# roahmlab/armour

Measured on AMD Instinct MI355X. Metric: planning iters/s (eval_g+jac) Kinova 7-DOF, 100 timesteps × 20 obstacles, higher is better.
Workload: dtype f64

## Files before the change

armour_amd/csrc/api.hip:

```cpp
#include <algorithm>
#include <cmath>
#include <cstdarg>
#include <chrono>
#include <cstring>
#include <mutex>
#include <new>

#include "../../include/armour_robot_fetch.h"
#include "../../include/armour_robot_kinova.h"
#include "bezier.h"
#include "cacc.h"
#include "common.h"
#include "solver_common.h"

static thread_local char g_err[512] = "";

void armour_set_error(const char* fmt, ...) {
    va_list ap;
    va_start(ap, fmt);
    vsnprintf(g_err, sizeof(g_err), fmt, ap);
    va_end(ap);
}

extern "C" const char* armour_last_error(void) { return g_err; }

extern "C" void armour_robot_kinova_gen3_no_gripper(ArmourRobot* robot) { armour_fill_kinova_gen3_no_gripper(robot); }
extern "C" void armour_robot_kinova_gen3_gripper(ArmourRobot* robot) { armour_fill_kinova_gen3_gripper(robot); }
extern "C" void armour_robot_fetch(ArmourRobot* robot) { armour_fill_fetch(robot); }
extern "C" int armour_robot_fetch8(ArmourRobot* robot) {
#if ARMOUR_MAX_FACTORS >= 8
    if (!robot) { armour_set_error("null argument"); return ARMOUR_EINVAL; }
    armour_fill_fetch8(robot);
    return ARMOUR_OK;
#else
    (void)robot;
    armour_set_error("armour_robot_fetch8: an 8-factor robot needs the 128-bit-key library (libarmour_hip_k128.so: armour_abi_max_factors() == 8)");
    return ARMOUR_EINVAL;
#endif
}
extern "C" void armour_params_default(ArmourParams* params, int32_t T) { armour_fill_default_params(params, T); }

extern "C" int armour_device_available(void) {
    int n = 0;
    if (hipGetDeviceCount(&n) != hipSuccess) return 0;
    return n > 0 ? 1 : 0;
}

namespace {
struct PinnedRange { const char* p; size_t bytes; };
std::mutex g_pinned_mu;
std::vector<PinnedRange> g_pinned;
bool in_pinned(const void* q, size_t bytes) {
    if (!q) return true;
    const char* c = static_cast<const char*>(q);
    std::lock_guard<std::mutex> lk(g_pinned_mu);
    for (const PinnedRange& r : g_pinned)
        if (c >= r.p && c + bytes <= r.p + r.bytes) return true;
    return false;
}
}

extern "C" int armour_alloc_pinned(uint64_t bytes, void** out) {
    if (!out) { armour_set_error("null argument"); return ARMOUR_EINVAL; }
    HIPCHK(hipHostMalloc(out, bytes ? bytes : 1, hipHostMallocDefault));
    std::lock_guard<std::mutex> lk(g_pinned_mu);
    g_pinned.push_back({static_cast<const char*>(*out), (size_t)(bytes ? bytes : 1)});
    return ARMOUR_OK;
}
extern "C" void armour_free_pinned(void* p) {
    if (!p) return;
    {
        std::lock_guard<std::mutex> lk(g_pinned_mu);
        for (size_t i = 0; i < g_pinned.size(); i++)
            if (g_pinned[i].p == p) { g_pinned.erase(g_pinned.begin() + i); break; }
    }
    (void)hipHostFree(p);
}

static int ensure_capacity(ArmourPlanner* h, int B, int O) {
    if (B <= h->allocB && O <= h->allocO) return ARMOUR_OK;
    const int nb = B > h->allocB ? B : h->allocB, no = O > h->allocO ? O : h->allocO;
    h->allocB = 0; h->allocO = 0;
    const size_t nl = (size_t)nb * h->J * h->T, nt = (size_t)nb * h->n * h->T;
    ARMOUR_TRY(h->d_link_count.reserve(nl));
    ARMOUR_TRY(h->d_link_center.reserve(nl * 3));
    ARMOUR_TRY(h->d_link_indep.reserve(nl * 3));
    ARMOUR_TRY(h->d_link_keys.reserve(nl * h->lim.link_monomials));
    ARMOUR_TRY(h->d_link_coeff.reserve(nl * h->lim.link_monomials * 3));
    ARMOUR_TRY(h->d_tq_count.reserve(nt));
    ARMOUR_TRY(h->d_tq_center.reserve(nt));
    ARMOUR_TRY(h->d_tq_indep.reserve(nt));
    ARMOUR_TRY(h->d_tq_keys.reserve(nt * h->lim.torque_monomials));
    ARMOUR_TRY(h->d_tq_coeff.reserve(nt * h->lim.torque_monomials));
    ARMOUR_TRY(h->d_planes.reserve((size_t)nb * armour_planes_per_problem(h->J * h->T * no)));
    ARMOUR_TRY(h->d_planes_ll.reserve((size_t)nb * armour_planes_ll_per_problem(h->J * h->T)));
    ARMOUR_TRY(h->d_obs_center.reserve((size_t)nb * 3 * (no > 0 ? no : 1)));
    ARMOUR_TRY(h->d_plane_skip.reserve((size_t)nb));
    ARMOUR_TRY(h->d_bez.reserve((size_t)nb * 3 * h->n));
    const size_t mmax = (size_t)h->n * h->T + (size_t)h->J * h->T * no + 4 * h->n;
    ARMOUR_TRY(h->d_k.reserve((size_t)nb * h->n));
    ARMOUR_TRY(h->d_g.reserve((size_t)nb * mmax + std::max((size_t)nb * mmax * h->n, (size_t)nb * h->T * h->J * 3)));
    h->d_jac = h->d_g + (size_t)nb * mmax;
    ARMOUR_TRY(h->d_bounds.reserve((size_t)2 * nb * mmax));
    h->allocB = nb;
    h->allocO = no;
    return ARMOUR_OK;
}

P2Tables armour_make_tables(const ArmourPlanner* h) {
    P2Tables tb;
    memset(&tb, 0, sizeof(tb));
    tb.B = h->B; tb.T = h->T; tb.J = h->J; tb.n = h->n; tb.O = h->O; tb.Q = h->Q; tb.m = h->m;
    tb.capL = h->lim.link_monomials; tb.capT = h->lim.torque_monomials;
    tb.row0 = h->row0; tb.mode = h->mode;
    tb.link_count = h->d_link_count; tb.link_center = h->d_link_center; tb.link_indep = h->d_link_indep;
    tb.link_keys = h->d_link_keys; tb.link_coeff = h->d_link_coeff;
    tb.tq_count = h->d_tq_count; tb.tq_center = h->d_tq_center; tb.tq_indep = h->d_tq_indep;
    tb.tq_keys = h->d_tq_keys; tb.tq_coeff = h->d_tq_coeff;
    tb.planes = h->d_planes; tb.planes_ll = h->d_planes_ll; tb.ll_shared = h->ll_shared;
    tb.ex_allowed = h->tune(ARMOUR_OPT_P2_EX);
    tb.obs_center = (h->d_from_center && (h->B >= 8 || !h->planes_have_d)) ? h->d_obs_center : nullptr;
    tb.plane_skip = h->d_plane_skip; tb.bez = h->d_bez;
    for (int i = 0; i < ARMOUR_MAX_FACTORS; i++) tb.k_range[i] = h->params.k_range[i];
    tb.duration = h->params.duration;
    return tb;
}

namespace {
struct TuningSpec { int option; double def, lo, hi; };
const TuningSpec kTuning[] = {
    {ARMOUR_OPT_P1_STEP_WAVES, 0, 0, 4}, {ARMOUR_OPT_P1_STEP_FREE, 1, 0, 1}, {ARMOUR_OPT_P1_STEP_SPLIT_FK, -1, -1, 1}, {ARMOUR_OPT_P1_STEP_AUX3, 1, 0, 1},
    {ARMOUR_OPT_P1_MAX_WAVES_PER_CU, 4, 1, 8}, {ARMOUR_OPT_P1_TWO_PASS, 1, 0, 1}, {ARMOUR_OPT_P1_STEP_PAIRS, 1, 0, 2}, {ARMOUR_OPT_P1_STEP_QUEUE, 1, 0, 3}, {ARMOUR_OPT_P1_STEP_TAIL_CROSS, 0, 0, 514}, {ARMOUR_OPT_P1_STEP_TWO_CU, 3, 0, 33}, {ARMOUR_OPT_P1_STEP_LEAN_BACK, 1, 0, 3}, {ARMOUR_OPT_P1_TV_TAIL_CROSS, 111, 0, 514} ,
    {ARMOUR_OPT_P1_TV_MIN_GROUPS, 31, 1, 1e6}, {ARMOUR_OPT_P1_TV_WAVES, 0, 0, 8}, {ARMOUR_OPT_P1_TV_FREE, 1, 0, 1}, {ARMOUR_OPT_P1_TV_SPLIT_FK, -1, -1, 1},
    {ARMOUR_OPT_P1_TV_DEDICATED, 1, 0, 1}, {ARMOUR_OPT_P1_TV_HELP_SHIFT, 0, 0, 3}, {ARMOUR_OPT_P1_TV_HELPERS, 1, 0, 31}, {ARMOUR_OPT_P1_TV_HELP_MIN, 192, 1, 1e6},
    {ARMOUR_OPT_P1_TV_HELP_N, 1, 0, 1}, {ARMOUR_OPT_P1_TV_AUX3, 1, 0, 1}, {ARMOUR_OPT_P1_TV_ROW_WIDTH, 0, 0, 64}, {ARMOUR_OPT_P1_FULL_PLANES, 0, 0, 1},
    {ARMOUR_OPT_P2_EX, 1, 0, 1}, {ARMOUR_OPT_STEPS_GRAPH_MIN, 2, 0, 1e6}, {ARMOUR_OPT_PINNED_MODE, 0, 0, 2}, {ARMOUR_OPT_CULL_ROWS, 0, 0, 1},
    {ARMOUR_OPT_SOLVE_SUB_TILES, 48, 1, 1e6}, {ARMOUR_OPT_SOLVE_DEVICE, 1, 0, 2}, {ARMOUR_OPT_SOLVE_CUT_TILES, 156, 1, 1e6}, {ARMOUR_OPT_SOLVE_BLOCKS, 0, 0, 1e6},
    {ARMOUR_OPT_SOLVE_SUB_BATCH, 0, 0, 1e6}, {ARMOUR_OPT_SOLVE_ROW_CAP, 0, 0, 1e7}, {ARMOUR_OPT_SOLVE_HARD_CAP_S, 0, 0, 1e6}, {ARMOUR_OPT_SOLVE_WAVES_PER_SIMD, 0, 0, 2}, {ARMOUR_OPT_SOLVE_CULL, -1, -1, 1},
};
const TuningSpec* tuning_spec(int option) {
    for (const TuningSpec& t : kTuning) if (t.option == option) return &t;
    return nullptr;
}
}
void armour_tuning_defaults(double* tuning) {
    for (int o = ARMOUR_OPT_FIRST_TUNING; o <= ARMOUR_OPT_LAST_TUNING; o++) tuning[o - ARMOUR_OPT_FIRST_TUNING] = 0.0;
    for (const TuningSpec& t : kTuning) tuning[t.option - ARMOUR_OPT_FIRST_TUNING] = t.def;
}
bool armour_trace_p1() { static const bool on = getenv("ARMOUR_P1_TRACE") != nullptr; return on; }
BuildStamps& armour_build_stamps() { static thread_local BuildStamps s; return s; }
void armour_build_stamp(const char* name) {
    if (!armour_trace_p1()) return;
    BuildStamps& s = armour_build_stamps();
    if (s.n < 12) { s.t[s.n] = std::chrono::duration<double, std::micro>(std::chrono::steady_clock::now().time_since_epoch()).count(); s.name[s.n] = name; s.n++; }
}
static void armour_build_stamps_print(const char* what) {
    if (!armour_trace_p1()) return;
    BuildStamps& s = armour_build_stamps();
    fprintf(stderr, "[%s, host side, us]", what);
    for (int i = 1; i < s.n; i++) fprintf(stderr, " %s %.1f", s.name[i], s.t[i] - s.t[i - 1]);
    if (s.n > 1) fprintf(stderr, " | total %.1f\n", s.t[s.n - 1] - s.t[0]);
}
bool armour_trace_solve() { static const bool on = getenv("ARMOUR_SOLVE_TIMING") != nullptr; return on; }

extern "C" int armour_create(const ArmourRobot* robot, const ArmourParams* params, const ArmourLimits* limits,
                             int32_t device, ArmourPlanner** out) {
    if (!robot || !params || !out) { armour_set_error("armour_create: null argument"); return ARMOUR_EINVAL; }
    if (!armour_robot_shape_ok(robot)) {
        armour_set_error("armour_create: unsupported robot (joints=%d, factors=%d; max %d joints, %d factors -- the monomial key "
                         "packs 9 bits per factor into 64, RT/PZsparse.h:8-21)", robot->num_joints, robot->num_factors,
                         ARMOUR_MAX_JOINTS, ARMOUR_MAX_FACTORS);
        return ARMOUR_EINVAL;
    }
    for (int i = 0; i < robot->num_joints; i++)
        if ((i < robot->num_factors) != (robot->axes[i] != 0)) {
            armour_set_error("armour_create: the actuated joints must come first and the fixed ones last (RT/Dynamics.cu:103-105)");
            return ARMOUR_EINVAL;
        }
    if (params->num_time_steps < 2 || (params->num_time_steps & 1)) {
        armour_set_error("armour_create: num_time_steps must be even and >= 2 (RT/Parameters.h:16)");
        return ARMOUR_EINVAL;
    }
    int ndev = 0;
    if (hipGetDeviceCount(&ndev) != hipSuccess || ndev <= 0) {
        armour_set_error("armour_create: no HIP device visible -- libarmour_hip has no CPU path");
        return ARMOUR_EDEVICE;
    }
    if (device < 0 || device >= ndev) { armour_set_error("armour_create: device %d out of range (%d visible)", device, ndev); return ARMOUR_EINVAL; }
    HIPCHK(hipSetDevice(device));
    ArmourPlanner* h = new (std::nothrow) ArmourPlanner();
    if (!h) { armour_set_error("out of host memory"); return ARMOUR_EINVAL; }
    h->robot = *robot;
    h->params = *params;
    armour_tuning_defaults(h->tuning);
    ArmourLimits lim;
    memset(&lim, 0, sizeof(lim));
    if (limits) lim = *limits;
    if (lim.max_batch <= 0) lim.max_batch = 1;
    if (lim.max_obstacles <= 0) lim.max_obstacles = 40;
    if (lim.link_monomials <= 0) lim.link_monomials = 32;
    if (lim.torque_monomials <= 0) lim.torque_monomials = 128;
    if (lim.work_monomials <= 0) lim.work_monomials = 1024;
    if (lim.raw_terms <= 0) lim.raw_terms = 4096;
    h->lim = lim;
    h->ub = armour_ultimate_bound(robot);
    h->device = device;
    h->T = params->num_time_steps; h->J = robot->num_joints; h->n = robot->num_factors;
    hipError_t e = hipStreamCreateWithFlags(&h->stream, hipStreamNonBlocking);
    if (e != hipSuccess) { armour_set_error("hipStreamCreate failed: %s", hipGetErrorString(e)); delete h; return ARMOUR_EDEVICE; }
    *out = h;
    return ARMOUR_OK;
}

double* armour_handle_pinned(ArmourPlanner* h, int slot, size_t bytes) {
    if (h->solve_pin[slot] && h->solve_pin_bytes[slot] >= bytes) return static_cast<double*>(h->solve_pin[slot]);
    if (h->solve_pin[slot]) { armour_free_pinned(h->solve_pin[slot]); h->solve_pin[slot] = nullptr; h->solve_pin_bytes[slot] = 0; }
    void* p = nullptr;
    if (armour_alloc_pinned(bytes, &p) != ARMOUR_OK) return nullptr;
    h->solve_pin[slot] = p; h->solve_pin_bytes[slot] = bytes;
    return static_cast<double*>(p);
}

static void drop_step_graphs(ArmourPlanner* h) {
    for (auto& g : h->step_graphs) (void)hipGraphExecDestroy(g.exec);
    h->step_graphs.clear();
}

extern "C" void armour_destroy(ArmourPlanner* h) {
    if (!h) return;
    (void)hipSetDevice(h->device);
    if (h->stream) (void)hipStreamSynchronize(h->stream);
    drop_step_graphs(h);
    for (void* pin : h->solve_pin) armour_free_pinned(pin);
    armour_p1_free(h);
    if (h->stream) (void)hipStreamDestroy(h->stream);
    delete h;
}

static int begin_problem_set(ArmourPlanner* h, int B, int O, const double* q0, const double* qd0, const double* qdd0,
                             const double* q_des, int mode = ARMOUR_MODE_ARMOUR) {
    if (!h || !q0 || !qd0 || !qdd0 || !q_des) { armour_set_error("null argument"); return ARMOUR_EINVAL; }
    if (B < 1 || O < 0) { armour_set_error("bad batch/obstacle count (B=%d, O=%d)", B, O); return ARMOUR_EINVAL; }
    {
        const double* arrs[4] = {q0, qd0, qdd0, q_des};
        const size_t bn = (size_t)B * h->n;
        for (int a = 0; a < 4; a++)
            if (const size_t i = first_nonfinite(arrs[a], bn); i < bn) { armour_set_error("non-finite entry in the initial state / goal arrays (array %d, entry %zu)", a, i); return ARMOUR_EINVAL; }
    }
    HIPCHK(hipSetDevice(h->device));
    h->ready = false;
    h->rel.fresh = false; h->rel2.fresh = false;
    h->bounds_on_device = false; h->bounds_on_host = false;
    h->tables_from_host = false;
    h->stats_fresh = false;
    drop_step_graphs(h);
    int rc = ensure_capacity(h, B, O);
    if (rc != ARMOUR_OK) return rc;
    h->B = B; h->O = O; h->Q = h->J * h->T * O;
    h->mode = mode;
    h->row0 = h->no_torque() ? 0 : h->n * h->T;
    h->m = h->row0 + h->Q + 4 * h->n;
    h->d_jac = h->d_g + (size_t)B * h->m;
    const size_t bn = (size_t)B * h->n;
    h->h_q0.assign(q0, q0 + bn); h->h_qd0.assign(qd0, qd0 + bn);
    h->h_qdes.assign(q_des, q_des + bn);
    if (mode == ARMOUR_MODE_ARMTD) { h->h_qdd0.assign(bn, 0.0); h->h_krange.assign(qdd0, qdd0 + bn); }
    else { h->h_qdd0.assign(qdd0, qdd0 + bn); h->h_krange.clear(); }
    std::vector<double> bz((size_t)B * 3 * h->n);
    const double D = mode == ARMOUR_MODE_ARMTD ? 1.0 : h->params.duration;
    for (int b = 0; b < B; b++)
        for (int i = 0; i < h->n; i++) {
            bz[((size_t)b * 3 + 0) * h->n + i] = q0[b * h->n + i];
            bz[((size_t)b * 3 + 1) * h->n + i] = qd0[b * h->n + i] * D;
            bz[((size_t)b * 3 + 2) * h->n + i] = qdd0[b * h->n + i] * D * D;
        }
    HIPCHK(hipMemcpy(h->d_bez, bz.data(), bz.size() * sizeof(double), hipMemcpyHostToDevice));
    return ARMOUR_OK;
}

int armour_refresh_table_stats(ArmourPlanner* h) {
    if (h->stats_fresh) { h->stats_fresh = false; return ARMOUR_OK; }
    const size_t nl = (size_t)h->B * h->J * h->T, nt = (size_t)h->B * h->n * h->T;
    std::vector<int> lc(nl), tc(nt);
    HIPCHK(hipMemcpy(lc.data(), h->d_link_count, nl * sizeof(int), hipMemcpyDeviceToHost));
    HIPCHK(hipMemcpy(tc.data(), h->d_tq_count, nt * sizeof(int), hipMemcpyDeviceToHost));
    long long sl = 0, st = 0;
    int ml = 0, mt = 0;
    for (int v : lc) { sl += v; if (v > ml) ml = v; }
    for (int v : tc) { st += v; if (v > mt) mt = v; }
    h->sum_link = sl; h->sum_torque = st; h->max_link = ml; h->max_torque = mt;
    h->h_plane_skip.assign((size_t)h->B, 0ull);
    if (h->O > 0) HIPCHK(hipMemcpy(h->h_plane_skip.data(), h->d_plane_skip, (size_t)h->B * sizeof(unsigned long long), hipMemcpyDeviceToHost));
    if (h->O > 0 && armour_trace_p1()) {
        unsigned long long all_and = ~0ull, all_or = 0ull;
        for (unsigned long long v : h->h_plane_skip) { all_and &= v; all_or |= v; }
        fprintf(stderr, "[P1 planes] plane_skip of %d problem(s): AND 0x%09llx OR 0x%09llx\n", h->B, all_and & ((1ull << ARMOUR_NPLANES) - 1ull), all_or & ((1ull << ARMOUR_NPLANES) - 1ull));
    }
    return ARMOUR_OK;
}

static int check_obstacles(int B, int O, const double* obstacles) {
    if (O > 0 && !obstacles) { armour_set_error("obstacles is null but O=%d", O); return ARMOUR_EINVAL; }
    const size_t cnt = (size_t)B * O * 12;
    if (const size_t i = first_nonfinite(obstacles, cnt); i < cnt) { armour_set_error("non-finite obstacle entry %zu", i); return ARMOUR_EINVAL; }
    return ARMOUR_OK;
}

extern "C" int armour_set_problems(ArmourPlanner* h, int32_t B, int32_t O, const double* q0, const double* qd0,
                                   const double* qdd0, const double* q_des, const double* obstacles) {
    armour_build_stamps().n = 0;
    armour_build_stamp("start");
    int rc = begin_problem_set(h, B, O, q0, qd0, qdd0, q_des);
    if (rc != ARMOUR_OK) return rc;
    ARMOUR_TRY(check_obstacles(B, O, obstacles));
    armour_build_stamp("checks+bezier-upload");
    rc = armour_p1_build(h, obstacles);
    if (rc != ARMOUR_OK) return rc;
    armour_build_stamp("copy-out");
    rc = armour_refresh_table_stats(h);
    if (rc != ARMOUR_OK) return rc;
    h->ready = true;
    armour_build_stamp("table-stats");
    armour_build_stamps_print("armour_set_problems");
    return ARMOUR_OK;
}

extern "C" int armour_set_problems_armtd(ArmourPlanner* h, int32_t B, int32_t O, const double* q0, const double* qd0, const double* q_des,
                                         const double* jrs, const double* k_range, const double* obstacles) {
    if (!jrs || !k_range) { armour_set_error("null argument"); return ARMOUR_EINVAL; }
    int rc = begin_problem_set(h, B, O, q0, qd0, k_range, q_des, ARMOUR_MODE_ARMTD);
    if (rc != ARMOUR_OK) return rc;
    ARMOUR_TRY(check_obstacles(B, O, obstacles));
    const size_t cnt = (size_t)B * h->n * 6 * h->T;
    if (const size_t i = first_nonfinite(jrs, cnt); i < cnt) { armour_set_error("non-finite entry %zu in the offline JRS tables", i); return ARMOUR_EINVAL; }
    ARMOUR_TRY(h->d_jrs.reserve(cnt));
    HIPCHK(hipMemcpy(h->d_jrs, jrs, cnt * sizeof(double), hipMemcpyHostToDevice));
    rc = armour_p1_build(h, obstacles);
    if (rc != ARMOUR_OK) return rc;
    rc = armour_refresh_table_stats(h);
    if (rc != ARMOUR_OK) return rc;
    h->ready = true;
    return ARMOUR_OK;
}

extern "C" int armour_debug_load_tables(ArmourPlanner* h, int32_t B, int32_t O, const double* q0, const double* qd0,
                                        const double* qdd0, const double* q_des, const int32_t* link_count,
                                        const double* link_center, const uint64_t* link_keys, const double* link_coeffs,
                                        int32_t cap_l, const int32_t* torque_count, const double* torque_center,
                                        const uint64_t* torque_keys, const double* torque_coeffs, int32_t cap_t,
                                        const double* A, const double* d, const double* delta, const double* torque_radius) {
    int rc = begin_problem_set(h, B, O, q0, qd0, qdd0, q_des);
    if (rc != ARMOUR_OK) return rc;
    h->build_ms = 0; h->build_info[0] = h->build_info[1] = h->build_info[2] = h->build_info[3] = 0;
    h->h_prune_margin.clear();
    const int J = h->J, T = h->T, n = h->n, capL = h->lim.link_monomials, capT = h->lim.torque_monomials;
    const size_t nl = (size_t)B * J * T, nt = (size_t)B * n * T;
    std::vector<double> lc(nl * 3), li(nl * 3), lco(nl * capL * 3, 0.0), tc(nt), ti(nt), tco(nt * capT, 0.0);
    std::vector<uint32_t> lk(nl * capL, 0), tk(nt * capT, 0);
    for (size_t i = 0; i < nl; i++) {
        if (link_count[i] > capL) { armour_set_error("link PZ %zu has %d monomials > capacity %d", i, link_count[i], capL); return ARMOUR_ECAPACITY; }
        for (int e = 0; e < 3; e++) { lc[i * 3 + e] = link_center[(i * 2) * 3 + e]; li[i * 3 + e] = link_center[(i * 2 + 1) * 3 + e]; }
        for (int mo = 0; mo < link_count[i]; mo++) {
            lk[i * capL + mo] = (uint32_t)link_keys[i * cap_l + mo];
            for (int e = 0; e < 3; e++) lco[(i * capL + mo) * 3 + e] = link_coeffs[(i * cap_l + mo) * 3 + e];
        }
    }
    for (size_t i = 0; i < nt; i++) {
        if (torque_count[i] > capT) { armour_set_error("torque PZ %zu has %d monomials > capacity %d", i, torque_count[i], capT); return ARMOUR_ECAPACITY; }
        tc[i] = torque_center[i * 2]; ti[i] = torque_center[i * 2 + 1];
        for (int mo = 0; mo < torque_count[i]; mo++) { tk[i * capT + mo] = (uint32_t)torque_keys[i * cap_t + mo]; tco[i * capT + mo] = torque_coeffs[i * cap_t + mo]; }
    }
    const size_t ppp = armour_planes_per_problem(h->Q);
    std::vector<double> pl((size_t)B * ppp, 0.0);
    for (int b = 0; b < B; b++)
        for (int t = 0; t < T; t++)
            for (int l = 0; l < J; l++)
                for (int o = 0; o < O; o++)
                    for (int p = 0; p < 36; p++) {
                        const size_t src = ((((size_t)b * T + t) * J + l) * O + o) * 36 + p;
                        const int q = (l * T + t) * O + o;
                        double* base = &pl[(size_t)b * ppp];
                        base[armour_plane_index(h->Q, q, p, 0)] = A[src * 3 + 0]; base[armour_plane_index(h->Q, q, p, 1)] = A[src * 3 + 1];
                        base[armour_plane_index(h->Q, q, p, 2)] = A[src * 3 + 2];
                        base[armour_plane_index(h->Q, q, p, 3)] = d[src]; base[armour_plane_index(h->Q, q, p, 4)] = delta[src];
                    }
#define UP(dst, vec) HIPCHK(hipMemcpy(dst, vec.data(), vec.size() * sizeof(vec[0]), hipMemcpyHostToDevice))
    HIPCHK(hipMemcpy(h->d_link_count, link_count, nl * sizeof(int), hipMemcpyHostToDevice));
    HIPCHK(hipMemcpy(h->d_tq_count, torque_count, nt * sizeof(int), hipMemcpyHostToDevice));
    UP(h->d_link_center, lc); UP(h->d_link_indep, li); UP(h->d_link_keys, lk); UP(h->d_link_coeff, lco);
    UP(h->d_tq_center, tc); UP(h->d_tq_indep, ti); UP(h->d_tq_keys, tk); UP(h->d_tq_coeff, tco);
    if (!pl.empty()) UP(h->d_planes, pl);
    {
        const int JT = J * T;
        std::vector<double> pll((size_t)B * armour_planes_ll_per_problem(JT), 0.0);
        bool shared = O > 0;
        for (int b = 0; b < B && O > 0; b++)
            for (int t = 0; t < T; t++)
                for (int l = 0; l < J; l++)
                    for (int p = ARMOUR_FIRST_LL_PLANE; p < 36; p++)
                        for (int o = 0; o < O; o++) {
                            const size_t src = ((((size_t)b * T + t) * J + l) * O + o) * 36 + p, src0 = ((((size_t)b * T + t) * J + l) * O) * 36 + p;
                            for (int cc = 0; cc < 3; cc++) {
                                if (o == 0) pll[(size_t)b * armour_planes_ll_per_problem(JT) + armour_plane_ll_index(JT, l * T + t, p - ARMOUR_FIRST_LL_PLANE, cc)] = A[src * 3 + cc];
                                else if (memcmp(&A[src * 3 + cc], &A[src0 * 3 + cc], sizeof(double)) != 0) shared = false;
                            }
                        }
        UP(h->d_planes_ll, pll);
        h->ll_shared = shared ? 1 : 0;
        h->d_from_center = 0;
        h->planes_lean = 0; h->planes_have_d = 1;
    }
    HIPCHK(hipMemset(h->d_plane_skip, 0, (size_t)B * sizeof(unsigned long long)));
#undef UP
    h->h_torque_radius.assign(torque_radius, torque_radius + (size_t)B * n * T);
    h->h_link_gens.assign((size_t)B * T * J * 18, 0.0);
    rc = armour_refresh_table_stats(h);
    if (rc != ARMOUR_OK) return rc;
    h->tables_from_host = true;
    h->ready = true;
    return ARMOUR_OK;
}

static const double* torque_radius_of(const ArmourPlanner* h, int b) { return h->no_torque() ? nullptr : &h->h_torque_radius[(size_t)b * h->n * h->T]; }

extern "C" int armour_get_sizes(const ArmourPlanner* h, int32_t* B, int32_t* n, int32_t* m) {
    NEED_READY(h);
    if (B) *B = h->B;
    if (n) *n = h->n;
    if (m) *m = h->m;
    return ARMOUR_OK;
}

extern "C" int armour_get_bounds(ArmourPlanner* h, double* x_l, double* x_u, double* g_l, double* g_u) {
    NEED_READY(h);
    const int n = h->n;
    if (x_l) for (int i = 0; i < n; i++) x_l[i] = -1.0;
    if (x_u) for (int i = 0; i < n; i++) x_u[i] = 1.0;
    if (!g_l || !g_u) return ARMOUR_OK;
    const slv::RowRule R = armour_row_rule(h);
    const slv::RowLimits L = armour_row_limits(h);
    for (int b = 0; b < h->B; b++) {
        const double* tr = torque_radius_of(h, b);
        for (int r = 0; r < R.m; r++) slv::row_bounds(R, L, r, tr, &g_l[(size_t)b * R.m + r], &g_u[(size_t)b * R.m + r]);
    }
    return ARMOUR_OK;
}

int armour_checked_collision_rows(const ArmourPlanner* h) {
    return h->mode == ARMOUR_MODE_ARMTD ? (h->n - 1 < h->J ? h->n - 1 : h->J) * h->T * h->O : h->Q;
}

slv::RowRule armour_row_rule(const ArmourPlanner* h) {
    slv::RowRule R;
    R.n = h->n; R.T = h->T; R.m = h->m; R.row0 = h->row0; R.Q = h->Q; R.n_checked = armour_checked_collision_rows(h);
    R.torque_slack = h->params.torque_violation_threshold; R.collision_slack = h->params.collision_violation_threshold;
    return R;
}

slv::RowLimits armour_row_limits(const ArmourPlanner* h) {
    slv::RowLimits L;
    for (int j = 0; j < ARMOUR_MAX_FACTORS; j++) {
        L.torque_limits[j] = h->robot.torque_limits[j]; L.lb[j] = h->robot.state_limits_lb[j]; L.ub[j] = h->robot.state_limits_ub[j]; L.speed[j] = h->robot.speed_limits[j];
    }
    L.qe = h->ub.qe; L.qde = h->ub.qde;
    return L;
}

void armour_plan_coeffs(const ArmourPlanner* h, size_t ix, double c[3]) {
    const double D = h->params.duration;
    const bool armtd = h->mode == ARMOUR_MODE_ARMTD;
    c[0] = h->h_q0[ix];
    c[1] = armtd ? h->h_qd0[ix] : h->h_qd0[ix] * D;
    c[2] = armtd ? h->h_krange[ix] : h->h_qdd0[ix] * D * D;
}

extern "C" int armour_eval_f(ArmourPlanner* h, const double* k, double* f) {
    NEED_READY(h);
    const int n = h->n;
    for (int b = 0; b < h->B; b++) {
        double sq[slv::NV];
        for (int i = 0; i < n; i++) {
            const size_t ix = (size_t)b * n + i;
            double c[3];
            armour_plan_coeffs(h, ix, c);
            const double qp = slv::plan_point(h->mode, c[0], c[1], c[2], h->params.k_range[i], k[ix], h->params.t_plan);
            const double e = h->robot.continuous[i] ? slv::wrap_to_pi(h->h_qdes[ix] - qp) : (h->h_qdes[ix] - qp);
            sq[i] = e * e;
        }
        f[b] = slv::cost_from_sq(n, h->continuous_mask(), sq, h->params.cost_scale);
    }
    return ARMOUR_OK;
}

extern "C" int armour_eval_grad_f(ArmourPlanner* h, const double* k, double* grad_f) {
    NEED_READY(h);
    const int n = h->n;
    const double tp = h->params.t_plan;
    for (int b = 0; b < h->B; b++)
        for (int i = 0; i < n; i++) {
            const size_t ix = (size_t)b * n + i;
            double c[3];
            armour_plan_coeffs(h, ix, c);
            const double qp = slv::plan_point(h->mode, c[0], c[1], c[2], h->params.k_range[i], k[ix], tp);
            const double dk = slv::plan_dk(h->mode, c[2], h->params.k_range[i], tp);
            const double e = h->robot.continuous[i] ? slv::wrap_to_pi(qp - h->h_qdes[ix]) : (qp - h->h_qdes[ix]);
            grad_f[ix] = 2 * e * dk * h->params.cost_scale;
        }
    return ARMOUR_OK;
}

extern "C" int armour_desired_trajectory(int32_t n, const double* q0, const double* qd0, const double* qdd0, const double* k_range,
                                         double duration, const double* k, double t, double* q, double* qd, double* qdd) {
    if (n < 1 || !q0 || !qd0 || !qdd0 || !k_range || !k || !(duration > 0)) { armour_set_error("bad argument"); return ARMOUR_EINVAL; }
    const double D = duration, s = t / D;
    for (int i = 0; i < n; i++) {
        const double a = qd0[i] * D, b = qdd0[i] * D * D, ka = k_range[i] * k[i];
        if (q) q[i] = bez::q_des(q0[i], a, b, ka, s);
        if (qd) qd[i] = bez::qd_des(q0[i], a, b, ka, s) / D;
        if (qdd) qdd[i] = bez::qdd_des(q0[i], a, b, ka, s) / (D * D);
    }
    return ARMOUR_OK;
}

extern "C" int armour_eval_g_jac_device(ArmourPlanner* h, const double* d_k, double* d_g, double* d_jac, void* stream) {
    NEED_READY(h);
    if (!d_k) { armour_set_error("d_k is null"); return ARMOUR_EINVAL; }
    const P2Tables tb = armour_make_tables(h);
    return armour_p2_launch(tb, h->max_link, h->max_torque, h->h_plane_skip.data(), d_k, d_g, d_jac, stream ? (hipStream_t)stream : h->stream);
}

static int enqueue_steps(ArmourPlanner* h, const double* d_k, int steps, double* d_g, double* d_jac, hipStream_t st) {
    const P2Tables tb = armour_make_tables(h);
    const size_t stride = (size_t)h->B * h->n;
    for (int s = 0; s < steps; s++) {
        int rc = armour_p2_launch(tb, h->max_link, h->max_torque, h->h_plane_skip.data(), d_k + (size_t)s * stride, d_g, d_jac, st);
        if (rc != ARMOUR_OK) return rc;
    }
    return ARMOUR_OK;
}

static int steps_graph(ArmourPlanner* h, const double* d_k, int steps, double* d_g, double* d_jac, hipGraphExec_t* out) {
    h->graph_clock++;
    for (auto& g : h->step_graphs)
        if (g.d_k == d_k && g.steps == steps && g.d_g == d_g && g.d_jac == d_jac) { g.last_use = h->graph_clock; *out = g.exec; return ARMOUR_OK; }
    HIPCHK(hipSetDevice(h->device));
    HIPCHK(hipStreamSynchronize(h->stream));
    hipGraph_t graph = nullptr;
    HIPCHK(hipStreamBeginCapture(h->stream, hipStreamCaptureModeThreadLocal));
    const int rc = enqueue_steps(h, d_k, steps, d_g, d_jac, h->stream);
    const hipError_t e = hipStreamEndCapture(h->stream, &graph);
    if (rc != ARMOUR_OK) { if (graph) (void)hipGraphDestroy(graph); return rc; }
    if (e != hipSuccess) { armour_set_error("hipStreamEndCapture failed: %s", hipGetErrorString(e)); return ARMOUR_EDEVICE; }
    hipGraphExec_t exec = nullptr;
    const hipError_t ei = hipGraphInstantiate(&exec, graph, nullptr, nullptr, 0);
    (void)hipGraphDestroy(graph);
    if (ei != hipSuccess) { armour_set_error("hipGraphInstantiate failed: %s", hipGetErrorString(ei)); return ARMOUR_EDEVICE; }
    if (h->step_graphs.size() >= 4) {
        size_t lru = 0;
        for (size_t i = 1; i < h->step_graphs.size(); i++) if (h->step_graphs[i].last_use < h->step_graphs[lru].last_use) lru = i;
        (void)hipGraphExecDestroy(h->step_graphs[lru].exec);
        h->step_graphs.erase(h->step_graphs.begin() + lru);
    }
    h->step_graphs.push_back({d_k, steps, d_g, d_jac, exec, h->graph_clock});
    *out = exec;
    return ARMOUR_OK;
}

static bool steps_use_graph(const ArmourPlanner* h, int steps) {
    const int min_steps = h->tune(ARMOUR_OPT_STEPS_GRAPH_MIN);
    return min_steps > 0 && steps >= min_steps;
}

extern "C" int armour_prepare_steps(ArmourPlanner* h, const double* d_k, int32_t steps, double* d_g, double* d_jac) {
    NEED_READY(h);
    if (!d_k || steps < 0) { armour_set_error("bad argument"); return ARMOUR_EINVAL; }
    if (!steps_use_graph(h, steps)) return ARMOUR_OK;
    hipGraphExec_t exec;
    return steps_graph(h, d_k, steps, d_g, d_jac, &exec);
}

extern "C" int armour_eval_g_jac_device_steps(ArmourPlanner* h, const double* d_k, int32_t steps, double* d_g, double* d_jac,
                                              void* stream) {
    NEED_READY(h);
    if (!d_k || steps < 0) { armour_set_error("bad argument"); return ARMOUR_EINVAL; }
    if (steps == 0 || (!d_g && !d_jac)) return ARMOUR_OK;
    const hipStream_t st = stream ? (hipStream_t)stream : h->stream;
    if (steps_use_graph(h, steps))
        for (auto& g : h->step_graphs)
            if (g.d_k == d_k && g.steps == steps && g.d_g == d_g && g.d_jac == d_jac) {
                g.last_use = ++h->graph_clock;
                HIPCHK(hipGraphLaunch(g.exec, st));
                return ARMOUR_OK;
            }
    return enqueue_steps(h, d_k, steps, d_g, d_jac, st);
}

extern "C" int armour_eval_g_jac_device_multi(ArmourPlanner* h, const double* d_k, int32_t points, double* d_g, double* d_jac,
                                              void* stream) {
    NEED_READY(h);
    if (!d_k || points < 0) { armour_set_error("bad argument"); return ARMOUR_EINVAL; }
    if (points == 0) return ARMOUR_OK;
    const P2Tables tb = armour_make_tables(h);
    const long long bn = (long long)h->B * h->n, bm = (long long)h->B * h->m;
    return armour_p2_launch(tb, h->max_link, h->max_torque, h->h_plane_skip.data(), d_k, d_g, d_jac, stream ? (hipStream_t)stream : h->stream,
                            points, bn, bm, bm * h->n);
}

int armour_spin_on_stream(hipStream_t st) {
    for (;;) {
        const hipError_t q = hipStreamQuery(st);
        if (q == hipSuccess) return ARMOUR_OK;
        if (q != hipErrorNotReady) { armour_set_error("hipStreamQuery failed: %s", hipGetErrorString(q)); return ARMOUR_EDEVICE; }
    }
}

extern "C" int armour_eval_g_jac(ArmourPlanner* h, const double* k, double* g, double* jac) {
    NEED_READY(h);
    if (!k) { armour_set_error("k is null"); return ARMOUR_EINVAL; }
    HIPCHK(hipSetDevice(h->device));
    const size_t bn = (size_t)h->B * h->n, bm = (size_t)h->B * h->m;
    const P2Tables tb = armour_make_tables(h);
    const int pinned_mode = h->tune(ARMOUR_OPT_PINNED_MODE);
    const bool all_pinned = in_pinned(k, bn * sizeof(double)) && in_pinned(g, bm * sizeof(double)) && in_pinned(jac, bm * h->n * sizeof(double));
    if (all_pinned && pinned_mode == 1) {
        int rc = armour_p2_launch(tb, h->max_link, h->max_torque, h->h_plane_skip.data(), k, g, jac, h->stream);
        if (rc != ARMOUR_OK) return rc;
        return armour_spin_on_stream(h->stream);
    }
    const double* k_dev = h->d_k;
    if (all_pinned && pinned_mode == 2) k_dev = k;
    else HIPCHK(hipMemcpyAsync(h->d_k, k, bn * sizeof(double), hipMemcpyHostToDevice, h->stream));
    int rc = armour_p2_launch(tb, h->max_link, h->max_torque, h->h_plane_skip.data(), k_dev, g ? h->d_g : nullptr, jac ? h->d_jac : nullptr, h->stream);
    if (rc != ARMOUR_OK) return rc;
    if (g && jac && jac == g + bm) {
        HIPCHK(hipMemcpyAsync(g, h->d_g, bm * (1 + (size_t)h->n) * sizeof(double), hipMemcpyDeviceToHost, h->stream));
        return armour_spin_on_stream(h->stream);
    }
    if (g) HIPCHK(hipMemcpyAsync(g, h->d_g, bm * sizeof(double), hipMemcpyDeviceToHost, h->stream));
    if (jac) HIPCHK(hipMemcpyAsync(jac, h->d_jac, bm * h->n * sizeof(double), hipMemcpyDeviceToHost, h->stream));
    return armour_spin_on_stream(h->stream);
}

extern "C" int armour_check_feasible(ArmourPlanner* h, const double* g, int32_t* feasible) {
    NEED_READY(h);
    const slv::RowRule R = armour_row_rule(h);
    const slv::RowLimits L = armour_row_limits(h);
    for (int b = 0; b < h->B; b++) {
        const double* gb = g + (size_t)b * R.m;
        const double* tr = torque_radius_of(h, b);
        bool ok = true;
        for (int r = 0; r < R.m && ok; r++) {
            double l, u;
            slv::row_bounds(R, L, r, tr, &l, &u);
            ok = !slv::outside_slack(R, r, gb[r], l, u);
        }
        feasible[b] = ok ? 1 : 0;
    }
    return ARMOUR_OK;
}

namespace {
struct BoundsArgs {
    slv::RowRule rule;
    slv::RowLimits lim;
    const double* tr;
    double* lo; double* hi;
};
__global__ __launch_bounds__(256) void armour_bounds_kernel(BoundsArgs a) {
    const int b = blockIdx.y, r = blockIdx.x * 256 + threadIdx.x, m = a.rule.m;
    if (r >= m) return;
    double l, u;
    slv::row_bounds(a.rule, a.lim, r, a.tr + (size_t)b * a.rule.n * a.rule.T, &l, &u);
    a.lo[(size_t)b * m + r] = l;
    a.hi[(size_t)b * m + r] = u;
}
}

int armour_bounds_launch(ArmourPlanner* h, const double* d_tr) {
    const size_t bm = (size_t)h->B * h->m;
    BoundsArgs a;
    a.rule = armour_row_rule(h); a.lim = armour_row_limits(h);
    a.lo = h->d_bounds; a.hi = h->d_bounds + bm;
    a.tr = d_tr;
    hipLaunchKernelGGL(armour_bounds_kernel, dim3((h->m + 255) / 256, h->B), dim3(256), 0, h->stream, a);
    HIPCHK(hipGetLastError());
    h->bounds_on_device = true;
    return ARMOUR_OK;
}

int armour_upload_bounds(ArmourPlanner* h) {
    if (h->bounds_on_device) return ARMOUR_OK;
    const double* d_tr = nullptr;
    if (!h->no_torque()) {
        const size_t ntr = (size_t)h->B * h->n * h->T;
        ARMOUR_TRY(h->d_tr_stage.reserve(ntr));
        HIPCHK(hipMemcpyAsync(h->d_tr_stage, h->h_torque_radius.data(), ntr * sizeof(double), hipMemcpyHostToDevice, h->stream));
        d_tr = h->d_tr_stage;
    }
    const int rc = armour_bounds_launch(h, d_tr);
    if (rc != ARMOUR_OK) return rc;
    HIPCHK(hipStreamSynchronize(h->stream));
    return ARMOUR_OK;
}

extern "C" int armour_set_option(ArmourPlanner* h, int32_t option, double value) {
    if (!h) { armour_set_error("null handle"); return ARMOUR_EINVAL; }
    if (option == ARMOUR_OPT_P1_BUILD && (value == 0.0 || value == 1.0 || value == 2.0)) { h->opt_p1_build = (int)value; return ARMOUR_OK; }
    if (option == ARMOUR_OPT_P1_WORK_MEMORY_MB && value >= 0.0 && value <= 1e9) { h->opt_p1_work_mb = value; return ARMOUR_OK; }
    if (option == ARMOUR_OPT_P1_KEEP_WORK_MEMORY && (value == 0.0 || value == 1.0)) { h->opt_p1_keep_work = (int)value; return ARMOUR_OK; }
    if (const TuningSpec* t = tuning_spec(option)) {
        bool ok = value >= t->lo && value <= t->hi && (option == ARMOUR_OPT_SOLVE_HARD_CAP_S || value == (double)(long long)value);
        if (ok && (option == ARMOUR_OPT_P1_STEP_TAIL_CROSS || option == ARMOUR_OPT_P1_TV_TAIL_CROSS)) {
            const int v = (int)value, lo2 = v % 100, hi2 = v / 100;
            ok = (lo2 <= 4 || (lo2 >= 10 && lo2 <= 14)) && hi2 <= 5;
        }
        if (ok && option == ARMOUR_OPT_P1_TV_ROW_WIDTH) ok = value == 0.0 || value == 50.0 || value == 64.0;
        if (ok && option == ARMOUR_OPT_P1_STEP_TWO_CU) { const int lv = (int)value % 10; ok = lv <= 3 && (value < 10.0 || lv >= 1); if (ok) h->p1_two_cu_off = false; }
        if (ok) {
            h->tuning[option - ARMOUR_OPT_FIRST_TUNING] = value;
            h->p1_step_cap_hint = 0; h->p1_tv_shape_hint = 0;
            return ARMOUR_OK;
        }
    }
    armour_set_error("armour_set_option: unknown option %d or bad value %g", option, value);
    return ARMOUR_EINVAL;
}

extern "C" int armour_abi_max_factors(void) { return ARMOUR_MAX_FACTORS; }

extern "C" int armour_device_memory(int32_t device, uint64_t* free_bytes, uint64_t* total_bytes) {
    int ndev = 0;
    if (hipGetDeviceCount(&ndev) != hipSuccess || device < 0 || device >= ndev) { (void)hipGetLastError(); armour_set_error("armour_device_memory: no such device %d", device); return ARMOUR_EDEVICE; }
    HIPCHK(hipSetDevice(device));
    size_t f = 0, t = 0;
    HIPCHK(hipMemGetInfo(&f, &t));
    if (free_bytes) *free_bytes = f;
    if (total_bytes) *total_bytes = t;
    return ARMOUR_OK;
}

extern "C" int armour_get_option(ArmourPlanner* h, int32_t option, double* value) {
    if (!h || !value) { armour_set_error("null argument"); return ARMOUR_EINVAL; }
    if (option == ARMOUR_OPT_P1_BUILD) { *value = h->opt_p1_build; return ARMOUR_OK; }
    if (option == ARMOUR_OPT_P1_WORK_MEMORY_MB) { *value = h->opt_p1_work_mb; return ARMOUR_OK; }
    if (option == ARMOUR_OPT_P1_KEEP_WORK_MEMORY) { *value = h->opt_p1_keep_work; return ARMOUR_OK; }
    if (tuning_spec(option)) { *value = h->tuning[option - ARMOUR_OPT_FIRST_TUNING]; return ARMOUR_OK; }
    armour_set_error("armour_get_option: unknown option %d", option);
    return ARMOUR_EINVAL;
}

namespace {
struct ViolArgs {
    slv::RowRule rule;
    const double* g; const double* lo; const double* hi;
    ArmourViolation* out;
};
__global__ __launch_bounds__(256) void armour_violation_kernel(ViolArgs a) {
    __shared__ slv::ViolShared<1> sh;
    const int b = blockIdx.x, tid = threadIdx.x, m = a.rule.m;
    const double* g = a.g + (size_t)b * m;
    const double* lo = a.lo + (size_t)b * m;
    const double* hi = a.hi + (size_t)b * m;
    slv::ViolPartial p[1];
    for (int r = tid; r < m; r += 256) p[0].take(a.rule, r, g[r], lo[r], hi[r]);
    slv::ViolPartial::tree_reduce(sh, p, tid);
    if (tid == 0) a.out[b] = slv::ViolPartial::finish(sh, 0);
}
}

static int eval_violations_device_impl(ArmourPlanner* h, const double* d_k, ArmourViolation* d_out, void* stream, bool allow_cull) {
    NEED_READY(h);
    if (!d_k || !d_out) { armour_set_error("null argument"); return ARMOUR_EINVAL; }
    HIPCHK(hipSetDevice(h->device));
    int rc = armour_upload_bounds(h);
    if (rc != ARMOUR_OK) return rc;
    const hipStream_t st = stream ? (hipStream_t)stream : h->stream;
    if (allow_cull && h->tune(ARMOUR_OPT_CULL_ROWS)) return armour_eval_violations_culled(h, d_k, d_out, st);
    const P2Tables tb = armour_make_tables(h);
    rc = armour_p2_launch(tb, h->max_link, h->max_torque, h->h_plane_skip.data(), d_k, h->d_g, nullptr, st);
    if (rc != ARMOUR_OK) return rc;
    ViolArgs a;
    a.rule = armour_row_rule(h);
    a.g = h->d_g; a.lo = h->d_bounds; a.hi = h->d_bounds + (size_t)h->B * h->m; a.out = d_out;
    hipLaunchKernelGGL(armour_violation_kernel, dim3(h->B), dim3(256), 0, st, a);
    HIPCHK(hipGetLastError());
    return ARMOUR_OK;
}

extern "C" int armour_eval_violations_device(ArmourPlanner* h, const double* d_k, ArmourViolation* d_out, void* stream) {
    return eval_violations_device_impl(h, d_k, d_out, stream, true);
}

extern "C" int armour_eval_violations(ArmourPlanner* h, const double* k, ArmourViolation* out) {
    NEED_READY(h);
    if (!k || !out) { armour_set_error("null argument"); return ARMOUR_EINVAL; }
    HIPCHK(hipSetDevice(h->device));
    const size_t bn = (size_t)h->B * h->n;
    ARMOUR_TRY(h->d_viol.reserve((size_t)h->B));
    double* hk = armour_handle_pinned(h, 6, bn * sizeof(double));
    ArmourViolation* hv = reinterpret_cast<ArmourViolation*>(armour_handle_pinned(h, 7, (size_t)h->B * sizeof(ArmourViolation)));
    if (!hk || !hv) return ARMOUR_EDEVICE;
    memcpy(hk, k, bn * sizeof(double));
    HIPCHK(hipMemcpyAsync(h->d_k, hk, bn * sizeof(double), hipMemcpyHostToDevice, h->stream));
    bool in_box = true;
    for (size_t i = 0; i < bn && in_box; i++) in_box = fabs(k[i]) <= 1.0;
    int rc = eval_violations_device_impl(h, h->d_k, h->d_viol, h->stream, in_box);
    if (rc != ARMOUR_OK) return rc;
    HIPCHK(hipMemcpyAsync(hv, h->d_viol, (size_t)h->B * sizeof(ArmourViolation), hipMemcpyDeviceToHost, h->stream));
    rc = armour_spin_on_stream(h->stream);
    if (rc != ARMOUR_OK) return rc;
    memcpy(out, hv, (size_t)h->B * sizeof(ArmourViolation));
    return ARMOUR_OK;
}

extern "C" int armour_get_torque_radius(ArmourPlanner* h, double* out) {
    NEED_READY(h);
    memcpy(out, h->h_torque_radius.data(), h->h_torque_radius.size() * sizeof(double));
    return ARMOUR_OK;
}

extern "C" int armour_get_link_generators(ArmourPlanner* h, double* out) {
    NEED_READY(h);
    memcpy(out, h->h_link_gens.data(), h->h_link_gens.size() * sizeof(double));
    return ARMOUR_OK;
}

extern "C" int armour_get_link_centers(ArmourPlanner* h, const double* k, double* centers) {
    NEED_READY(h);
    HIPCHK(hipSetDevice(h->device));
    const size_t bn = (size_t)h->B * h->n, cnt = (size_t)h->B * h->T * h->J * 3;
    HIPCHK(hipMemcpyAsync(h->d_k, k, bn * sizeof(double), hipMemcpyHostToDevice, h->stream));
    const P2Tables tb = armour_make_tables(h);
    int rc = armour_p2_slice_links_launch(tb, h->d_k, h->d_jac, h->stream);
    if (rc != ARMOUR_OK) return rc;
    HIPCHK(hipMemcpyAsync(centers, h->d_jac, cnt * sizeof(double), hipMemcpyDeviceToHost, h->stream));
    HIPCHK(hipStreamSynchronize(h->stream));
    return ARMOUR_OK;
}

extern "C" int armour_get_pz(ArmourPlanner* h, int32_t b, int32_t which, int32_t i, int32_t t, double* center,
                             uint64_t* keys, double* coeffs, int32_t capacity) {
    NEED_READY(h);
    if (b < 0 || b >= h->B || t < 0 || t >= h->T || which < 0 || which > 1 || i < 0 || i >= (which == 0 ? h->J : h->n)) {
        armour_set_error("armour_get_pz: index out of range");
        return ARMOUR_EINVAL;
    }
    if (which == 1 && h->no_torque()) {
        if (center) center[0] = center[1] = 0.0;
        return 0;
    }
    HIPCHK(hipSetDevice(h->device));
    HIPCHK(hipStreamSynchronize(h->stream));
    const int sz = which == 0 ? 3 : 1;
    const int cap = which == 0 ? h->lim.link_monomials : h->lim.torque_monomials;
    const size_t idx = which == 0 ? ((size_t)b * h->J + i) * h->T + t : ((size_t)b * h->n + i) * h->T + t;
    int cnt = 0;
    HIPCHK(hipMemcpy(&cnt, (which == 0 ? h->d_link_count : h->d_tq_count) + idx, sizeof(int), hipMemcpyDeviceToHost));
    if (center) {
        HIPCHK(hipMemcpy(center, (which == 0 ? h->d_link_center : h->d_tq_center) + idx * sz, sz * sizeof(double), hipMemcpyDeviceToHost));
        HIPCHK(hipMemcpy(center + sz, (which == 0 ? h->d_link_indep : h->d_tq_indep) + idx * sz, sz * sizeof(double), hipMemcpyDeviceToHost));
    }
    if (keys && coeffs) {
        if (capacity < cnt) { armour_set_error("armour_get_pz: capacity %d < count %d", capacity, cnt); return ARMOUR_EINVAL; }
        std::vector<uint32_t> k32(cnt > 0 ? cnt : 1);
        if (cnt > 0) {
            HIPCHK(hipMemcpy(k32.data(), (which == 0 ? h->d_link_keys : h->d_tq_keys) + idx * cap, cnt * sizeof(uint32_t), hipMemcpyDeviceToHost));
            HIPCHK(hipMemcpy(coeffs, (which == 0 ? h->d_link_coeff : h->d_tq_coeff) + idx * cap * sz, (size_t)cnt * sz * sizeof(double), hipMemcpyDeviceToHost));
        }
        for (int mo = 0; mo < cnt; mo++) keys[mo] = k32[mo];
    }
    return cnt;
}

extern "C" int armour_get_table_sizes(ArmourPlanner* h, int64_t* out4) {
    NEED_READY(h);
    out4[0] = h->sum_link; out4[1] = h->sum_torque; out4[2] = h->max_link; out4[3] = h->max_torque;
    return ARMOUR_OK;
}

extern "C" int armour_get_hyperplanes(ArmourPlanner* h, double* A, double* d, double* delta) {
    NEED_READY(h);
    HIPCHK(hipSetDevice(h->device));
    HIPCHK(hipStreamSynchronize(h->stream));
    const int B = h->B, T = h->T, J = h->J, O = h->O;
    const size_t ppp = armour_planes_per_problem(h->Q);
    std::vector<double> pl(h->Q > 0 ? (size_t)B * ppp : 0);
    if (pl.empty()) return ARMOUR_OK;
    if (h->planes_lean) {
        DevBuf<double> d_full;
        int rc = d_full.reserve(pl.size());
        if (rc == ARMOUR_OK) rc = armour_p1_full_planes(h, d_full);
        if (rc != ARMOUR_OK) return rc;
        if (hipMemcpy(pl.data(), d_full, pl.size() * sizeof(double), hipMemcpyDeviceToHost) != hipSuccess) { armour_set_error("copy of the half-space table failed"); return ARMOUR_EDEVICE; }
    } else
    HIPCHK(hipMemcpy(pl.data(), h->d_planes, pl.size() * sizeof(double), hipMemcpyDeviceToHost));
    for (int b = 0; b < B; b++)
        for (int t = 0; t < T; t++)
            for (int l = 0; l < J; l++)
                for (int o = 0; o < O; o++)
                    for (int p = 0; p < 36; p++) {
                        const size_t dst = ((((size_t)b * T + t) * J + l) * O + o) * 36 + p;
                        const int q = (l * T + t) * O + o;
                        const double* base = &pl[(size_t)b * ppp];
                        if (A) { A[dst * 3 + 0] = base[armour_plane_index(h->Q, q, p, 0)]; A[dst * 3 + 1] = base[armour_plane_index(h->Q, q, p, 1)]; A[dst * 3 + 2] = base[armour_plane_index(h->Q, q, p, 2)]; }
                        if (d) d[dst] = base[armour_plane_index(h->Q, q, p, 3)];
                        if (delta) delta[dst] = base[armour_plane_index(h->Q, q, p, 4)];
                    }
    return ARMOUR_OK;
}

extern "C" int armour_debug_pz_op(ArmourPlanner* h, int32_t op, int32_t nops, const int32_t* sz, const int32_t* cnt, const uint64_t* const* keys,
                                  const double* const* coef, const double* cen, const double* ind, const double* ind2, const double* consts,
                                  int32_t r, int32_t out_cap, uint64_t* out_keys, double* out_coef, double* out_misc) {
    if (!h || nops < 1 || nops > 3 || op < 0 || op > 11) { armour_set_error("armour_debug_pz_op: bad argument"); return ARMOUR_EINVAL; }
    for (int o = 0; o < nops; o++)
        if ((sz[o] != 1 && sz[o] != 3 && sz[o] != 9) || cnt[o] < 0 || cnt[o] > h->lim.work_monomials || (sz[o] == 9 && o == 1 && cnt[o] > 8)) {
            armour_set_error("armour_debug_pz_op: bad operand"); return ARMOUR_EINVAL;
        }
    return armour_p1_debug_pz_op(h, op, nops, sz, cnt, keys, coef, cen, ind, ind2, consts, r, out_cap, out_keys, out_coef, out_misc);
}

extern "C" int armour_get_plane_skip(ArmourPlanner* h, uint64_t* plane_skip) {
    NEED_READY(h);
    if (!plane_skip) { armour_set_error("null argument"); return ARMOUR_EINVAL; }
    for (int b = 0; b < h->B; b++) plane_skip[b] = (uint64_t)h->h_plane_skip[b] & ((1ull << ARMOUR_NPLANES) - 1ull);
    return ARMOUR_OK;
}

extern "C" int armour_get_prune_margin(ArmourPlanner* h, double* margin) {
    NEED_READY(h);
    if (!margin) { armour_set_error("null argument"); return ARMOUR_EINVAL; }
    if ((int)h->h_prune_margin.size() != h->B) { armour_set_error("no reach-set build on this handle (tables loaded by armour_debug_load_tables carry no prune margin)"); return ARMOUR_ESTATE; }
    for (int b = 0; b < h->B; b++) margin[b] = h->h_prune_margin[(size_t)b];
    return ARMOUR_OK;
}

extern "C" int armour_get_build_ms(ArmourPlanner* h, double* ms) {
    NEED_READY(h);
    *ms = h->build_ms;
    return ARMOUR_OK;
}

extern "C" int armour_get_build_info(ArmourPlanner* h, int32_t* out4) {
    NEED_READY(h);
    if (!out4) { armour_set_error("null argument"); return ARMOUR_EINVAL; }
    for (int i = 0; i < 4; i++) out4[i] = h->build_info[i];
    return ARMOUR_OK;
}
```

armour_amd/csrc/common.h:

```cpp
#pragma once

#include <hip/hip_runtime.h>

#include <cstdint>
#include <cstdio>
#include <string>
#include <vector>

#include "../../include/armour_hip.h"
#include "device_mem.h"
#include "row_rules.h"

#define ARMOUR_NPLANES 36
#define ARMOUR_PLANE_COMPONENTS 5

#define ARMOUR_FIRST_LL_PLANE 21
#define ARMOUR_N_LL_PLANES 15
__host__ __device__ inline int armour_row_stride(int Q) { return (Q + 15) & ~15; }
__host__ __device__ inline size_t armour_planes_ab_offset(int Q) { (void)Q; return 0; }
__host__ __device__ inline size_t armour_planes_cd_offset(int Q) { return (size_t)2 * ARMOUR_NPLANES * armour_row_stride(Q); }
__host__ __device__ inline size_t armour_planes_dll_offset(int Q) { return (size_t)4 * ARMOUR_NPLANES * armour_row_stride(Q); }
__host__ __device__ inline size_t armour_planes_d_offset(int Q) { return (size_t)(4 * ARMOUR_NPLANES + 16) * armour_row_stride(Q); }
__host__ __device__ inline size_t armour_planes_per_problem(int Q) { return (size_t)(5 * ARMOUR_NPLANES + 16) * armour_row_stride(Q); }
__host__ __device__ inline size_t armour_plane_index(int Q, int q, int p, int c) {
    const size_t Qs = (size_t)armour_row_stride(Q);
    if (c < 2) return ((size_t)p * Qs + q) * 2 + c;
    if (c == 2) return armour_planes_cd_offset(Q) + ((size_t)p * Qs + q) * 2;
    if (c == 3) return armour_planes_d_offset(Q) + (size_t)p * Qs + q;
    if (p < ARMOUR_FIRST_LL_PLANE) return armour_planes_cd_offset(Q) + ((size_t)p * Qs + q) * 2 + 1;
    return armour_planes_dll_offset(Q) + ((size_t)((p - ARMOUR_FIRST_LL_PLANE) >> 1) * Qs + q) * 2 + ((p - ARMOUR_FIRST_LL_PLANE) & 1);
}
#define ARMOUR_RECOMPUTE_D_ROWS 32768
#define ARMOUR_LL_RECORD 48
__host__ __device__ inline size_t armour_planes_ll_per_problem(int JT) { return (size_t)ARMOUR_LL_RECORD * (size_t)JT; }
__host__ __device__ inline size_t armour_plane_ll_index(int JT, int lt, int pll, int c) { (void)JT; return (size_t)lt * ARMOUR_LL_RECORD + (size_t)pll * 3 + c; }

int armour_spin_on_stream(hipStream_t st);

struct P2Tables {
    int B, T, J, n, O, Q, m;
    int capL, capT;
    int row0;
    const int* link_count;
    const double* link_center;
    const double* link_indep;
    const uint32_t* link_keys;
    const double* link_coeff;
    const int* tq_count;
    const double* tq_center;
    const double* tq_indep;
    const uint32_t* tq_keys;
    const double* tq_coeff;
    const double* planes;
    const double* obs_center;
    const double* planes_ll;
    int ll_shared;
    int ex_allowed;
    int mode;
    const unsigned long long* plane_skip;
    const double* bez;
    double k_range[ARMOUR_MAX_FACTORS];
    double duration;
};

#define ARMOUR_MODE_ARMOUR 0
#define ARMOUR_MODE_ARMTD 1

struct SolveDeviceWork {
    DevBuf<unsigned char> ctl;
    DevBuf<unsigned char> blk_word;
    int words_clean = 0;
    DevBuf<unsigned char> blk_rows, qp_rows, flags;
};

struct RelLists {
    DevBuf<unsigned char> mask;
    DevBuf<int> rows;
    DevBuf<int> count;
    DevBuf<double> packed;
    DevBuf<long long> pack_off;
    DevBuf<int> extra;
    std::vector<int> h_count, h_tq_count;
    int max_count = 0;
    bool fresh = false;
    double ms = 0;
};

struct ArmourPlanner {
    ArmourRobot robot;
    ArmourParams params;
    ArmourLimits lim;
    ArmourUltimateBound ub;
    int device = 0;
    hipStream_t stream = nullptr;
    int T = 0, J = 0, n = 0;
    int B = 0, O = 0, Q = 0, m = 0;
    bool ready = false;
    int mode = ARMOUR_MODE_ARMOUR;
    bool no_torque() const { return mode == ARMOUR_MODE_ARMTD || params.input_constraints_off != 0; }
    int continuous_mask() const { int mk = 0; for (int i = 0; i < n; i++) if (robot.continuous[i]) mk |= 1 << i; return mk; }
    int row0 = 0;
    std::vector<double> h_krange;
    DevBuf<double> d_jrs;
    void* solve_pin[10] = {nullptr, nullptr, nullptr, nullptr, nullptr, nullptr, nullptr, nullptr, nullptr, nullptr};
    size_t solve_pin_bytes[10] = {0, 0, 0, 0, 0, 0, 0, 0, 0, 0};
    bool stats_fresh = false;
    int opt_p1_build = 0;
    double opt_p1_work_mb = 0;
    int opt_p1_keep_work = 1;
    double tuning[ARMOUR_OPT_LAST_TUNING - ARMOUR_OPT_FIRST_TUNING + 1];
    int tune(int option) const { return (int)tuning[option - ARMOUR_OPT_FIRST_TUNING]; }
    double tune_f(int option) const { return tuning[option - ARMOUR_OPT_FIRST_TUNING]; }
    DevBuf<ArmourViolation> d_viol;
    RelLists rel, rel2;
    int rel2_tq_cap = 0;
    DevBuf<unsigned char> d_sweep;
    SolveDeviceWork solve_dev;
    DevBuf<double> d_bounds;
    bool bounds_on_device = false, bounds_on_host = false;
    bool tables_from_host = false;
    std::vector<double> h_gl, h_gu;
    std::vector<double> h_q0, h_qd0, h_qdd0, h_qdes;
    std::vector<double> h_torque_radius;
    DevBuf<double> d_tr_stage;
    std::vector<double> h_link_gens;
    std::vector<unsigned long long> h_plane_skip;
    std::vector<double> h_prune_margin;
    int allocB = 0, allocO = 0;
    DevBuf<int> d_link_count;
    DevBuf<double> d_link_center;
    DevBuf<double> d_link_indep;
    DevBuf<uint32_t> d_link_keys;
    DevBuf<double> d_link_coeff;
    DevBuf<int> d_tq_count;
    DevBuf<double> d_tq_center;
    DevBuf<double> d_tq_indep;
    DevBuf<uint32_t> d_tq_keys;
    DevBuf<double> d_tq_coeff;
    DevBuf<double> d_planes;
    DevBuf<double> d_obs_center;
    int d_from_center = 0;
    int planes_lean = 0;
    int planes_have_d = 1;
    double planes_ms = 0;
    DevBuf<double> d_planes_ll;
    int ll_shared = 0;
    DevBuf<unsigned long long> d_plane_skip;
    DevBuf<double> d_bez;
    DevBuf<double> d_k;
    DevBuf<double> d_g;
    double* d_jac = nullptr;
    double build_ms = 0;
    int p1_step_cap_hint = 0, p1_tv_shape_hint = 0;
    bool p1_two_cu_off = false;
    int p1_hint_B = 0, p1_hint_T = 0, p1_hint_O = 0, p1_hint_builds = 0;
    int build_info[4] = {0, 0, 0, 0};
    int max_link = 0, max_torque = 0;
    long long sum_link = 0, sum_torque = 0;
    void* p1 = nullptr;
    struct StepsGraph { const double* d_k; int steps; double* d_g; double* d_jac; hipGraphExec_t exec; unsigned long long last_use; };
    std::vector<StepsGraph> step_graphs;
    unsigned long long graph_clock = 0;
};

void armour_tuning_defaults(double* tuning);
bool armour_trace_p1();
bool armour_trace_solve();

int armour_p2_launch(const P2Tables& tb, int max_link, int max_torque, const unsigned long long* h_skip, const double* d_k, double* d_g, double* d_jac, hipStream_t stream,
                     int steps = 1, long long k_stride = 0, long long g_stride = 0, long long j_stride = 0, bool skip_collision_blocks = false);
int armour_relevance_build(ArmourPlanner* h, bool for_solver);
int armour_eval_violations_culled(ArmourPlanner* h, const double* d_k, ArmourViolation* d_out, hipStream_t st);
int armour_refresh_table_stats(ArmourPlanner* h);
int armour_checked_collision_rows(const ArmourPlanner* h);
slv::RowRule armour_row_rule(const ArmourPlanner* h);
slv::RowLimits armour_row_limits(const ArmourPlanner* h);
#define NEED_READY(h)                                                                        \
    if (!(h)) { armour_set_error("null handle"); return ARMOUR_EINVAL; }                     \
    if (!(h)->ready) { armour_set_error("no problem set: call armour_set_problems first"); return ARMOUR_ESTATE; }
void armour_plan_coeffs(const ArmourPlanner* h, size_t ix, double c[3]);
double* armour_handle_pinned(ArmourPlanner* h, int slot, size_t bytes);
int armour_p2_slice_links_launch(const P2Tables& tb, const double* d_k, double* d_centers, hipStream_t stream);
P2Tables armour_make_tables(const ArmourPlanner* h);
int armour_upload_bounds(ArmourPlanner* h);
struct BuildStamps { double t[12]; const char* name[12]; int n; };
BuildStamps& armour_build_stamps();
void armour_build_stamp(const char* name);
int armour_bounds_launch(ArmourPlanner* h, const double* d_torque_radius);

int armour_p1_build(ArmourPlanner* h, const double* obstacles);
void armour_p1_free(ArmourPlanner* h);
int armour_p1_full_planes(ArmourPlanner* h, double* d_full);

inline int armour_p1_auto_kernel(int B, int T, int min_groups, bool fk_only) {
    return (long long)B * T >= 50ll * (fk_only ? min_groups * 5 / 3 : min_groups) ? ARMOUR_P1_KERNEL_TIME_VECTORISED : ARMOUR_P1_KERNEL_PER_STEP;
}

int armour_p1_debug_pz_op(ArmourPlanner* h, int op, int nops, const int* sz, const int* cnt, const uint64_t* const* keys,
                          const double* const* coef, const double* cen, const double* ind, const double* ind2, const double* consts,
                          int r, int out_cap, uint64_t* out_keys, double* out_coef, double* out_misc);
```

armour_amd/csrc/solver.hip:

```cpp
#include <chrono>
#include <cmath>
#include <cstdio>
#include <cstdlib>
#include <cstring>
#include <thread>
#include <vector>

#include "bezier.h"
#include "common.h"
#include "solver_common.h"
#include "solver_device.h"

using slv::NV;
using slv::SolveRow;

namespace {

constexpr double kInf = 1e300;
using Clock = std::chrono::steady_clock;

bool spd_solve(const double* M, int q, const double* rhs, double* y) {
    double L[NV][NV], inv[NV];
    for (int i = 0; i < q; i++)
        for (int j = 0; j <= i; j++) {
            double s = M[i * NV + j];
            for (int k = 0; k < j; k++) s -= L[i][k] * L[j][k];
            if (i == j) {
                if (s <= 1e-14 * std::fabs(M[i * NV + i]) || s <= 0) return false;
                L[i][i] = std::sqrt(s);
                inv[i] = 1.0 / L[i][i];
            } else {
                L[i][j] = s * inv[j];
            }
        }
    double t[NV];
    for (int i = 0; i < q; i++) {
        double s = rhs[i];
        for (int k = 0; k < i; k++) s -= L[i][k] * t[k];
        t[i] = s * inv[i];
    }
    for (int i = q - 1; i >= 0; i--) {
        double s = t[i];
        for (int k = i + 1; k < q; k++) s -= L[k][i] * y[k];
        y[i] = s * inv[i];
    }
    return true;
}

struct QpRow {
    double a[NV];
    double b;
};

struct QpResult {
    double x[NV];
    double max_mult;
    int iterations;
    bool feasible;
    int dropped, dropped_mid, excluded, active;
};

QpResult solve_qp(int n, const double* Gd, const double* g0, const std::vector<QpRow>& rows, int max_iter = slv::kQpMaxSteps, int box_rows = 0) {
    QpResult res;
    res.iterations = 0; res.feasible = true; res.max_mult = 0;
    res.dropped = res.dropped_mid = res.excluded = res.active = 0;
    double x[NV], invG[NV];
    for (int j = 0; j < n; j++) { invG[j] = 1.0 / Gd[j]; x[j] = -g0[j] * invG[j]; }
    if (box_rows == 2 * n && (int)rows.size() >= box_rows) {
        const int m0 = (int)rows.size() - box_rows;
        double lo[NV], hi[NV], d[NV];
        for (int j = 0; j < n; j++) { lo[j] = rows[m0 + 2 * j].b; hi[j] = -rows[m0 + 2 * j + 1].b; }
        const double mm = slv::box_clipped_step(n, Gd, invG, g0, lo, hi, d);
        bool ok = true;
        for (int i = 0; i < (int)rows.size() && ok; i++) {
            double s = -rows[i].b;
            for (int j = 0; j < n; j++) s += rows[i].a[j] * d[j];
            if (s < -1e-7) ok = false;
        }
        if (ok) {
            for (int j = 0; j < n; j++) res.x[j] = d[j];
            res.max_mult = mm;
            return res;
        }
    }
    int A[NV];
    double u[NV + 1];
    int q = 0;
    const int m = (int)rows.size();
    std::vector<char> is_active(m, 0), excluded(m, 0);
    for (;;) {
        int p = -1;
        double worst = -1e-10;
        for (int i = 0; i < m; i++) {
            if (is_active[i] || excluded[i]) continue;
            double s = -rows[i].b;
            for (int j = 0; j < n; j++) s += rows[i].a[j] * x[j];
            if (s < worst) { worst = s; p = i; }
        }
        if (p < 0) break;
        if (++res.iterations > max_iter) { res.feasible = false; break; }
        const double* np = rows[p].a;
        double up = 0.0;
        bool added = false;
        for (int guard = 0; guard < 4 * NV + 8 && !added; guard++) {
            double r[NV] = {0}, z[NV];
            if (q > 0) {
                double M[NV * NV], rhs[NV];
                for (int i = 0; i < q; i++) {
                    for (int k = 0; k <= i; k++) {
                        double s = 0;
                        for (int j = 0; j < n; j++) s += rows[A[i]].a[j] * rows[A[k]].a[j] * invG[j];
                        M[i * NV + k] = s; M[k * NV + i] = s;
                    }
                    double s = 0;
                    for (int j = 0; j < n; j++) s += rows[A[i]].a[j] * np[j] * invG[j];
                    rhs[i] = s;
                }
                if (!spd_solve(M, q, rhs, r)) { excluded[p] = 1; res.excluded++; break; }
            }
            double zz = 0, znp = 0;
            for (int j = 0; j < n; j++) {
                double s = np[j];
                for (int i = 0; i < q; i++) s -= rows[A[i]].a[j] * r[i];
                z[j] = s * invG[j];
                zz += z[j] * z[j];
                znp += z[j] * np[j];
            }
            double t1 = kInf;
            int l = -1;
            for (int i = 0; i < q; i++)
                if (r[i] > 1e-14 && u[i] / r[i] < t1) { t1 = u[i] / r[i]; l = i; }
            double sp = -rows[p].b;
            for (int j = 0; j < n; j++) sp += np[j] * x[j];
            double t2 = kInf;
            if (zz > 1e-24 && znp > 1e-16) t2 = -sp / znp;
            if (t2 < 0) t2 = 0;
            const double t = t1 < t2 ? t1 : t2;
            if (t >= kInf) { res.feasible = false; break; }
            if (t2 >= kInf) {
                for (int i = 0; i < q; i++) u[i] -= t * r[i];
                up += t;
                is_active[A[l]] = 0;
                res.dropped++; if (l < q - 1) res.dropped_mid++;
                for (int i = l; i < q - 1; i++) { A[i] = A[i + 1]; u[i] = u[i + 1]; }
                q--;
                continue;
            }
            for (int j = 0; j < n; j++) x[j] += t * z[j];
            for (int i = 0; i < q; i++) u[i] -= t * r[i];
            up += t;
            if (t == t2) {
                if (q >= n) { res.feasible = false; break; }
                A[q] = p; u[q] = up; q++;
                is_active[p] = 1;
                added = true;
            } else {
                is_active[A[l]] = 0;
                res.dropped++; if (l < q - 1) res.dropped_mid++;
                for (int i = l; i < q - 1; i++) { A[i] = A[i + 1]; u[i] = u[i + 1]; }
                q--;
            }
        }
        if (!res.feasible) break;
        if (!added && !excluded[p]) { excluded[p] = 1; res.excluded++; }
    }
    res.active = q;
    for (int j = 0; j < n; j++) res.x[j] = x[j];
    for (int i = 0; i < q; i++) if (u[i] > res.max_mult) res.max_mult = u[i];
    for (int i = 0; i < m && res.feasible; i++) {
        double s = -rows[i].b;
        for (int j = 0; j < n; j++) s += rows[i].a[j] * x[j];
        if (s < -1e-7) res.feasible = false;
    }
    return res;
}

constexpr int kElasticAttempts = 4;
inline double elastic_sigma(int attempt) { return attempt == 0 ? 0.0 : attempt == 1 ? 0.5 : attempt == 2 ? 0.9 : 0.99; }
inline double elastic_rhs(double v, double sigma) { return v - (v > 0 ? sigma * v : 0.0); }
template <class RowsAt>
QpResult solve_qp_elastic(int n, const double* Hd, const double* gradf, std::vector<QpRow>& rows, RowsAt&& rows_at, double* sigma_out, int* attempt_out, QpResult* tried = nullptr) {
    QpResult qp;
    int attempt = 0;
    for (;; attempt++) {
        rows_at(elastic_sigma(attempt));
        qp = solve_qp(n, Hd, gradf, rows, slv::kQpMaxSteps, 2 * n);
        if (tried) tried[attempt] = qp;
        if (qp.feasible || attempt == kElasticAttempts - 1) break;
    }
    *sigma_out = elastic_sigma(attempt);
    *attempt_out = attempt;
    return qp;
}
inline void append_box_rows(int n, const double* xl, const double* xu, const double* x, std::vector<QpRow>& rows) {
    for (int j = 0; j < n; j++) {
        QpRow r; memset(&r, 0, sizeof(r)); r.a[j] = 1.0; r.b = xl[j] - x[j]; rows.push_back(r);
        QpRow r2; memset(&r2, 0, sizeof(r2)); r2.a[j] = -1.0; r2.b = -(xu[j] - x[j]); rows.push_back(r2);
    }
}

constexpr int kScanRowsPerBlock = 2048;

template <int MODE>
__global__ __launch_bounds__(256) void armour_solve_scan_kernel(slv::RowRule rule, const double* __restrict__ g_all, const double* __restrict__ jac_all,
                                                                const double* __restrict__ lo_all, const double* __restrict__ hi_all, int cap,
                                                                long long* __restrict__ viol_out, int* __restrict__ count_out, SolveRow* __restrict__ rows_out) {
    const int b = blockIdx.y, seg = blockIdx.x, nseg = gridDim.x, tid = threadIdx.x, lane = tid & 63, wv = tid >> 6;
    const int m = rule.m, n = rule.n;
    const double* g = g_all + (size_t)b * m;
    constexpr bool ROWS = MODE == 1;
    const double* jac = ROWS ? jac_all + (size_t)b * m * n : nullptr;
    const double* lo = lo_all + (size_t)b * m;
    const double* hi = hi_all + (size_t)b * m;
    SolveRow* rows = ROWS ? rows_out + ((size_t)b * nseg + seg) * cap : nullptr;
    const int row_end = min(m, (seg + 1) * kScanRowsPerBlock);
    __shared__ int wave_tot[4];
    __shared__ long long red[256];
    int base = 0, bad = 0;
    long long vsum = 0;
    for (int i0 = seg * kScanRowsPerBlock; i0 < row_end; i0 += 256) {
        const int i = i0 + tid;
        const bool in = i < row_end;
        const double gi = in ? g[i] : 0.0, li = in ? lo[i] : -1e300, ui = in ? hi[i] : 1e300;
        vsum += slv::row_violation(gi, li, ui);
        if (MODE == 2 && in && slv::outside_slack(rule, i, gi, li, ui)) bad++;
        if (ROWS) {
            double J[NV], l1 = 0.0;
#pragma unroll
            for (int j = 0; j < NV; j++) { J[j] = (in && j < n) ? jac[(size_t)i * n + j] : 0.0; l1 += fabs(J[j]); }
            const bool fh = in && slv::row_upper_candidate(gi, ui, l1);
            const bool fl = in && slv::row_lower_candidate(gi, li, l1);
            const unsigned long long bh = __ballot(fh), bl = __ballot(fl);
            const unsigned long long below = (1ull << lane) - 1ull;
            if (lane == 0) wave_tot[wv] = __popcll(bh) + __popcll(bl);
            __syncthreads();
            int pos = base + __popcll(bh & below) + __popcll(bl & below);
            for (int w2 = 0; w2 < wv; w2++) pos += wave_tot[w2];
            if (fh) {
                if (pos < cap) {
                    SolveRow r; r.idx = i; r.side = 0; r.v = gi - ui;
#pragma unroll
                    for (int j = 0; j < NV; j++) r.a[j] = -J[j];
                    rows[pos] = r;
                }
                pos++;
            }
            if (fl && pos < cap) {
                SolveRow r; r.idx = i; r.side = 1; r.v = li - gi;
#pragma unroll
                for (int j = 0; j < NV; j++) r.a[j] = J[j];
                rows[pos] = r;
            }
            base += wave_tot[0] + wave_tot[1] + wave_tot[2] + wave_tot[3];
            __syncthreads();
        }
    }
    red[tid] = vsum;
    __syncthreads();
    for (int s2 = 128; s2 > 0; s2 >>= 1) {
        if (tid < s2) red[tid] += red[tid + s2];
        __syncthreads();
    }
    if (MODE == 2) {
        __shared__ int bad_tot;
        if (tid == 0) bad_tot = 0;
        __syncthreads();
        if (bad) atomicAdd(&bad_tot, bad);
        __syncthreads();
        base = bad_tot;
    }
    if (tid == 0) { viol_out[(size_t)b * nseg + seg] = red[0]; if (MODE != 0) count_out[(size_t)b * nseg + seg] = base; }
}

}

extern "C" void armour_solve_options_default(ArmourSolveOptions* o) {
    memset(o, 0, sizeof(*o));
    o->max_iterations = 60;
    o->max_line_search = 12;
    o->tolerance = 1e-4;
    o->max_wall_time_s = 0.0;
}

extern "C" int armour_debug_qp(int32_t n, const double* Gd, const double* g0, int32_t m, const double* Amat, const double* lo,
                               const double* hi, double* x, int32_t* feasible) {
    if (n < 1 || n > NV || m < 0) { armour_set_error("armour_debug_qp: bad size"); return ARMOUR_EINVAL; }
    std::vector<QpRow> rows;
    for (int i = 0; i < m; i++) {
        if (hi[i] < 1e18) { QpRow r; for (int j = 0; j < n; j++) r.a[j] = -Amat[i * n + j]; r.b = -hi[i]; rows.push_back(r); }
        if (lo[i] > -1e18) { QpRow r; for (int j = 0; j < n; j++) r.a[j] = Amat[i * n + j]; r.b = lo[i]; rows.push_back(r); }
    }
    const QpResult q = solve_qp(n, Gd, g0, rows);
    for (int j = 0; j < n; j++) x[j] = q.x[j];
    *feasible = q.feasible ? 1 : 0;
    return ARMOUR_OK;
}

extern "C" int armour_debug_qp_box(int32_t n, const double* Gd, const double* g0, int32_t m, const double* Amat, const double* lo, const double* hi,
                                   const double* x_lo, const double* x_hi, int32_t first_try, double* x, int32_t* feasible, int32_t* steps, double* max_mult) {
    if (n < 1 || n > NV || m < 0 || !x_lo || !x_hi) { armour_set_error("armour_debug_qp_box: bad argument"); return ARMOUR_EINVAL; }
    std::vector<QpRow> rows;
    for (int i = 0; i < m; i++) {
        if (hi[i] < 1e18) { QpRow r; for (int j = 0; j < n; j++) r.a[j] = -Amat[i * n + j]; r.b = -hi[i]; rows.push_back(r); }
        if (lo[i] > -1e18) { QpRow r; for (int j = 0; j < n; j++) r.a[j] = Amat[i * n + j]; r.b = lo[i]; rows.push_back(r); }
    }
    for (int j = 0; j < n; j++) {
        QpRow r; memset(&r, 0, sizeof(r)); r.a[j] = 1.0; r.b = x_lo[j]; rows.push_back(r);
        QpRow r2; memset(&r2, 0, sizeof(r2)); r2.a[j] = -1.0; r2.b = -x_hi[j]; rows.push_back(r2);
    }
    const QpResult q = solve_qp(n, Gd, g0, rows, slv::kQpMaxSteps, first_try ? 2 * n : 0);
    for (int j = 0; j < n; j++) x[j] = q.x[j];
    *feasible = q.feasible ? 1 : 0;
    if (steps) *steps = q.iterations;
    if (max_mult) *max_mult = q.max_mult;
    return ARMOUR_OK;
}

static int check_posed_qp(const char* who, int32_t n, const double* Hd, const double* gradf, const double* x, int32_t ncand, const double* a, const double* v) {
    if (n < 1 || n > NV || ncand < 0 || ncand > 16384 || !Hd || !gradf || !x || (ncand > 0 && (!a || !v))) { armour_set_error("%s: bad argument (n = %d, ncand = %d)", who, n, ncand); return ARMOUR_EINVAL; }
    bool ok = finite_all(Hd, n) && finite_all(gradf, n) && finite_all(x, n) && finite_all(a, (size_t)ncand * n) && finite_all(v, ncand);
    for (int j = 0; j < n && ok; j++) ok = Hd[j] > 0;
    if (!ok) { armour_set_error("%s: non-finite input or Hd <= 0", who); return ARMOUR_EINVAL; }
    return ARMOUR_OK;
}

extern "C" int armour_debug_qp_elastic(int32_t n, const double* Hd, const double* gradf, const double* x, int32_t ncand, const double* a, const double* v,
                                       double* d, int32_t* feasible, int32_t* attempt, double* max_mult, int32_t* steps, int32_t* dropped,
                                       int32_t* dropped_mid, int32_t* excluded, int32_t* active) {
    ARMOUR_TRY(check_posed_qp("armour_debug_qp_elastic", n, Hd, gradf, x, ncand, a, v));
    if (!d || !feasible || !attempt) { armour_set_error("armour_debug_qp_elastic: null output"); return ARMOUR_EINVAL; }
    double xl[NV], xu[NV];
    for (int j = 0; j < NV; j++) { xl[j] = -1.0; xu[j] = 1.0; }
    std::vector<QpRow> rows;
    const auto rows_at = [&](double sigma) {
        rows.clear();
        for (int i = 0; i < ncand; i++) {
            QpRow r; for (int j = 0; j < n; j++) r.a[j] = a[(size_t)i * n + j];
            r.b = elastic_rhs(v[i], sigma); rows.push_back(r);
        }
        append_box_rows(n, xl, xu, x, rows);
    };
    QpResult tried[kElasticAttempts];
    double sigma = 0.0;
    int k = 0;
    const QpResult qp = solve_qp_elastic(n, Hd, gradf, rows, rows_at, &sigma, &k, tried);
    for (int j = 0; j < n; j++) d[j] = qp.x[j];
    *feasible = qp.feasible ? 1 : 0;
    *attempt = k;
    if (max_mult) *max_mult = qp.max_mult;
    for (int e = 0; e < kElasticAttempts; e++) {
        const bool ran = e <= k;
        if (steps) steps[e] = ran ? tried[e].iterations : -1;
        if (dropped) dropped[e] = ran ? tried[e].dropped : -1;
        if (dropped_mid) dropped_mid[e] = ran ? tried[e].dropped_mid : -1;
        if (excluded) excluded[e] = ran ? tried[e].excluded : -1;
        if (active) active[e] = ran ? tried[e].active : -1;
    }
    return ARMOUR_OK;
}

extern "C" int armour_debug_qp_device(int32_t n, const double* Hd, const double* gradf, const double* x, int32_t ncand, const double* a, const double* v,
                                      int32_t wps, int32_t lds_rows, double* d, int32_t* feasible, int32_t* attempt, double* max_mult, int32_t* qp_iter) {
    ARMOUR_TRY(check_posed_qp("armour_debug_qp_device", n, Hd, gradf, x, ncand, a, v));
    if (!d || !feasible || !attempt || (wps != 1 && wps != 2) || lds_rows < 0 || lds_rows > armour_qp_probe_lds_rows(wps)) {
        armour_set_error("armour_debug_qp_device: wps = %d (1, 2), lds_rows = %d (0..%d), or a null output", wps, lds_rows, armour_qp_probe_lds_rows(wps == 2 ? 2 : 1));
        return ARMOUR_EINVAL;
    }
    if (!armour_device_available()) { armour_set_error("armour_debug_qp_device: no HIP device visible (armour_debug_qp_elastic runs without one)"); return ARMOUR_EDEVICE; }
    QpProbe io;
    memset(&io, 0, sizeof(io));
    for (int j = 0; j < NV; j++) { io.x[j] = j < n ? x[j] : 0.0; io.gradf[j] = j < n ? gradf[j] : 0.0; io.Hd[j] = j < n ? Hd[j] : 1e-12; }
    io.ncand = ncand;
    std::vector<SolveRow> rows((size_t)ncand);
    for (int i = 0; i < ncand; i++) {
        SolveRow& r = rows[i];
        r.idx = i; r.side = 0; r.v = v[i];
        for (int j = 0; j < NV; j++) r.a[j] = j < n ? a[(size_t)i * n + j] : 0.0;
    }
    ARMOUR_TRY(armour_qp_probe(n, rows.data(), wps, lds_rows, &io));
    for (int j = 0; j < n; j++) d[j] = io.d[j];
    *feasible = io.feasible;
    *attempt = io.attempt;
    if (max_mult) *max_mult = io.max_mult;
    if (qp_iter) for (int e = 0; e < 4; e++) qp_iter[e] = e <= io.attempt ? io.qp_iter[e] : -1;
    return ARMOUR_OK;
}

enum class DeviceOutcome { Solved, HandBack };

struct DevicePlan {
    SolvePlan plan;
    bool culled = false;
    p2::SparseList sl = {nullptr, nullptr, nullptr, nullptr};
    const int* tq_tiles = nullptr; const int* tq_count = nullptr;
    int tq_cap = 0, n_tiles_culled = 0;
    int Bs = 0, n_launch = 0, nb = 0, tiles_per_block = 0, cap_blk = 0, cap_rows = 0;
};

static int plan_device_solve(ArmourPlanner* h, const P2Tables& tb, DevicePlan& p) {
    const int B = h->B, m = h->m;
    SolvePlan& plan = p.plan;
    int rc;
    const int cull_opt = h->tune(ARMOUR_OPT_SOLVE_CULL);
    constexpr long long kSolveCullMinRows = 150000;
    p.culled = h->Q > 0 && (cull_opt > 0 || (cull_opt < 0 && (long long)B * h->Q >= kSolveCullMinRows));
    if (p.culled) {
        if ((rc = armour_solver_lists(h, &p.sl, &p.tq_tiles, &p.tq_count, &p.tq_cap)) != ARMOUR_OK) return rc;
        for (int b = 0; b < B; b++) p.n_tiles_culled = std::max(p.n_tiles_culled, (h->rel2.h_tq_count[b] + P2_BLOCK - 1) / P2_BLOCK + (h->rel2.h_count[b] + P2_BLOCK - 1) / P2_BLOCK + 1);
    }
    if ((rc = armour_solve_device_capacity(tb, h->max_link, h->max_torque, h->h_plane_skip.data(), h->device, B, h->tune(ARMOUR_OPT_SOLVE_WAVES_PER_SIMD), &plan, p.n_tiles_culled)) != ARMOUR_OK) return rc;
    if (plan.capacity < 1) return ARMOUR_OK;
    const int sub_tiles = std::max(1, h->tune(ARMOUR_OPT_SOLVE_SUB_TILES));
    const int cut_tiles = std::max(1, h->tune(ARMOUR_OPT_SOLVE_CUT_TILES));
    int Bs = B;
    if (plan.capacity < B || (plan.n_tiles + std::max(1, plan.capacity / B) - 1) / std::max(1, plan.capacity / B) > cut_tiles) {
        const int nb_want = std::min(plan.n_tiles, (plan.n_tiles + sub_tiles - 1) / sub_tiles);
        Bs = std::max(1, std::min(B, plan.capacity / std::max(1, nb_want)));
        if ((rc = armour_solve_device_capacity(tb, h->max_link, h->max_torque, h->h_plane_skip.data(), h->device, Bs, h->tune(ARMOUR_OPT_SOLVE_WAVES_PER_SIMD), &plan, p.n_tiles_culled)) != ARMOUR_OK) return rc;
        Bs = std::max(1, std::min(Bs, plan.capacity));
    }
    int nb = std::min(std::min(plan.n_tiles, plan.capacity / Bs), 1024);
    if (h->tune(ARMOUR_OPT_SOLVE_BLOCKS) > 0) nb = std::max(1, std::min(nb, h->tune(ARMOUR_OPT_SOLVE_BLOCKS)));
    if (h->tune(ARMOUR_OPT_SOLVE_SUB_BATCH) > 0) Bs = std::max(1, std::min(Bs, h->tune(ARMOUR_OPT_SOLVE_SUB_BATCH)));
    p.Bs = Bs; p.nb = nb;
    p.n_launch = (B + Bs - 1) / Bs;
    p.tiles_per_block = (plan.n_tiles + nb - 1) / nb;
    p.cap_blk = std::min(2 * p.tiles_per_block * (p.culled ? P2_BLOCK : 64), 4096);
    p.cap_rows = std::min(2 * m, 16384);
    if (h->tune(ARMOUR_OPT_SOLVE_ROW_CAP) > 0) p.cap_blk = std::max(1, std::min(p.cap_blk, h->tune(ARMOUR_OPT_SOLVE_ROW_CAP)));
    return ARMOUR_OK;
}

struct DeviceStage {
    SolveArgs a;
    ArmourSolveResult* hres = nullptr;
    unsigned char* hblock = nullptr;
    long long* hstamps = nullptr;
    size_t off_args = 0, args_stride = 0, block_bytes = 0;
    double hard_s = 0;
};

static int stage_device_solve(ArmourPlanner* h, const ArmourSolveOptions& opt, const double* k_start, const P2Tables& tb, const DevicePlan& p, Clock::time_point t_begin, DeviceStage& s) {
    const int B = h->B, n = h->n, m = h->m;
    const SolvePlan& plan = p.plan;
    int rc;
    if ((rc = armour_upload_bounds(h)) != ARMOUR_OK) return rc;
    SolveDeviceWork& w = h->solve_dev;
    const size_t off_qdes = ((size_t)B * sizeof(SolveCtl) + 255) & ~(size_t)255;
    s.off_args = (off_qdes + (size_t)B * n * sizeof(double) + 255) & ~(size_t)255;
    s.args_stride = (sizeof(SolveArgs) + 255) & ~(size_t)255;
    s.block_bytes = s.off_args + (size_t)p.n_launch * s.args_stride;
    ARMOUR_TRY(w.ctl.reserve(s.block_bytes));
    bool fresh = false;
    ARMOUR_TRY(w.blk_word.reserve((size_t)p.Bs * p.nb * sizeof(BlockWord), &fresh));
    if (fresh || !w.words_clean) HIPCHK(hipMemsetAsync(w.blk_word, 0, w.blk_word.cap, h->stream));
    w.words_clean = 0;
    ARMOUR_TRY(w.blk_rows.reserve((size_t)p.Bs * p.nb * p.cap_blk * sizeof(SolveRow)));
    ARMOUR_TRY(w.qp_rows.reserve((size_t)p.Bs * p.cap_rows * sizeof(SolveRow)));
    ARMOUR_TRY(w.flags.reserve((size_t)p.Bs * 8 * (p.cap_rows + 2 * NV)));
    s.hres = reinterpret_cast<ArmourSolveResult*>(armour_handle_pinned(h, 1, (size_t)B * sizeof(ArmourSolveResult)));
    s.hblock = reinterpret_cast<unsigned char*>(armour_handle_pinned(h, 2, s.block_bytes));
    if (!s.hres || !s.hblock) return ARMOUR_EDEVICE;
    SolveCtl* hctl = reinterpret_cast<SolveCtl*>(s.hblock);
    memset(s.hres, 0, (size_t)B * sizeof(ArmourSolveResult));
    memset(hctl, 0, (size_t)B * sizeof(SolveCtl));
    for (int b = 0; b < B; b++) {
        hctl[b].go = 1; s.hres[b].status = -2;
        if (k_start) for (int j = 0; j < n; j++) hctl[b].x[j] = k_start[(size_t)b * n + j];
    }
    memcpy(s.hblock + off_qdes, h->h_qdes.data(), (size_t)B * n * sizeof(double));
    SolveArgs& a = s.a;
    memset(&a, 0, sizeof(a));
    a.tb = tb; a.lp = plan.lp; a.nb = p.nb; a.n_tiles = plan.n_tiles; a.cap_blk = p.cap_blk; a.cap_rows = p.cap_rows;
    a.lds_rows = (int)(plan.smem / ((NV + 1) * sizeof(double)));
    a.culled = p.culled ? 1 : 0; a.sl = p.sl; a.tq_tiles = p.tq_tiles; a.tq_count = p.tq_count; a.tq_cap = p.tq_cap;
    a.lo = h->d_bounds; a.hi = h->d_bounds + (size_t)B * m; a.g = h->d_g; a.jac = h->d_jac;
    a.ctl = w.ctl.as<SolveCtl>(); a.blk_word = w.blk_word.as<BlockWord>();
    a.blk_rows = w.blk_rows.as<SolveRow>(); a.qp_rows = w.qp_rows.as<SolveRow>(); a.flags = w.flags;
    a.q_des = reinterpret_cast<const double*>(w.ctl + off_qdes); a.out = s.hres;
    a.continuous_mask = h->continuous_mask();
    a.max_iter = opt.max_iterations; a.max_ls = opt.max_line_search; a.tol = opt.tolerance;
    const slv::RowRule rule = armour_row_rule(h);
    a.n_checked_collision = rule.n_checked; a.torque_slack = rule.torque_slack; a.collision_slack = rule.collision_slack;
    a.t_plan = h->params.t_plan; a.cost_scale = h->params.cost_scale;
    a.budget_ticks = -1;
    if (opt.max_wall_time_s > 0) {
        const double left_ms = (opt.max_wall_time_s - std::chrono::duration<double>(Clock::now() - t_begin).count()) * 1e3 / p.n_launch;
        a.budget_ticks = left_ms > 0 ? (long long)(left_ms * plan.ticks_per_ms) : 0;
    }
    const double hard_cap_s = h->tune_f(ARMOUR_OPT_SOLVE_HARD_CAP_S);
    const double no_budget_s = std::max(5.0, 1.0 + 50.0 * (double)std::max(1, opt.max_iterations) * (1.0 + std::max(0, opt.max_line_search)) * p.tiles_per_block * 4e-6);
    s.hard_s = hard_cap_s > 0 ? hard_cap_s : (a.budget_ticks >= 0 ? a.budget_ticks / plan.ticks_per_ms * 1e-3 + 1.0 : no_budget_s);
    a.hard_ticks = std::max<long long>(1, (long long)(s.hard_s * 1e3 * plan.ticks_per_ms));
    const bool timing = armour_trace_solve();
    s.hstamps = timing ? reinterpret_cast<long long*>(armour_handle_pinned(h, 0, (size_t)B * 64 * sizeof(long long) + (size_t)B * n * sizeof(double))) : nullptr;
    if (s.hstamps) memset(s.hstamps, 0, (size_t)B * 64 * sizeof(long long));
    a.stamps = s.hstamps;
    return ARMOUR_OK;
}

static void report_device_timing(const ArmourPlanner* h, const DevicePlan& p, const DeviceStage& s, double ms, Clock::time_point t_begin, Clock::time_point t_launch) {
    const SolvePlan& plan = p.plan;
    const ArmourSolveResult* hres = s.hres;
    const long long* hstamps = s.hstamps;
    const int B = h->B, n_launch = p.n_launch, Bs = p.Bs, nb = p.nb, n_tiles_culled = p.n_tiles_culled;
    if (p.culled) fprintf(stderr, "[armour_solve, device form] culled: at most %d listed tiles per problem (problem 0: %d of %d collision rows, %d of %d torque rows), lists %.3f + %.3f ms\n",
                          n_tiles_culled, h->rel2.h_count[0], h->Q, h->rel2.h_tq_count[0], h->row0, h->rel.ms, h->rel2.ms);
    fprintf(stderr, "[armour_solve, device form] B=%d in %d launch(es) of <= %d problems: %d blocks per problem (%d tiles), %.3f ms wall (%.3f ms before the launch), kernel %.3f ms (problem 0); phases of problem 0 in us (barrier passed / leader done):", B, n_launch, Bs, nb, plan.n_tiles, ms,
            std::chrono::duration<double, std::milli>(t_launch - t_begin).count(), hres[0].time_ms / plan.ticks_per_ms);
    int bs = 0;
    for (int b = 1; b < B; b++) if (hres[b].time_ms > hres[bs].time_ms) bs = b;
    for (int which = 0; which < 2; which++) {
        const int b = which == 0 ? 0 : bs;
        const long long* st = hstamps + (size_t)b * 64;
        if (which == 1) fprintf(stderr, "\n   slowest problem %d: kernel %.3f ms, %d iterations, %d evaluations, status %d, %lld QP solves with %lld steps in all; phases in us:", b, hres[b].time_ms / plan.ticks_per_ms,
                                hres[b].iterations, hres[b].evaluations, hres[b].status, st[43], st[42]);
        for (int i = 0; i < 32 && (i < 2 || st[i]); i++) fprintf(stderr, " %.1f", st[i] / plan.ticks_per_ms * 1e3);
        fprintf(stderr, " | first leader step: bookkeeping %.1f, candidates gathered %.1f, QP done %.1f us (%lld QP steps, %lld candidate rows)", st[32] / plan.ticks_per_ms * 1e3,
                st[33] / plan.ticks_per_ms * 1e3, st[34] / plan.ticks_per_ms * 1e3, st[40], st[41]);
        fprintf(stderr, " | QP steps by attempt (sigma 0, 0.5, 0.9, 0.99), all solves: %lld %lld %lld %lld", st[44], st[45], st[46], st[47]);
        fprintf(stderr, " | attempt 0, all steps, us: row search %.1f, entering row %.1f, M + rhs %.1f, factor + solves %.1f, z + step lengths %.1f, update %.1f",
                st[50] / plan.ticks_per_ms * 1e3, st[51] / plan.ticks_per_ms * 1e3, st[52] / plan.ticks_per_ms * 1e3, st[53] / plan.ticks_per_ms * 1e3, st[54] / plan.ticks_per_ms * 1e3, st[55] / plan.ticks_per_ms * 1e3);
    }
    long long longest_ok = 0, long_bad = 0, steps_all = 0;
    for (int b = 0; b < B; b++) { const long long* st = hstamps + (size_t)b * 64; longest_ok = std::max(longest_ok, st[48]); long_bad += st[49]; steps_all += st[44] + st[45] + st[46] + st[47]; }
    fprintf(stderr, "\n   all problems: %lld QP steps; longest attempt that ended feasible %lld steps; attempts of more than 60 steps that ended infeasible: %lld\n", steps_all, longest_ok, long_bad);
}

static int solve_on_device(ArmourPlanner* h, const ArmourSolveOptions& opt, const double* k_start, ArmourSolveResult* results, Clock::time_point t_begin, DeviceOutcome* out) {
    *out = DeviceOutcome::HandBack;
    const P2Tables tb = armour_make_tables(h);
    DevicePlan p;
    DeviceStage s;
    int rc;
    if ((rc = plan_device_solve(h, tb, p)) != ARMOUR_OK || p.plan.capacity < 1) return rc;
    if ((rc = stage_device_solve(h, opt, k_start, tb, p, t_begin, s)) != ARMOUR_OK) return rc;
    SolveDeviceWork& w = h->solve_dev;
    const int B = h->B, n_launch = p.n_launch;
    const auto t_launch = Clock::now();
    for (int li = 0; li < n_launch; li++) { s.a.b0 = li * p.Bs; memcpy(s.hblock + s.off_args + (size_t)li * s.args_stride, &s.a, sizeof(SolveArgs)); }
    HIPCHK(hipMemcpyAsync(w.ctl, s.hblock, s.block_bytes, hipMemcpyHostToDevice, h->stream));
    for (int li = 0; li < n_launch; li++)
        if ((rc = armour_solve_device_launch(reinterpret_cast<const SolveArgs*>(w.ctl + s.off_args + (size_t)li * s.args_stride), p.nb, p.plan,
                                             std::min(p.Bs, B - li * p.Bs), h->stream)) != ARMOUR_OK) return rc;
    for (unsigned long long polls = 0;; polls++) {
        const hipError_t q = hipStreamQuery(h->stream);
        if (q == hipSuccess) break;
        if (q != hipErrorNotReady) { armour_set_error("armour_solve (device form): %s", hipGetErrorString(q)); return ARMOUR_EDEVICE; }
        if ((polls & 0xfffull) == 0xfffull && std::chrono::duration<double>(Clock::now() - t_launch).count() > n_launch * (2.0 * s.hard_s + 5.0)) {
            armour_set_error("armour_solve (device form): the persistent kernel did not finish within %.1f s", n_launch * (2.0 * s.hard_s + 5.0));
            return ARMOUR_EDEVICE;
        }
    }
    w.words_clean = 1;
    for (int b = 0; b < B; b++)
        if (s.hres[b].status < 0) { w.words_clean = 0; return ARMOUR_OK; }
    const double ms = std::chrono::duration<double, std::milli>(Clock::now() - t_begin).count();
    if (s.hstamps) report_device_timing(h, p, s, ms, t_begin, t_launch);
    for (int b = 0; b < B; b++) { results[b] = s.hres[b]; results[b].time_ms = ms; }
    *out = DeviceOutcome::Solved;
    return ARMOUR_OK;
}

enum class Scan { Violation = 0, Rows = 1, Verdict = 2 };

struct ProblemState {
    double x[NV] = {}, f, gradf[NV], viol, mu = 1.0;
    int iters = 0, evals = 0, status = 0;
    bool done = false;
    bool searching = false;
    double d[NV], alpha, phi0, dphi;
};

struct HostSolve {
    ArmourPlanner* h;
    ArmourSolveOptions opt;
    int B, n, m, nseg, cap_rows;
    double* hk; long long* hviol_seg; int* hcount; SolveRow* hrows;
    double *hg = nullptr, *hj = nullptr;
    bool full_on_host = false;
    std::vector<double> xl, xu, Hd;
    std::vector<double> viol, f, gradf;
    std::vector<ProblemState> st;
    double t_eval = 0, t_qp = 0;
};

static int setup_host_solve(ArmourPlanner* h, const ArmourSolveOptions& opt, const double* k_start, HostSolve& s) {
    const int B = h->B, n = h->n, m = h->m;
    int rc;
    s.h = h; s.opt = opt; s.B = B; s.n = n; s.m = m;
    s.hk = armour_handle_pinned(h, 0, (size_t)B * n * sizeof(double));
    if (!s.hk) return ARMOUR_EDEVICE;
    s.xl.resize(n); s.xu.resize(n);
    if ((rc = armour_upload_bounds(h)) != ARMOUR_OK) return rc;
    if (!h->bounds_on_host) {
        h->h_gl.resize((size_t)B * m); h->h_gu.resize((size_t)B * m);
        if ((rc = armour_get_bounds(h, s.xl.data(), s.xu.data(), h->h_gl.data(), h->h_gu.data())) != ARMOUR_OK) return rc;
        h->bounds_on_host = true;
    } else if ((rc = armour_get_bounds(h, s.xl.data(), s.xu.data(), nullptr, nullptr)) != ARMOUR_OK) return rc;
    s.nseg = (m + kScanRowsPerBlock - 1) / kScanRowsPerBlock;
    s.cap_rows = (int)std::max<size_t>(64, std::min<size_t>(2 * kScanRowsPerBlock, ((size_t)128 << 20) / ((size_t)B * s.nseg * sizeof(SolveRow))));
    if (h->tune(ARMOUR_OPT_SOLVE_ROW_CAP) > 0) s.cap_rows = std::max(1, h->tune(ARMOUR_OPT_SOLVE_ROW_CAP));
    s.hviol_seg = reinterpret_cast<long long*>(armour_handle_pinned(h, 3, (size_t)B * s.nseg * sizeof(long long)));
    s.hcount = reinterpret_cast<int*>(armour_handle_pinned(h, 4, (size_t)B * s.nseg * sizeof(int)));
    s.hrows = reinterpret_cast<SolveRow*>(armour_handle_pinned(h, 5, (size_t)B * s.nseg * s.cap_rows * sizeof(SolveRow)));
    if (!s.hviol_seg || !s.hcount || !s.hrows) return ARMOUR_EDEVICE;
    s.viol.resize(B); s.f.resize(B); s.gradf.resize((size_t)B * n);
    s.Hd.assign((size_t)B * NV, 1e-12);
    for (int b = 0; b < B; b++)
        for (int j = 0; j < n; j++) {
            const size_t ix = (size_t)b * n + j;
            const double dk = slv::plan_dk(h->mode, h->mode == ARMOUR_MODE_ARMTD ? h->h_krange[ix] : 0.0, h->params.k_range[j], h->params.t_plan);
            s.Hd[(size_t)b * NV + j] = slv::hess_diag(h->params.cost_scale, dk);
        }
    s.st.assign(B, ProblemState());
    std::fill(s.hk, s.hk + (size_t)B * n, 0.0);
    if (k_start)
        for (int b = 0; b < B; b++) for (int j = 0; j < n; j++) s.hk[(size_t)b * n + j] = s.st[b].x[j] = k_start[(size_t)b * n + j];
    return ARMOUR_OK;
}

static int evaluate(HostSolve& s, Scan mode) {
    const auto e0 = Clock::now();
    struct Acc { double& t; decltype(e0) s; ~Acc() { t += std::chrono::duration<double, std::milli>(Clock::now() - s).count(); } } acc{s.t_eval, e0};
    ArmourPlanner* h = s.h;
    const int B = s.B, n = s.n, m = s.m, nseg = s.nseg;
    const size_t bm = (size_t)B * m;
    const bool rows = mode == Scan::Rows;
    int r = armour_eval_g_jac_device(h, s.hk, h->d_g, rows ? h->d_jac : nullptr, h->stream);
    if (r != ARMOUR_OK) return r;
    const auto scan = mode == Scan::Violation ? armour_solve_scan_kernel<0> : rows ? armour_solve_scan_kernel<1> : armour_solve_scan_kernel<2>;
    hipLaunchKernelGGL(scan, dim3(nseg, B), dim3(256), 0, h->stream, armour_row_rule(h), h->d_g, rows ? h->d_jac : nullptr,
                       h->d_bounds, h->d_bounds + bm, s.cap_rows, s.hviol_seg, mode == Scan::Violation ? nullptr : s.hcount, rows ? s.hrows : nullptr);
    HIPCHK(hipGetLastError());
    if ((r = armour_spin_on_stream(h->stream)) != ARMOUR_OK) return r;
    for (int b = 0; b < B; b++) {
        long long v = 0;
        for (int sg = 0; sg < nseg; sg++) v += s.hviol_seg[(size_t)b * nseg + sg];
        s.viol[b] = slv::viol_from_fixed(v);
    }
    s.full_on_host = false;
    if (!rows) return ARMOUR_OK;
    bool overflow = false;
    for (size_t i = 0; i < (size_t)B * nseg; i++) overflow = overflow || s.hcount[i] > s.cap_rows;
    if (overflow) {
        s.hg = armour_handle_pinned(h, 1, bm * sizeof(double));
        s.hj = armour_handle_pinned(h, 2, bm * n * sizeof(double));
        if (!s.hg || !s.hj) return ARMOUR_EDEVICE;
        HIPCHK(hipMemcpyAsync(s.hg, h->d_g, bm * sizeof(double), hipMemcpyDeviceToHost, h->stream));
        HIPCHK(hipMemcpyAsync(s.hj, h->d_jac, bm * n * sizeof(double), hipMemcpyDeviceToHost, h->stream));
        if ((r = armour_spin_on_stream(h->stream)) != ARMOUR_OK) return r;
        s.full_on_host = true;
    }
    return ARMOUR_OK;
}

static void gather_rows(const HostSolve& s, int b, double sigma, std::vector<QpRow>& rows) {
    const int n = s.n, m = s.m, nseg = s.nseg;
    const auto elastic = [sigma](double v) { return elastic_rhs(v, sigma); };
    rows.clear();
    if (!s.full_on_host) {
        for (int sg = 0; sg < nseg; sg++) {
            const SolveRow* cr = s.hrows + ((size_t)b * nseg + sg) * s.cap_rows;
            for (int r0 = 0; r0 < s.hcount[(size_t)b * nseg + sg]; r0++) {
                QpRow r; for (int j = 0; j < n; j++) r.a[j] = cr[r0].a[j];
                r.b = elastic(cr[r0].v); rows.push_back(r);
            }
        }
    } else {
        const double* g = s.hg + (size_t)b * m;
        const double* J = s.hj + (size_t)b * m * n;
        const double* lo = s.h->h_gl.data() + (size_t)b * m;
        const double* hi = s.h->h_gu.data() + (size_t)b * m;
        for (int i = 0; i < m; i++) {
            const double* Ji = J + (size_t)i * n;
            double l1 = 0;
            for (int j = 0; j < n; j++) l1 += std::fabs(Ji[j]);
            if (slv::row_upper_candidate(g[i], hi[i], l1)) { QpRow r; for (int j = 0; j < n; j++) r.a[j] = -Ji[j]; r.b = elastic(g[i] - hi[i]); rows.push_back(r); }
            if (slv::row_lower_candidate(g[i], lo[i], l1)) { QpRow r; for (int j = 0; j < n; j++) r.a[j] = Ji[j]; r.b = elastic(lo[i] - g[i]); rows.push_back(r); }
        }
    }
    append_box_rows(n, s.xl.data(), s.xu.data(), s.st[b].x, rows);
}

static void qp_step(HostSolve& s, int it, int b0, int b1) {
    const int n = s.n;
    const ArmourSolveOptions& opt = s.opt;
    std::vector<QpRow> rows;
    for (int b = b0; b < b1; b++) {
        ProblemState& p = s.st[b];
        if (p.done) continue;
        double sigma = 0.0;
        int attempt = 0;
        const QpResult qp = solve_qp_elastic(n, &s.Hd[(size_t)b * NV], p.gradf, rows, [&](double sg) { gather_rows(s, b, sg, rows); }, &sigma, &attempt);
        if (armour_trace_solve() && s.B == 1) {
            fprintf(stderr, "[armour_solve, host form] iteration %d: QP %s at sigma %.2f after %d steps, %zu rows; x =", it, qp.feasible ? "feasible" : "INFEASIBLE", sigma, qp.iterations, rows.size());
            for (int j = 0; j < n; j++) fprintf(stderr, " %.6g", p.x[j]);
            fprintf(stderr, "; d =");
            for (int j = 0; j < n; j++) fprintf(stderr, " %.6g", qp.x[j]);
            fprintf(stderr, "; viol %.6g\n", p.viol);
        }
        if (!qp.feasible) { p.done = true; p.status = 3; continue; }
        double dn = 0, gd = 0;
        for (int j = 0; j < n; j++) { p.d[j] = qp.x[j]; dn = std::fmax(dn, std::fabs(qp.x[j])); gd += p.gradf[j] * qp.x[j]; }
        if (dn <= opt.tolerance * 1e-2 || (dn <= opt.tolerance && p.viol <= opt.tolerance)) { p.done = true; p.status = 1; continue; }
        p.mu = std::fmax(p.mu, 1.5 * qp.max_mult + 1e-3);
        p.phi0 = p.f + p.mu * p.viol;
        p.dphi = gd - p.mu * (1.0 - sigma) * p.viol;
        if (p.dphi > -1e-14) p.dphi = -1e-14;
        p.alpha = 1.0;
        p.searching = true;
    }
}

static int line_search(HostSolve& s, bool* linearised) {
    const int B = s.B, n = s.n, max_ls = s.opt.max_line_search;
    int rc;
    *linearised = false;
    for (int ls = 0; ls <= max_ls; ls++) {
        bool need = false;
        for (int b = 0; b < B; b++) {
            const ProblemState& p = s.st[b];
            for (int j = 0; j < n; j++) s.hk[b * n + j] = p.x[j] + (p.searching ? p.alpha * p.d[j] : 0.0);
            need = need || p.searching;
        }
        if (!need) break;
        const bool speculative = ls == 0;
        if ((rc = evaluate(s, speculative ? Scan::Rows : Scan::Violation)) != ARMOUR_OK) return rc;
        if (speculative) *linearised = true;
        if ((rc = armour_eval_f(s.h, s.hk, s.f.data())) != ARMOUR_OK) return rc;
        for (int b = 0; b < B; b++) {
            ProblemState& p = s.st[b];
            if (!p.searching) continue;
            p.evals++;
            const double v = s.viol[b];
            const double phi = s.f[b] + p.mu * v;
            if (phi <= p.phi0 + 1e-4 * p.alpha * p.dphi || ls == max_ls) {
                if (ls == max_ls && phi > p.phi0) { p.done = true; p.status = 4; p.searching = false; continue; }
                for (int j = 0; j < n; j++) p.x[j] = s.hk[b * n + j];
                p.f = s.f[b]; p.viol = v; p.searching = false; p.iters++;
            } else {
                p.alpha *= 0.5;
                *linearised = false;
            }
        }
    }
    return ARMOUR_OK;
}

static int finish_host_solve(HostSolve& s, ArmourSolveResult* results, Clock::time_point t_begin) {
    const int B = s.B, n = s.n, nseg = s.nseg;
    int rc;
    for (int b = 0; b < B; b++) for (int j = 0; j < n; j++) s.hk[b * n + j] = s.st[b].x[j];
    if ((rc = evaluate(s, Scan::Verdict)) != ARMOUR_OK) return rc;
    if ((rc = armour_eval_f(s.h, s.hk, s.f.data())) != ARMOUR_OK) return rc;
    const double ms = std::chrono::duration<double, std::milli>(Clock::now() - t_begin).count();
    if (armour_trace_solve()) fprintf(stderr, "[armour_solve] B=%d total %.3f ms: evaluations+scan %.3f ms, QP %.3f ms, rows of problem 0, segment 0: %d (cap %d, %d segments)\n", B, ms, s.t_eval, s.t_qp, s.hcount[0], s.cap_rows, nseg);
    for (int b = 0; b < B; b++) {
        int bad = 0;
        for (int sg = 0; sg < nseg; sg++) bad += s.hcount[(size_t)b * nseg + sg];
        ArmourSolveResult& r = results[b];
        memset(&r, 0, sizeof(r));
        for (int j = 0; j < n; j++) r.k_opt[j] = s.st[b].x[j];
        r.cost = s.f[b];
        r.max_violation = s.viol[b];
        r.feasible = bad == 0 ? 1 : 0;
        r.iterations = s.st[b].iters;
        r.evaluations = s.st[b].evals + 1;
        r.status = s.st[b].done ? s.st[b].status : 2;
        r.time_ms = ms;
    }
    return ARMOUR_OK;
}

static int solve_on_host(ArmourPlanner* h, const ArmourSolveOptions& opt, const double* k_start, ArmourSolveResult* results, Clock::time_point t_begin) {
    HostSolve s;
    int rc;
    if ((rc = setup_host_solve(h, opt, k_start, s)) != ARMOUR_OK) return rc;
    const int B = s.B, n = s.n;
    if ((rc = evaluate(s, Scan::Rows)) != ARMOUR_OK) return rc;
    if ((rc = armour_eval_f(h, s.hk, s.f.data())) != ARMOUR_OK) return rc;
    if ((rc = armour_eval_grad_f(h, s.hk, s.gradf.data())) != ARMOUR_OK) return rc;
    for (int b = 0; b < B; b++) {
        s.st[b].f = s.f[b];
        for (int j = 0; j < n; j++) s.st[b].gradf[j] = s.gradf[(size_t)b * n + j];
        s.st[b].viol = s.viol[b];
        s.st[b].evals = 1;
    }
    const unsigned nthreads = std::max(1u, std::min(std::thread::hardware_concurrency(), (unsigned)B / 32u));
    for (int it = 0; it < opt.max_iterations; it++) {
        bool any = false;
        for (int b = 0; b < B; b++) any = any || !s.st[b].done;
        if (!any) break;
        if (opt.max_wall_time_s > 0 && std::chrono::duration<double>(Clock::now() - t_begin).count() >= opt.max_wall_time_s) {
            for (int b = 0; b < B; b++) if (!s.st[b].done) { s.st[b].done = true; s.st[b].status = 5; }
            break;
        }
        for (int b = 0; b < B; b++) s.st[b].searching = false;
        const auto q0 = Clock::now();
        if (nthreads <= 1) qp_step(s, it, 0, B);
        else {
            std::vector<std::thread> th;
            const int per = (B + (int)nthreads - 1) / (int)nthreads;
            for (unsigned tI = 0; tI < nthreads; tI++) { const int b0 = (int)tI * per, b1 = std::min(B, b0 + per); if (b0 < b1) th.emplace_back(qp_step, std::ref(s), it, b0, b1); }
            for (auto& t : th) t.join();
        }
        s.t_qp += std::chrono::duration<double, std::milli>(Clock::now() - q0).count();
        bool linearised = false;
        if ((rc = line_search(s, &linearised)) != ARMOUR_OK) return rc;
        for (int b = 0; b < B; b++) for (int j = 0; j < n; j++) s.hk[b * n + j] = s.st[b].x[j];
        if (!linearised && (rc = evaluate(s, Scan::Rows)) != ARMOUR_OK) return rc;
        if ((rc = armour_eval_grad_f(h, s.hk, s.gradf.data())) != ARMOUR_OK) return rc;
        for (int b = 0; b < B; b++) {
            if (s.st[b].done) continue;
            s.st[b].evals++;
            for (int j = 0; j < n; j++) s.st[b].gradf[j] = s.gradf[(size_t)b * n + j];
            s.st[b].viol = s.viol[b];
        }
    }
    return finish_host_solve(s, results, t_begin);
}

extern "C" int armour_solve(ArmourPlanner* h, const ArmourSolveOptions* opt_in, ArmourSolveResult* results) { return armour_solve_from(h, opt_in, nullptr, results); }

extern "C" int armour_solve_from(ArmourPlanner* h, const ArmourSolveOptions* opt_in, const double* k_start, ArmourSolveResult* results) {
    if (!results) { armour_set_error("null argument"); return ARMOUR_EINVAL; }
    NEED_READY(h);
    if (k_start)
        for (size_t i = 0; i < (size_t)h->B * h->n; i++)
            if (!(std::fabs(k_start[i]) <= 1.0)) { armour_set_error("armour_solve_from: k_start[%zu] = %g is outside [-1, 1]", i, k_start[i]); return ARMOUR_EINVAL; }
    ArmourSolveOptions opt;
    if (opt_in) opt = *opt_in; else armour_solve_options_default(&opt);
    const auto t_begin = Clock::now();
    const int dev_env = h->tune(ARMOUR_OPT_SOLVE_DEVICE);
    const bool want_device = opt.force_host_qp > 0.0 ? false : opt.force_host_qp < 0.0 ? true : dev_env != 0;
    HIPCHK(hipSetDevice(h->device));
    if (want_device) {
        DeviceOutcome out;
        const int rc = solve_on_device(h, opt, k_start, results, t_begin, &out);
        if (rc != ARMOUR_OK || out == DeviceOutcome::Solved) return rc;
    }
    return solve_on_host(h, opt, k_start, results, t_begin);
}
```

armour_amd/csrc/solver_device.h:

```cpp
#pragma once
#include "common.h"
#include "p2_tiles.h"
#include "p2_sparse.h"
#include "solver_common.h"

struct alignas(128) SolveCtl {
    unsigned go;
    int pad0;
    double x[slv::NV];
};
struct alignas(64) BlockWord {
    unsigned flag;
    int count;
    int bad;
    int pad0;
    long long viol;
};

struct SolveArgs {
    P2Tables tb;
    p2::P2Launch lp;
    int nb, n_tiles;
    int culled;
    p2::SparseList sl;
    const int* tq_tiles; const int* tq_count; int tq_cap;
    int b0;
    int cap_blk, cap_rows;
    int lds_rows;
    const double* lo; const double* hi;
    double* g; double* jac;
    SolveCtl* ctl;
    BlockWord* blk_word;
    slv::SolveRow* blk_rows;
    slv::SolveRow* qp_rows;
    unsigned char* flags;
    const double* q_des;
    ArmourSolveResult* out;
    int continuous_mask;
    int max_iter, max_ls;
    int n_checked_collision;
    double t_plan, cost_scale, tol, torque_slack, collision_slack;
    long long budget_ticks;
    long long hard_ticks;
    long long* stamps;
};

struct SolvePlan {
    p2::P2Launch lp;
    size_t smem;
    bool six;
    int n_tiles;
    int capacity;
    double ticks_per_ms;
    const void* fn;
};

int armour_p2_plan(const P2Tables& tb, int max_link, int max_torque, const unsigned long long* h_skip, int steps, long long k_stride,
                   long long g_stride, long long j_stride, p2::P2Launch* lp_out, size_t* smem_out, bool* dfc_out, bool* six_out, bool* exact_out);
int armour_solve_device_capacity(const P2Tables& tb, int max_link, int max_torque, const unsigned long long* h_skip, int device, int b_launch, int waves_per_simd, SolvePlan* plan,
                                 int n_tiles_override = 0);
int armour_solver_lists(ArmourPlanner* h, p2::SparseList* sl, const int** tq_tiles, const int** tq_count, int* tq_cap);
int armour_solve_device_launch(const SolveArgs* d_args, int nb, const SolvePlan& plan, int B, hipStream_t stream);

struct QpProbe {
    double x[slv::NV], gradf[slv::NV], Hd[slv::NV];
    int ncand, pad0;
    double d[slv::NV], max_mult;
    int feasible, attempt, qp_iter[4];
};
int armour_qp_probe_lds_rows(int wps);
int armour_qp_probe(int n, const slv::SolveRow* rows, int wps, int lds_rows, QpProbe* io);
```

armour_amd/csrc/solver_device.hip:

```cpp
#include <algorithm>
#include <atomic>
#include <cmath>
#include <cstring>

#include "bezier.h"
#include "cacc.h"
#include "common.h"
#include "p2_tiles.h"
#include "solver_common.h"
#include "solver_device.h"

using namespace p2;
using namespace slv;

namespace {

enum { CMD_EVAL = 1, CMD_DONE = 4 };
enum { ST_AFTER_FIRST = 0, ST_AFTER_TRIAL = 1, ST_AFTER_RELIN = 2, ST_AFTER_VERDICT = 3 };
constexpr double kInf = 1e300;
#define WAVE_LDS_SYNC() do { __builtin_amdgcn_fence(__ATOMIC_SEQ_CST, "wavefront"); __builtin_amdgcn_wave_barrier(); } while (0)

__device__ inline unsigned ld_coh(const unsigned* p) { return __hip_atomic_load(p, __ATOMIC_RELAXED, __HIP_MEMORY_SCOPE_AGENT); }
__device__ inline int ld_coh(const int* p) { return __hip_atomic_load(p, __ATOMIC_RELAXED, __HIP_MEMORY_SCOPE_AGENT); }
__device__ inline long long ld_coh(const long long* p) { return __hip_atomic_load(p, __ATOMIC_RELAXED, __HIP_MEMORY_SCOPE_AGENT); }
__device__ inline double ld_coh(const double* p) { return __longlong_as_double(__hip_atomic_load(reinterpret_cast<const long long*>(p), __ATOMIC_RELAXED, __HIP_MEMORY_SCOPE_AGENT)); }
__device__ inline void st_coh(unsigned* p, unsigned v) { __hip_atomic_store(p, v, __ATOMIC_RELAXED, __HIP_MEMORY_SCOPE_AGENT); }
__device__ inline void st_coh(int* p, int v) { __hip_atomic_store(p, v, __ATOMIC_RELAXED, __HIP_MEMORY_SCOPE_AGENT); }
__device__ inline void st_coh(long long* p, long long v) { __hip_atomic_store(p, v, __ATOMIC_RELAXED, __HIP_MEMORY_SCOPE_AGENT); }
__device__ inline void st_coh(double* p, double v) { __hip_atomic_store(reinterpret_cast<long long*>(p), __double_as_longlong(v), __ATOMIC_RELAXED, __HIP_MEMORY_SCOPE_AGENT); }
__device__ inline void wait_my_memory_ops() { asm volatile("s_waitcnt vmcnt(0) lgkmcnt(0)" ::: "memory"); }
__device__ inline void st_coh_row(SolveRow* dst, const SolveRow& r) {
    long long* d = reinterpret_cast<long long*>(dst);
    st_coh(d, ((long long)(unsigned)r.side << 32) | (unsigned)r.idx);
    st_coh(reinterpret_cast<double*>(d + 1), r.v);
#pragma unroll
    for (int j = 0; j < NV; j++) st_coh(reinterpret_cast<double*>(d + 2 + j), r.a[j]);
}
__device__ inline SolveRow ld_coh_row(const SolveRow* src) {
    const long long* d = reinterpret_cast<const long long*>(src);
    SolveRow r;
    const long long w0 = ld_coh(d);
    r.idx = (int)(unsigned)(w0 & 0xffffffffll); r.side = (int)(w0 >> 32);
    r.v = ld_coh(reinterpret_cast<const double*>(d + 1));
#pragma unroll
    for (int j = 0; j < NV; j++) r.a[j] = ld_coh(reinterpret_cast<const double*>(d + 2 + j));
    return r;
}

__device__ inline void tile_info(const SolveArgs& a, int t, int& role, int& r0, int& r1) {
    const int nbt = a.lp.nbt, nbc = a.lp.nbc, row0 = a.tb.row0;
    if (t < nbt) { role = nbc + t; r0 = t * P2_TQ_ROWS; r1 = min(row0, r0 + P2_TQ_ROWS); }
    else if (t < nbt + nbc) { role = t - nbt; r0 = row0 + (t - nbt) * P2_ROWS; r1 = min(row0 + a.tb.Q, r0 + P2_ROWS); }
    else { role = nbc + nbt; r0 = row0 + a.tb.Q; r1 = a.tb.m; }
}

__device__ inline double plan_point(const SolveArgs& a, const double* bz, int i, double k) {
    const int n = a.tb.n;
    return a.tb.mode == ARMOUR_MODE_ARMTD ? cacc::q_plan(bz[i], bz[n + i], bz[2 * n + i], k)
                                          : bez::q_des(bz[i], bz[n + i], bz[2 * n + i], a.tb.k_range[i] * k, a.t_plan);
}
__device__ inline double cost_sum(const SolveArgs& a, const double* sq) {
    double obj = 0;
    for (int pass = 0; pass < 2; pass++)
        for (int i = 0; i < a.tb.n; i++)
            if ((((a.continuous_mask >> i) & 1) != 0) == (pass == 0)) obj += sq[i];
    return obj * a.cost_scale;
}
__device__ inline double plan_dk(const SolveArgs& a, const double* bz, int i) {
    const double tp = a.t_plan;
    return a.tb.mode == ARMOUR_MODE_ARMTD ? cacc::q_plan_dk(bz[2 * a.tb.n + i]) : (tp * tp * tp) * (6 * tp * tp - 15 * tp + 10) * a.tb.k_range[i];
}
__device__ inline void block_sum(long long& v, int& i, long long* sh4, int* si4) {
#pragma unroll
    for (int off = 32; off > 0; off >>= 1) { v += __shfl_xor(v, off, 64); i += __shfl_xor(i, off, 64); }
    __syncthreads();
    if ((threadIdx.x & 63) == 0) { sh4[threadIdx.x >> 6] = v; si4[threadIdx.x >> 6] = i; }
    __syncthreads();
    v = sh4[0] + sh4[1] + sh4[2] + sh4[3];
    i = si4[0] + si4[1] + si4[2] + si4[3];
}
__device__ inline int block_exclusive_scan(int v, int* si4, int& total) {
    const int lane = threadIdx.x & 63, wv = threadIdx.x >> 6;
    int inc = v;
#pragma unroll
    for (int off = 1; off < 64; off <<= 1) { const int o = __shfl_up(inc, off, 64); if (lane >= off) inc += o; }
    __syncthreads();
    if (lane == 63) si4[wv] = inc;
    __syncthreads();
    int base = 0;
#pragma unroll
    for (int w = 0; w < 4; w++) if (w < wv) base += si4[w];
    total = si4[0] + si4[1] + si4[2] + si4[3];
    return base + inc - v;
}

struct ScanShared {
    int wave_tot[4];
    long long red[256];
    int redi[256];
};
template <int MODE>
__device__ inline void scan_rows(const SolveArgs& a, int b, int r0, int r1, SolveRow* __restrict__ rows, int cap, ScanShared& sh,
                                 long long& viol_out, int& count_out, int& bad_out) {
    const int n = a.tb.n, m = a.tb.m, tid = threadIdx.x, lane = tid & 63, wv = tid >> 6;
    const double* g = a.g + (size_t)b * m;
    const double* jac = a.jac + (size_t)b * m * n;
    const double* lo = a.lo + (size_t)b * m;
    const double* hi = a.hi + (size_t)b * m;
    const int n_unchecked = a.tb.Q - a.n_checked_collision;
    int base = 0, bad = 0;
    long long vsum = 0;
    for (int i0 = r0; i0 < r1; i0 += 256) {
        const int i = i0 + tid;
        const bool in = i < r1;
        const double gi = in ? g[i] : 0.0, li = in ? lo[i] : -1e300, ui = in ? hi[i] : 1e300;
        vsum += row_violation(gi, li, ui);
        if ((MODE & 2) && in) {
            const int ic = i - a.tb.row0 - a.n_checked_collision;
            const double slack = i < a.tb.row0 ? a.torque_slack : ic < 0 ? a.collision_slack : 0.0;
            if ((ic < 0 || ic >= n_unchecked) && (gi < li - slack || gi > ui + slack)) bad++;
        }
        if (MODE & 1) {
            double J[NV], l1 = 0.0;
#pragma unroll
            for (int j = 0; j < NV; j++) { J[j] = (in && j < n) ? jac[(size_t)i * n + j] : 0.0; l1 += fabs(J[j]); }
            const bool fh = in && row_upper_candidate(gi, ui, l1);
            const bool fl = in && row_lower_candidate(gi, li, l1);
            const unsigned long long bh = __ballot(fh), bl = __ballot(fl);
            const unsigned long long below = (1ull << lane) - 1ull;
            if (lane == 0) sh.wave_tot[wv] = __popcll(bh) + __popcll(bl);
            __syncthreads();
            int pos = base + __popcll(bh & below) + __popcll(bl & below);
            for (int w2 = 0; w2 < wv; w2++) pos += sh.wave_tot[w2];
            if (fh) {
                if (pos < cap) {
                    SolveRow r; r.idx = i; r.side = 0; r.v = gi - ui;
#pragma unroll
                    for (int j = 0; j < NV; j++) r.a[j] = -J[j];
                    st_coh_row(rows + pos, r);
                }
                pos++;
            }
            if (fl && pos < cap) {
                SolveRow r; r.idx = i; r.side = 1; r.v = li - gi;
#pragma unroll
                for (int j = 0; j < NV; j++) r.a[j] = J[j];
                st_coh_row(rows + pos, r);
            }
            base += sh.wave_tot[0] + sh.wave_tot[1] + sh.wave_tot[2] + sh.wave_tot[3];
            __syncthreads();
        }
    }
    block_sum(vsum, bad, sh.red, sh.redi);
    viol_out = vsum;
    bad_out = bad;
    count_out = base;
    __syncthreads();
}

struct TileSet { int ntq, nsp, cnt2, cntq; };
__device__ inline TileSet problem_tiles(const SolveArgs& a, int b) {
    TileSet ts;
    ts.cntq = a.tq_count[b]; ts.ntq = (ts.cntq + P2_BLOCK - 1) / P2_BLOCK;
    ts.cnt2 = a.sl.count[b]; ts.nsp = (ts.cnt2 + P2_BLOCK - 1) / P2_BLOCK;
    return ts;
}
__device__ inline int tile_row(const SolveArgs& a, int b, const TileSet& ts, int t, int tid) {
    if (t < ts.ntq) {
        const int i = t * P2_BLOCK + tid;
        return i < ts.cntq ? a.tq_tiles[(size_t)b * a.tq_cap + i] : -1;
    }
    if (t < ts.ntq + ts.nsp) {
        const int i = (t - ts.ntq) * P2_BLOCK + tid;
        return i < ts.cnt2 ? a.tb.row0 + a.sl.rows[(size_t)b * a.tb.Q + i] : -1;
    }
    const int r = a.tb.row0 + a.tb.Q + tid;
    return r < a.tb.m ? r : -1;
}
__device__ inline void scan_tiles(const SolveArgs& a, int b, const TileSet& ts, int t0, int t1, SolveRow* __restrict__ rows, int cap, ScanShared& sh,
                                  long long& viol_out, int& count_out, int& bad_out) {
    const int n = a.tb.n, m = a.tb.m, tid = threadIdx.x, lane = tid & 63, wv = tid >> 6;
    const double* g = a.g + (size_t)b * m;
    const double* jac = a.jac + (size_t)b * m * n;
    const double* lo = a.lo + (size_t)b * m;
    const double* hi = a.hi + (size_t)b * m;
    const int n_unchecked = a.tb.Q - a.n_checked_collision;
    int base = 0, bad = 0;
    long long vsum = 0;
    for (int t = t0; t < t1; t++) {
        const int i = tile_row(a, b, ts, t, tid);
        const bool in = i >= 0;
        const double gi = in ? g[i] : 0.0, li = in ? lo[i] : -1e300, ui = in ? hi[i] : 1e300;
        vsum += row_violation(gi, li, ui);
        if (in) {
            const int ic = i - a.tb.row0 - a.n_checked_collision;
            const double slack = i < a.tb.row0 ? a.torque_slack : ic < 0 ? a.collision_slack : 0.0;
            if ((ic < 0 || ic >= n_unchecked) && (gi < li - slack || gi > ui + slack)) bad++;
        }
        double J[NV], l1 = 0.0;
#pragma unroll
        for (int j = 0; j < NV; j++) { J[j] = (in && j < n) ? jac[(size_t)i * n + j] : 0.0; l1 += fabs(J[j]); }
        const bool fh = in && row_upper_candidate(gi, ui, l1);
        const bool fl = in && row_lower_candidate(gi, li, l1);
        const unsigned long long bh = __ballot(fh), bl = __ballot(fl);
        const unsigned long long below = (1ull << lane) - 1ull;
        if (lane == 0) sh.wave_tot[wv] = __popcll(bh) + __popcll(bl);
        __syncthreads();
        int pos = base + __popcll(bh & below) + __popcll(bl & below);
        for (int w2 = 0; w2 < wv; w2++) pos += sh.wave_tot[w2];
        if (fh) {
            if (pos < cap) {
                SolveRow r; r.idx = i; r.side = 0; r.v = gi - ui;
#pragma unroll
                for (int j = 0; j < NV; j++) r.a[j] = -J[j];
                st_coh_row(rows + pos, r);
            }
            pos++;
        }
        if (fl && pos < cap) {
            SolveRow r; r.idx = i; r.side = 1; r.v = li - gi;
#pragma unroll
            for (int j = 0; j < NV; j++) r.a[j] = J[j];
            st_coh_row(rows + pos, r);
        }
        base += sh.wave_tot[0] + sh.wave_tot[1] + sh.wave_tot[2] + sh.wave_tot[3];
        __syncthreads();
    }
    block_sum(vsum, bad, sh.red, sh.redi);
    viol_out = vsum;
    bad_out = bad;
    count_out = base;
    __syncthreads();
}

constexpr int kFlagsInLds = 1024;
struct Leader {
    double x[NV], d[NV], xt[NV], gradf[NV], Hd[NV];
    double f, viol, mu, alpha, phi0, dphi;
    int it, ls, iters, evals, status, stage, ncand, bad;
    long long t_start;
    double bz[3 * NV], qdes[NV];
    double qx[NV], u[NV + 1], An[NV][NV], np[NV];
    double M[NV * NV], Lc[NV][NV], Lci[NV], invHd[NV], rhs[NV], r[NV], z[NV];
    double bp, up, max_mult, sigma;
    int A[NV], q, p, qp_iter, feasible, stop, added, chol_rows;
    unsigned char act[kFlagsInLds], exc[kFlagsInLds];
    double rs[256];
    int ri[256];
    int scan[1024];
};

__device__ inline int ld_lds_int(const int* p) { return *reinterpret_cast<const volatile int*>(p); }
struct QpWave {
    double qx[NV], An[NV][NV], np[NV], M[NV * NV], Lc[NV][NV], Lci[NV], rhs[NV];
    double bp, max_mult;
    int A[NV], q, qp_iter, feasible;
    unsigned char act[kFlagsInLds], exc[kFlagsInLds];
};
struct QpShared {
    QpWave w[4];
    int first_ok;
};
__device__ inline double attempt_sigma(int attempt) { return attempt == 0 ? 0.0 : attempt == 1 ? 0.5 : attempt == 2 ? 0.9 : 0.99; }
__device__ inline void qp_row_s(const SolveArgs& a, const Leader& L, const SolveRow* cand, int i, double sigma, double* arow, double& brow) {
    if (i < L.ncand) {
        const SolveRow& r = cand[i];
#pragma unroll
        for (int j = 0; j < NV; j++) arow[j] = r.a[j];
        const double v = r.v;
        brow = v - (v > 0 ? sigma * v : 0.0);
    } else {
        const int e = i - L.ncand, j = e >> 1;
        const double sg = (e & 1) == 0 ? 1.0 : -1.0;
#pragma unroll
        for (int jj = 0; jj < NV; jj++) arow[jj] = jj == j ? sg : 0.0;
        brow = (e & 1) == 0 ? -1.0 - L.x[j] : -(1.0 - L.x[j]);
    }
}
__device__ inline double readlane_f64(double v, int src_lane) {
    return __hiloint2double(__builtin_amdgcn_readlane(__double2hiint(v), src_lane), __builtin_amdgcn_readlane(__double2loint(v), src_lane));
}
template <int CTRL, int ROW_MASK>
__device__ inline void min_pair_dpp(double& best, int& bi) {
    const int hi = __double2hiint(best), lo = __double2loint(best);
    const int ohi = __builtin_amdgcn_update_dpp(hi, hi, CTRL, ROW_MASK, 0xf, false);
    const int olo = __builtin_amdgcn_update_dpp(lo, lo, CTRL, ROW_MASK, 0xf, false);
    const int oi = __builtin_amdgcn_update_dpp(bi, bi, CTRL, ROW_MASK, 0xf, false);
    const double o = __hiloint2double(ohi, olo);
    if (oi >= 0 && (bi < 0 || o < best || (o == best && oi < bi))) { best = o; bi = oi; }
}
__device__ inline int wave_argmin_first(double best, int bi) {
    min_pair_dpp<0x111, 0xf>(best, bi);
    min_pair_dpp<0x112, 0xf>(best, bi);
    min_pair_dpp<0x114, 0xf>(best, bi);
    min_pair_dpp<0x118, 0xf>(best, bi);
    min_pair_dpp<0x142, 0xa>(best, bi);
    min_pair_dpp<0x143, 0xc>(best, bi);
    return __builtin_amdgcn_readlane(bi, 63);
}

template <int WPS>
__device__ __forceinline__ void solve_qp_wave(const SolveArgs& a, const Leader& L, QpShared& S, const SolveRow* cand, const double* lds_rows, unsigned char* flags_g, int max_iter = kQpMaxSteps) {
    constexpr int kRegRows = WPS == 1 ? 4 : 2;
    const int n = a.tb.n, lane = threadIdx.x & 63, attempt = threadIdx.x >> 6;
    QpWave& W = S.w[attempt];
    const double sigma = attempt_sigma(attempt);
    const int mrows = L.ncand + 2 * n;
    unsigned char* is_active = mrows <= kFlagsInLds ? W.act : flags_g + (size_t)(2 * attempt) * (a.cap_rows + 2 * NV);
    unsigned char* excluded = mrows <= kFlagsInLds ? W.exc : flags_g + (size_t)(2 * attempt + 1) * (a.cap_rows + 2 * NV);
    for (int i = lane; i < mrows; i += 64) { is_active[i] = 0; excluded[i] = 0; }
    const bool reg_rows = mrows <= 64 * kRegRows;
    auto load_row = [&](int i, double* arow, double& brow) {
        if (lds_rows && i < L.ncand) {
#pragma unroll
            for (int j = 0; j < NV; j++) arow[j] = lds_rows[(size_t)j * a.lds_rows + i];
            const double v = lds_rows[(size_t)NV * a.lds_rows + i];
            brow = v - (v > 0 ? sigma * v : 0.0);
        } else qp_row_s(a, L, cand, i, sigma, arow, brow);
    };
    double my_a[kRegRows][NV], my_b[kRegRows];
#pragma unroll
    for (int r = 0; r < kRegRows; r++) {
        my_b[r] = 0.0;
#pragma unroll
        for (int j = 0; j < NV; j++) my_a[r][j] = 0.0;
        if (reg_rows && lane + 64 * r < mrows) load_row(lane + 64 * r, my_a[r], my_b[r]);
    }
    double qx[NV], u[NV + 1], ih[NV];
#pragma unroll
    for (int j = 0; j < NV; j++) { ih[j] = L.invHd[j]; qx[j] = j < n ? -L.gradf[j] * ih[j] : 0.0; u[j] = 0.0; }
    u[NV] = 0.0;
    int q = 0, cv = 0, qp_iter = 0;
    bool feasible = true, stop = false;
    unsigned act_bits = 0, exc_bits = 0;
    long long* qst = a.stamps && attempt == 0 ? a.stamps + (size_t)(blockIdx.x / a.nb + a.b0) * 64 + 50 : nullptr;
    long long q_t = qst ? wall_clock64() : 0;
#define QPW_LAP(slot) if (qst && lane == 0) { const long long n__ = wall_clock64(); qst[slot] += n__ - q_t; q_t = n__; }
    WAVE_LDS_SYNC();
    {
        double lo[NV], hi[NV], hd[NV], g0[NV], d[NV];
#pragma unroll
        for (int j = 0; j < NV; j++) { lo[j] = -1.0 - L.x[j]; hi[j] = 1.0 - L.x[j]; hd[j] = L.Hd[j]; g0[j] = L.gradf[j]; d[j] = 0.0; }
        const double mmc = box_clipped_step(n, hd, ih, g0, lo, hi, d);
        int viol = 0;
        for (int i = lane; i < mrows; i += 64) {
            double ar[NV], br;
            load_row(i, ar, br);
            double s = -br;
#pragma unroll
            for (int j = 0; j < NV; j++) if (j < n) s += ar[j] * d[j];
            if (s < -1e-7) viol = 1;
        }
        if (__ballot(viol != 0) == 0ull) {
            if (lane == 0) {
                W.q = 0; W.qp_iter = 0; W.feasible = 1; W.max_mult = mmc;
                atomicMin(&S.first_ok, attempt);
            }
#pragma unroll
            for (int j = 0; j < NV; j++) if (lane == j) W.qx[j] = d[j];
            return;
        }
    }
    while (!stop) {
        if (ld_lds_int(&S.first_ok) < attempt) { feasible = false; break; }
        double best = -1e-10;
        int bi = -1;
        if (reg_rows) {
#pragma unroll
            for (int r = 0; r < kRegRows; r++) {
                const int i = lane + 64 * r;
                if (i < mrows && !(((act_bits | exc_bits) >> r) & 1u)) {
                    double s = -my_b[r];
#pragma unroll
                    for (int j = 0; j < NV; j++) if (j < n) s += my_a[r][j] * qx[j];
                    if (s < best) { best = s; bi = i; }
                }
            }
        } else {
            for (int i0 = lane; i0 < mrows; i0 += 4 * 64) {
                double ar[4][NV], br[4];
#pragma unroll
                for (int e = 0; e < 4; e++) load_row(min(i0 + 64 * e, mrows - 1), ar[e], br[e]);
#pragma unroll
                for (int e = 0; e < 4; e++) {
                    const int i = i0 + 64 * e;
                    if (i < mrows && !is_active[i] && !excluded[i]) {
                        double s = -br[e];
#pragma unroll
                        for (int j = 0; j < NV; j++) if (j < n) s += ar[e][j] * qx[j];
                        if (s < best) { best = s; bi = i; }
                    }
                }
            }
        }
        const int p = wave_argmin_first(best, bi);
        QPW_LAP(0)
        if (p < 0) break;
        if (++qp_iter > max_iter) { feasible = false; break; }
        double npr[NV], bp;
        if (reg_rows) {
            const int slot = p >> 6, src = p & 63;
            double v[NV + 1];
#pragma unroll
            for (int j = 0; j <= NV; j++) v[j] = 0.0;
#pragma unroll
            for (int r = 0; r < kRegRows; r++) {
                if (slot == r) {
#pragma unroll
                    for (int j = 0; j < NV; j++) v[j] = my_a[r][j];
                    v[NV] = my_b[r];
                }
            }
#pragma unroll
            for (int j = 0; j < NV; j++) npr[j] = readlane_f64(v[j], src);
            bp = readlane_f64(v[NV], src);
        } else {
            load_row(p, npr, bp);
        }
        if (lane < NV) W.np[lane] = 0.0;
#pragma unroll
        for (int j = 0; j < NV; j++) if (lane == j) W.np[j] = npr[j];
        double up = 0.0;
        bool added = false;
        QPW_LAP(1)
        for (int guard = 0; guard < 4 * NV + 8 && !added; guard++) {
            double rr[NV];
#pragma unroll
            for (int i = 0; i < NV; i++) rr[i] = 0.0;
            WAVE_LDS_SYNC();
            if (q > 0) {
                constexpr bool kRhsOwnLanes = NV * NV + NV <= 64;
                static_assert(NV * NV <= 64, "solve_qp_wave: one lane per entry of M");
                if (lane < NV * NV) {
                    const int i = lane / NV, k = lane - i * NV;
                    if (i < q && k <= i) {
                        double s = 0;
#pragma unroll
                        for (int j = 0; j < NV; j++) if (j < n) s += W.An[i][j] * W.An[k][j] * ih[j];
                        W.M[i * NV + k] = s; W.M[k * NV + i] = s;
                    }
                } else if (kRhsOwnLanes && lane < NV * NV + NV) {
                    const int i = lane - NV * NV;
                    if (i < q) {
                        double s = 0;
#pragma unroll
                        for (int j = 0; j < NV; j++) if (j < n) s += W.An[i][j] * npr[j] * ih[j];
                        W.rhs[i] = s;
                    }
                }
                if constexpr (!kRhsOwnLanes) {
                    if (lane < NV && lane < q) {
                        const int i = lane;
                        double s = 0;
#pragma unroll
                        for (int j = 0; j < NV; j++) if (j < n) s += W.An[i][j] * npr[j] * ih[j];
                        W.rhs[i] = s;
                    }
                }
                WAVE_LDS_SYNC();
                QPW_LAP(2)
                double Lr[NV][NV], Li[NV];
#pragma unroll
                for (int i = 0; i < NV; i++) {
                    Li[i] = i < cv ? W.Lci[i] : 0.0;
#pragma unroll
                    for (int k = 0; k <= i; k++) Lr[i][k] = i < cv ? W.Lc[i][k] : 0.0;
                }
                bool spd = true;
#pragma unroll
                for (int i = 0; i < NV; i++) {
                    if (i >= cv && i < q && spd) {
#pragma unroll
                        for (int jj = 0; jj <= i; jj++) {
                            if (spd) {
                                double s = W.M[i * NV + jj];
#pragma unroll
                                for (int k = 0; k < jj; k++) s -= Lr[i][k] * Lr[jj][k];
                                if (jj == i) {
                                    if (s <= 1e-14 * fabs(W.M[i * NV + i]) || s <= 0) spd = false;
                                    else { Lr[i][i] = sqrt(s); Li[i] = 1.0 / Lr[i][i]; }
                                } else {
                                    Lr[i][jj] = s * Li[jj];
                                }
                            }
                        }
                        if (spd) {
#pragma unroll
                            for (int k = 0; k <= i; k++) W.Lc[i][k] = Lr[i][k];
                            W.Lci[i] = Li[i];
                            cv = i + 1;
                        }
                    }
                }
                if (!spd) {
                    if (reg_rows) { if (lane == (p & 63)) exc_bits |= 1u << (p >> 6); }
                    else if (lane == 0) excluded[p] = 1;
                    break;
                }
                double tt[NV];
#pragma unroll
                for (int i = 0; i < NV; i++) {
                    tt[i] = 0.0;
                    if (i < q) {
                        double s = W.rhs[i];
#pragma unroll
                        for (int k = 0; k < i; k++) s -= Lr[i][k] * tt[k];
                        tt[i] = s * Li[i];
                    }
                }
#pragma unroll
                for (int i = NV - 1; i >= 0; i--) {
                    if (i < q) {
                        double s = tt[i];
#pragma unroll
                        for (int k = i + 1; k < NV; k++) if (k < q) s -= Lr[k][i] * rr[k];
                        rr[i] = s * Li[i];
                    }
                }
            }
            QPW_LAP(3)
            double zmine = 0.0;
            {
                const int j = lane < NV ? lane : 0;
                double s = 0.0;
#pragma unroll
                for (int jj = 0; jj < NV; jj++) if (jj == j) s = npr[jj];
#pragma unroll
                for (int i = 0; i < NV; i++) if (i < q) s -= W.An[i][j] * rr[i];
                double ihj = 0.0;
#pragma unroll
                for (int jj = 0; jj < NV; jj++) if (jj == j) ihj = ih[jj];
                zmine = s * ihj;
            }
            double z[NV];
#pragma unroll
            for (int j = 0; j < NV; j++) z[j] = j < n ? readlane_f64(zmine, j) : 0.0;
            double zz = 0, znp = 0;
#pragma unroll
            for (int j = 0; j < NV; j++) if (j < n) { zz += z[j] * z[j]; znp += z[j] * npr[j]; }
            double t1 = kInf;
            int l = -1;
#pragma unroll
            for (int i = 0; i < NV; i++)
                if (i < q && rr[i] > 1e-14) { const double ur = u[i] / rr[i]; if (ur < t1) { t1 = ur; l = i; } }
            double sp = -bp;
#pragma unroll
            for (int j = 0; j < NV; j++) if (j < n) sp += npr[j] * qx[j];
            double t2 = kInf;
            if (zz > 1e-24 && znp > 1e-16) t2 = -sp / znp;
            if (t2 < 0) t2 = 0;
            const double t = t1 < t2 ? t1 : t2;
            if (t >= kInf) { feasible = false; break; }
            QPW_LAP(4)
            const bool dual_only = t2 >= kInf;
            if (!dual_only) {
#pragma unroll
                for (int j = 0; j < NV; j++) if (j < n) qx[j] += t * z[j];
            }
#pragma unroll
            for (int i = 0; i < NV; i++) if (i < q) u[i] -= t * rr[i];
            up += t;
            if (!dual_only && t == t2) {
                if (q >= n) { feasible = false; break; }
#pragma unroll
                for (int i = 0; i < NV; i++) if (i == q) u[i] = up;
                if (lane < NV) W.An[q][lane] = W.np[lane];
                if (lane == 0) W.A[q] = p;
                if (reg_rows) { if (lane == (p & 63)) act_bits |= 1u << (p >> 6); }
                else if (lane == 0) is_active[p] = 1;
                q++;
                added = true;
            } else {
                {
                    const int d = ld_lds_int(&W.A[l]);
                    if (reg_rows) { if (lane == (d & 63)) act_bits &= ~(1u << (d >> 6)); }
                    else if (lane == 0) is_active[d] = 0;
                }
                WAVE_LDS_SYNC();
                for (int i = l; i < q - 1; i++) {
                    if (lane < NV) W.An[i][lane] = W.An[i + 1][lane];
                    if (lane == 0) W.A[i] = W.A[i + 1];
                    WAVE_LDS_SYNC();
                }
#pragma unroll
                for (int i = 0; i < NV; i++) if (i >= l && i < q - 1) u[i] = u[i + 1];
                q--;
                if (cv > l) cv = l;
            }
        }
        QPW_LAP(5)
        if (!feasible) break;
        WAVE_LDS_SYNC();
        if (!added) {
            if (reg_rows) { if (lane == (p & 63)) exc_bits |= 1u << (p >> 6); }
            else if (!excluded[p]) { WAVE_LDS_SYNC(); if (lane == 0) excluded[p] = 1; }
        }
        WAVE_LDS_SYNC();
    }
    if (feasible) {
        int viol = 0;
        for (int i = lane; i < mrows; i += 64) {
            double ar[NV], br;
            load_row(i, ar, br);
            double s = -br;
#pragma unroll
            for (int j = 0; j < NV; j++) if (j < n) s += ar[j] * qx[j];
            if (s < -1e-7) viol = 1;
        }
        if (__ballot(viol != 0) != 0ull) feasible = false;
    }
    double mm = 0.0;
#pragma unroll
    for (int i = 0; i < NV; i++) if (i < q && u[i] > mm) mm = u[i];
    if (lane == 0) {
        W.q = q; W.qp_iter = qp_iter; W.feasible = feasible ? 1 : 0; W.max_mult = mm;
        if (feasible) atomicMin(&S.first_ok, attempt);
    }
#pragma unroll
    for (int j = 0; j < NV; j++) if (lane == j) W.qx[j] = qx[j];
}

__device__ inline bool gather_candidates(const SolveArgs& a, Leader& L, int b, SolveRow* cand) {
    const int tid = threadIdx.x, nb = a.nb;
    const BlockWord* bw = a.blk_word + (size_t)(b - a.b0) * nb;
    int mine[4], tot = 0;
#pragma unroll
    for (int e = 0; e < 4; e++) { const int jb = tid * 4 + e; mine[e] = jb < nb ? ld_coh(&bw[jb].count) : 0; tot += mine[e]; }
    int total;
    int run = block_exclusive_scan(tot, L.ri, total);
#pragma unroll
    for (int e = 0; e < 4; e++) { L.scan[tid * 4 + e] = run; run += mine[e]; }
    bool ok = total <= a.cap_rows;
#pragma unroll
    for (int e = 0; e < 4; e++) if (tid * 4 + e < nb && mine[e] > a.cap_blk) ok = false;
    const bool overflow = __syncthreads_or(ok ? 0 : 1) != 0;
    if (overflow) return false;
    for (int c = tid; c < total; c += 256) {
        int lo = 0, hi = nb - 1;
        while (lo < hi) {
            const int mid = (lo + hi + 1) >> 1;
            if (L.scan[mid] <= c) lo = mid; else hi = mid - 1;
        }
        cand[c] = ld_coh_row(a.blk_rows + ((size_t)(b - a.b0) * nb + lo) * a.cap_blk + (c - L.scan[lo]));
    }
    if (tid == 0) L.ncand = total;
    __threadfence_block();
    __syncthreads();
    return true;
}

template <int WPS>
__device__ __forceinline__ int leader_step(const SolveArgs& a, Leader& L, QpShared& QS, int b, long long viol_fx, int bad, SolveRow* cand,
                                  unsigned char* flags_g, double* x_pub, double* lds_stage) {
    const int n = a.tb.n, tid = threadIdx.x;
    const double viol = viol_from_fixed(viol_fx);
#define LSTAMP(k) do { if (a.stamps && tid == 0 && first) a.stamps[(size_t)b * 64 + 32 + (k)] = wall_clock64() - L.t_start; } while (0)
    const bool first = L.stage == ST_AFTER_FIRST;
    const double* pt = first ? L.x : L.xt;
    if (tid < n) {
        const bool cont = (a.continuous_mask >> tid) & 1;
        const double qp = plan_point(a, L.bz, tid, pt[tid]);
        const double eg = cont ? wrap_to_pi(qp - L.qdes[tid]) : (qp - L.qdes[tid]);
        L.np[tid] = 2 * eg * plan_dk(a, L.bz, tid) * a.cost_scale;
        const double e = cont ? wrap_to_pi(L.qdes[tid] - qp) : (L.qdes[tid] - qp);
        L.z[tid] = e * e;
    }
    __syncthreads();
    if (tid == 0) {
        const double fpt = cost_sum(a, L.z);
        L.stop = 0;
        if (first) {
            L.f = fpt; L.evals = 1; L.viol = viol; L.bad = bad; L.status = 0;
            for (int j = 0; j < n; j++) L.gradf[j] = L.np[j];
        } else {
            L.evals++;
            const double phi = fpt + L.mu * viol;
            if (phi <= L.phi0 + 1e-4 * L.alpha * L.dphi || L.ls == a.max_ls) {
                if (L.ls == a.max_ls && phi > L.phi0) { L.status = 4; L.stop = 1; }
                else {
                    for (int j = 0; j < n; j++) { L.x[j] = L.xt[j]; L.gradf[j] = L.np[j]; }
                    L.f = fpt; L.viol = viol; L.bad = bad; L.iters++; L.it++;
                    L.evals++;
                }
            } else {
                L.alpha *= 0.5;
                L.ls++;
                for (int j = 0; j < n; j++) L.xt[j] = L.x[j] + L.alpha * L.d[j];
                L.stop = 3;
            }
        }
        L.stage = ST_AFTER_TRIAL;
        if (L.stop == 0) {
            if (L.it >= a.max_iter) { L.status = 2; L.stop = 1; }
            else if (a.budget_ticks >= 0 && wall_clock64() - L.t_start >= a.budget_ticks) { L.status = 5; L.stop = 1; }
        }
    }
    __syncthreads();
    LSTAMP(0);
    if (L.stop == 0) {
        bool finish = false;
        if (!gather_candidates(a, L, b, cand)) {
            if (tid == 0) L.status = -1;
            finish = true;
        }
        if (!finish) {
            LSTAMP(1);
            if (tid == 0) {
                QS.first_ok = 4;
                for (int j = 0; j < NV; j++) L.invHd[j] = 1.0 / L.Hd[j];
            }
            const double* staged = nullptr;
            if (L.ncand > 64 * (WPS == 1 ? 4 : 2) - 2 * n && L.ncand <= a.lds_rows) {
                for (int i = tid; i < L.ncand; i += 256) {
                    const SolveRow& r = cand[i];
#pragma unroll
                    for (int j = 0; j < NV; j++) lds_stage[(size_t)j * a.lds_rows + i] = r.a[j];
                    lds_stage[(size_t)NV * a.lds_rows + i] = r.v;
                }
                staged = lds_stage;
            }
            __syncthreads();
            solve_qp_wave<WPS>(a, L, QS, cand, staged, flags_g);
            __syncthreads();
            if (tid == 0) {
                int k = 0;
                while (k < 3 && !QS.w[k].feasible) k++;
                const QpWave& W = QS.w[k];
                for (int j = 0; j < NV; j++) L.qx[j] = W.qx[j];
                L.max_mult = W.max_mult; L.feasible = W.feasible; L.sigma = attempt_sigma(k); L.qp_iter = W.qp_iter;
                if (a.stamps) {
                    for (int e = 0; e < 4; e++) {
                        a.stamps[(size_t)b * 64 + 44 + e] += QS.w[e].qp_iter;
                        if (QS.w[e].feasible && QS.w[e].qp_iter > a.stamps[(size_t)b * 64 + 48]) a.stamps[(size_t)b * 64 + 48] = QS.w[e].qp_iter;
                        if (QS.w[e].qp_iter > 60 && !QS.w[e].feasible) a.stamps[(size_t)b * 64 + 49] += 1;
                    }
                }
            }
            __syncthreads();
            LSTAMP(2);
            if (tid == 0 && a.stamps) { if (L.it == 0) { a.stamps[(size_t)b * 64 + 40] = L.qp_iter; a.stamps[(size_t)b * 64 + 41] = L.ncand; } a.stamps[(size_t)b * 64 + 42] += L.qp_iter; a.stamps[(size_t)b * 64 + 43] += 1; }
            if (tid == 0) {
                if (!L.feasible) { L.status = 3; L.stop = 1; }
                else {
                    double dn = 0, gd = 0;
                    for (int j = 0; j < n; j++) { L.d[j] = L.qx[j]; dn = fmax(dn, fabs(L.qx[j])); gd += L.gradf[j] * L.qx[j]; }
                    if (dn <= a.tol * 1e-2 || (dn <= a.tol && L.viol <= a.tol)) { L.status = 1; L.stop = 1; }
                    else {
                        L.mu = fmax(L.mu, 1.5 * L.max_mult + 1e-3);
                        L.phi0 = L.f + L.mu * L.viol;
                        L.dphi = gd - L.mu * (1.0 - L.sigma) * L.viol;
                        if (L.dphi > -1e-14) L.dphi = -1e-14;
                        L.alpha = 1.0;
                        L.ls = 0;
                        for (int j = 0; j < n; j++) L.xt[j] = L.x[j] + L.alpha * L.d[j];
                        L.stop = 3;
                    }
                }
            }
        }
        __syncthreads();
        if (finish && tid == 0) L.stop = 1;
        __syncthreads();
    }
    int next;
    if (L.stop == 3) {
        const int outside = a.culled && tid < n && !(fabs(L.xt[tid]) <= 1.0 + 1e-6) ? 1 : 0;
        if (__syncthreads_or(outside)) {
            if (tid == 0) a.out[b].status = -1;
            __syncthreads();
            return CMD_DONE;
        }
        if (tid < n) st_coh(x_pub + tid, L.xt[tid]);
        next = CMD_EVAL;
    } else {
        if (tid == 0) {
            ArmourSolveResult& r = a.out[b];
            if (L.status == -1) r.status = -1;
            else {
                for (int j = 0; j < NV; j++) r.k_opt[j] = j < n ? L.x[j] : 0.0;
                r.cost = L.f;
                r.max_violation = L.viol;
                r.feasible = L.bad == 0 ? 1 : 0;
                r.iterations = L.iters;
                r.evaluations = L.evals + 1;
                r.status = L.status;
                r.time_ms = (double)(wall_clock64() - L.t_start);
            }
        }
        next = CMD_DONE;
    }
    __syncthreads();
    return next;
}

template <bool LL, int PPW, int WPS>
__global__ __launch_bounds__(P2_BLOCK) __attribute__((amdgpu_waves_per_eu(WPS, WPS))) void armour_solve_kernel(const SolveArgs* __restrict__ args) {
    const SolveArgs& a = *args;
    extern __shared__ __attribute__((aligned(16))) unsigned char smem_raw[];
    __shared__ ScanShared scan_sh;
    __shared__ Leader L;
    __shared__ QpShared QS;
    __shared__ int s_cmd;
    __shared__ double s_x[NV];
    const int tid = threadIdx.x;
    const int b_local = blockIdx.x / a.nb, jb = blockIdx.x - b_local * a.nb;
    const int b = a.b0 + b_local;
    const bool leader = jb == 0;
    const int n = a.tb.n, m = a.tb.m;
    SolveCtl* c = a.ctl + b;
    TileSet ts = {0, 0, 0, 0};
    int my_tiles = a.n_tiles;
    if (a.culled) { ts = problem_tiles(a, b); my_tiles = ts.ntq + ts.nsp + 1; }
    const int t0 = (int)(((long long)jb * my_tiles) / a.nb), t1 = (int)(((long long)(jb + 1) * my_tiles) / a.nb);
    int role = 0, r0 = 0, r1 = 0, rdummy;
    if (!a.culled) {
        tile_info(a, t0, role, r0, rdummy);
        tile_info(a, t1 - 1, role, rdummy, r1);
    }
    SolveRow* my_rows = a.blk_rows + ((size_t)(b - a.b0) * a.nb + jb) * a.cap_blk;
    SolveRow* cand = a.qp_rows + (size_t)(b - a.b0) * a.cap_rows;
    unsigned char* flags_g = a.flags + (size_t)(b - a.b0) * 8 * (a.cap_rows + 2 * NV);
    double* g = a.g + (size_t)b * m;
    double* jac = a.jac + (size_t)b * m * n;
    if (leader && tid < 3 * NV) L.bz[tid] = tid < 3 * n ? a.tb.bez[(size_t)b * 3 * n + tid] : 0.0;
    if (leader && tid >= 32 && tid < 32 + NV) L.qdes[tid - 32] = tid - 32 < n ? a.q_des[(size_t)b * n + tid - 32] : 0.0;
    if (leader && tid >= 64 && tid < 64 + NV) L.x[tid - 64] = tid - 64 < n ? ld_coh(&c->x[tid - 64]) : 0.0;
    __syncthreads();
    if (leader && tid == 0) {
        L.t_start = wall_clock64();
        for (int j = 0; j < NV; j++) {
            double Hd = 1e-12;
            if (j < n) {
                const double dk = plan_dk(a, L.bz, j);
                Hd = hess_diag(a.cost_scale, dk);
            }
            L.Hd[j] = Hd;
        }
        L.mu = 1.0; L.it = 0; L.iters = 0; L.evals = 0; L.status = 0; L.stage = ST_AFTER_FIRST; L.ncand = 0; L.sigma = 0.0;
    }
    const double* my_x = s_x;
    unsigned phase = 0;
    const long long t_block = wall_clock64();
    for (;;) {
        if (tid == 0) {
            unsigned w;
            unsigned spins = 0;
            while (((w = ld_coh(&c->go)) >> 3) < phase) {
                __builtin_amdgcn_s_sleep(2);
                if ((++spins & 1023u) == 0 && wall_clock64() - t_block > a.hard_ticks) { w = (unsigned)CMD_DONE; break; }
            }
            asm volatile("" ::: "memory");
            s_cmd = (int)(w & 7u);
        }
        __syncthreads();
        const int cmd = s_cmd;
        if (cmd == CMD_DONE) {
            if (tid == 0) st_coh(&a.blk_word[(size_t)(b - a.b0) * a.nb + jb].flag, 0u);
            break;
        }
        if (tid < NV) s_x[tid] = tid < n ? ld_coh(&c->x[tid]) : 0.0;
        __syncthreads();
        const double kf = tid < n ? s_x[tid] : 0.0;
        for (int t = t0; t < t1; t++) {
            if (a.culled) {
                if (t < ts.ntq + ts.nsp) {
                    KPow& kp = *reinterpret_cast<KPow*>(smem_raw);
                    fill_kpow(kp, kf, n);
                    __syncthreads();
                    if (t < ts.ntq) {
                        const int i = t * P2_BLOCK + tid;
                        if (i < ts.cntq) sparse_torque_row(a.tb, b, a.tq_tiles[(size_t)b * a.tq_cap + i], a.lp.strideT, kp, g, jac);
                    } else {
                        const int i = (t - ts.ntq) * P2_BLOCK + tid;
                        if (i < ts.cnt2) sparse_collision_row<true>(a.tb, a.sl, b, i, kp, g, jac);
                    }
                    __syncthreads();
                    continue;
                }
                role = a.lp.nbc + a.lp.nbt;
            } else {
                int tr0, tr1;
                tile_info(a, t, role, tr0, tr1);
            }
            if (role < a.lp.nbc) {
                if constexpr (LL) {
                    if (a.tb.obs_center) collision_block<true, true, false, true, LL, PPW, false>(a.tb, a.lp, b, role, my_x, kf, g, jac, smem_raw);
                    else collision_block<true, true, false, false, LL, PPW, false>(a.tb, a.lp, b, role, my_x, kf, g, jac, smem_raw);
                } else collision_block<true, true, false, false, LL, PPW, false>(a.tb, a.lp, b, role, my_x, kf, g, jac, smem_raw);
            }
            else if (role < a.lp.nbc + a.lp.nbt) torque_block<true, true, false, false, LL, PPW, false>(a.tb, a.lp, b, role, my_x, kf, g, jac, smem_raw);
            else limit_block<true, true, false, false, LL, PPW, false>(a.tb, a.lp, b, role, my_x, kf, g, jac, smem_raw);
            __syncthreads();
        }
        __builtin_amdgcn_fence(__ATOMIC_SEQ_CST, "workgroup");
        __syncthreads();
        long long vfx = 0;
        int cnt = 0, bad = 0;
        if (a.culled) scan_tiles(a, b, ts, t0, t1, my_rows, a.cap_blk, scan_sh, vfx, cnt, bad);
        else scan_rows<3>(a, b, r0, r1, my_rows, a.cap_blk, scan_sh, vfx, cnt, bad);
        BlockWord* mine = a.blk_word + (size_t)(b - a.b0) * a.nb + jb;
        if (tid == 0) { st_coh(&mine->viol, vfx); st_coh(&mine->bad, bad); st_coh(&mine->count, cnt); }
        wait_my_memory_ops();
        __syncthreads();
        phase++;
        if (tid == 0) st_coh(&mine->flag, phase);
        if (!leader) continue;
        bool group_lost = false;
        for (unsigned spins = 0;; spins++) {
            int all = 1;
#pragma unroll
            for (int e = 0; e < 4; e++) { const int j2 = tid * 4 + e; if (j2 < a.nb && ld_coh(&a.blk_word[(size_t)(b - a.b0) * a.nb + j2].flag) < phase) all = 0; }
            if (__syncthreads_and(all)) break;
            if ((spins & 255u) == 255u && __syncthreads_or(wall_clock64() - t_block > a.hard_ticks ? 1 : 0)) { group_lost = true; break; }
        }
        asm volatile("" ::: "memory");
        if (group_lost) {
            if (tid == 0) {
                a.out[b].status = -1;
                wait_my_memory_ops();
                st_coh(&c->go, phase * 8u + (unsigned)CMD_DONE);
                st_coh(&a.blk_word[(size_t)(b - a.b0) * a.nb + jb].flag, 0u);
            }
            break;
        }
        long long viol_fx = 0;
        int nbad = 0;
        {
            long long v = 0;
            int bd = 0;
#pragma unroll
            for (int e = 0; e < 4; e++) { const int j2 = tid * 4 + e; if (j2 < a.nb) { v += ld_coh(&a.blk_word[(size_t)(b - a.b0) * a.nb + j2].viol); bd += ld_coh(&a.blk_word[(size_t)(b - a.b0) * a.nb + j2].bad); } }
            block_sum(v, bd, scan_sh.red, scan_sh.redi);
            viol_fx = v; nbad = bd;
            __syncthreads();
        }
        if (a.stamps && tid == 0 && phase <= 16) a.stamps[(size_t)b * 64 + 2 * (phase - 1)] = wall_clock64() - L.t_start;
        const int next = leader_step<WPS>(a, L, QS, b, viol_fx, nbad, cand, flags_g, c->x, reinterpret_cast<double*>(smem_raw));
        if (a.stamps && tid == 0 && phase <= 16) a.stamps[(size_t)b * 64 + 2 * (phase - 1) + 1] = wall_clock64() - L.t_start;
        wait_my_memory_ops();
        __syncthreads();
        if (tid == 0) st_coh(&c->go, phase * 8u + (unsigned)next);
        __syncthreads();
    }
}

template <int WPS>
__global__ __launch_bounds__(P2_BLOCK) __attribute__((amdgpu_waves_per_eu(WPS, WPS))) void armour_qp_probe_kernel(const SolveArgs* __restrict__ args, const SolveRow* __restrict__ cand,
                                                                                                                  QpProbe* __restrict__ io) {
    const SolveArgs& a = *args;
    extern __shared__ __attribute__((aligned(16))) unsigned char smem_raw[];
    __shared__ Leader L;
    __shared__ QpShared QS;
    const int tid = threadIdx.x, n = a.tb.n;
    double* lds_stage = reinterpret_cast<double*>(smem_raw);
    if (tid < NV) { L.x[tid] = io->x[tid]; L.gradf[tid] = io->gradf[tid]; L.Hd[tid] = io->Hd[tid]; }
    if (tid == 0) L.ncand = io->ncand;
    __syncthreads();
    if (tid == 0) {
        QS.first_ok = 4;
        for (int j = 0; j < NV; j++) L.invHd[j] = 1.0 / L.Hd[j];
    }
    const double* staged = nullptr;
    if (L.ncand > 64 * (WPS == 1 ? 4 : 2) - 2 * n && L.ncand <= a.lds_rows) {
        for (int i = tid; i < L.ncand; i += 256) {
            const SolveRow& r = cand[i];
#pragma unroll
            for (int j = 0; j < NV; j++) lds_stage[(size_t)j * a.lds_rows + i] = r.a[j];
            lds_stage[(size_t)NV * a.lds_rows + i] = r.v;
        }
        staged = lds_stage;
    }
    __syncthreads();
    solve_qp_wave<WPS>(a, L, QS, cand, staged, a.flags);
    __syncthreads();
    if (tid == 0) {
        int k = 0;
        while (k < 3 && !QS.w[k].feasible) k++;
        const QpWave& W = QS.w[k];
        for (int j = 0; j < NV; j++) io->d[j] = W.qx[j];
        io->max_mult = W.max_mult; io->feasible = W.feasible; io->attempt = k;
        for (int e = 0; e < 4; e++) io->qp_iter[e] = QS.w[e].qp_iter;
    }
}

}

constexpr size_t kSolveLdsOnePerCu = (size_t)96 * 1024, kSolveLdsTwoPerCu = (size_t)40 * 1024;

int armour_qp_probe_lds_rows(int wps) { return (int)((wps == 1 ? kSolveLdsOnePerCu : kSolveLdsTwoPerCu) / ((NV + 1) * sizeof(double))); }

int armour_qp_probe(int n, const SolveRow* rows, int wps, int lds_rows, QpProbe* io) {
    static_assert(P2_BLOCK == 256, "solve_qp_wave: four waves, one per elastic attempt");
    const int ncand = io->ncand;
    if (lds_rows <= 0) lds_rows = armour_qp_probe_lds_rows(wps);
    DevStream st;
    ARMOUR_TRY(st.create());
    DevBuf<SolveRow> d_rows;
    DevBuf<unsigned char> d_flags;
    DevBuf<SolveArgs> d_args;
    DevBuf<QpProbe> d_io;
    SolveArgs a;
    memset(&a, 0, sizeof(a));
    a.tb.n = n; a.nb = 1; a.b0 = 0;
    a.cap_rows = std::max(ncand, 1);
    a.lds_rows = lds_rows;
    ARMOUR_TRY(d_rows.upload(rows, (size_t)ncand, st));
    ARMOUR_TRY(d_flags.reserve((size_t)8 * (a.cap_rows + 2 * NV)));
    a.qp_rows = d_rows; a.flags = d_flags; a.stamps = nullptr;
    ARMOUR_TRY(d_args.upload(&a, 1, st));
    ARMOUR_TRY(d_io.upload(io, 1, st));
    const void* fn = wps == 1 ? (const void*)armour_qp_probe_kernel<1> : (const void*)armour_qp_probe_kernel<2>;
    const size_t smem = (size_t)lds_rows * (NV + 1) * sizeof(double);
    HIPCHK(hipFuncSetAttribute(fn, hipFuncAttributeMaxDynamicSharedMemorySize, (int)smem));
    if (wps == 1) hipLaunchKernelGGL(armour_qp_probe_kernel<1>, dim3(1), dim3(P2_BLOCK), smem, st, d_args.p, d_rows.p, d_io.p);
    else hipLaunchKernelGGL(armour_qp_probe_kernel<2>, dim3(1), dim3(P2_BLOCK), smem, st, d_args.p, d_rows.p, d_io.p);
    HIPCHK(hipGetLastError());
    HIPCHK(hipMemcpyAsync(io, d_io, sizeof(QpProbe), hipMemcpyDeviceToHost, st));
    HIPCHK(hipStreamSynchronize(st));
    return ARMOUR_OK;
}

int armour_solve_device_capacity(const P2Tables& tb, int max_link, int max_torque, const unsigned long long* h_skip, int device, int b_launch, int waves_per_simd, SolvePlan* plan,
                                 int n_tiles_override) {
    P2Launch lp;
    size_t smem = 0;
    bool dfc, six, exact;
    int rc = armour_p2_plan(tb, max_link, max_torque, h_skip, 1, 0, 0, 0, &lp, &smem, &dfc, &six, &exact);
    if (rc != ARMOUR_OK) return rc;
    plan->lp = lp; plan->smem = smem; plan->six = six;
    plan->n_tiles = n_tiles_override > 0 ? n_tiles_override : lp.nbt + lp.nbc + 1;
    int coop = 0;
    HIPCHK(hipDeviceGetAttribute(&coop, hipDeviceAttributeCooperativeLaunch, device));
    if (!coop) { plan->capacity = 0; return ARMOUR_OK; }
    hipDeviceProp_t prop;
    HIPCHK(hipGetDeviceProperties(&prop, device));
    const void* fn1 = !tb.ll_shared ? (const void*)armour_solve_kernel<false, 9, 1> : six ? (const void*)armour_solve_kernel<true, 6, 1> : (const void*)armour_solve_kernel<true, 9, 1>;
    const void* fn2 = !tb.ll_shared ? (const void*)armour_solve_kernel<false, 9, 2> : six ? (const void*)armour_solve_kernel<true, 6, 2> : (const void*)armour_solve_kernel<true, 9, 2>;
    const int wps_env = waves_per_simd;
    const size_t smem1 = std::max(smem, kSolveLdsOnePerCu), smem2 = std::max(smem, kSolveLdsTwoPerCu);
    int per_cu = 0;
    {
        static std::atomic<unsigned long long> set1[3], set2[3];
        const int which = !tb.ll_shared ? 0 : six ? 1 : 2;
        const unsigned long long bit = 1ull << (device & 63);
        if (smem1 > kSolveLdsOnePerCu || !(set1[which].load() & bit)) { HIPCHK(hipFuncSetAttribute(fn1, hipFuncAttributeMaxDynamicSharedMemorySize, (int)smem1)); set1[which].fetch_or(bit); }
        if (smem2 > kSolveLdsTwoPerCu || !(set2[which].load() & bit)) { HIPCHK(hipFuncSetAttribute(fn2, hipFuncAttributeMaxDynamicSharedMemorySize, (int)smem2)); set2[which].fetch_or(bit); }
    }
    HIPCHK(hipOccupancyMaxActiveBlocksPerMultiprocessor(&per_cu, fn1, P2_BLOCK, smem1));
    const int cap1 = per_cu * prop.multiProcessorCount;
    const int blocks1 = cap1 / std::max(1, b_launch);
    const bool one = wps_env ? wps_env == 1 : (blocks1 >= 1 && (n_tiles_override > 0 || (plan->n_tiles + blocks1 - 1) / blocks1 <= 24));
    const void* fn = one ? fn1 : fn2;
    plan->fn = fn;
    plan->smem = one ? smem1 : smem2;
    if (!one) HIPCHK(hipOccupancyMaxActiveBlocksPerMultiprocessor(&per_cu, fn, P2_BLOCK, smem2));
    plan->capacity = per_cu * prop.multiProcessorCount;
    int rate_khz = 0;
    HIPCHK(hipDeviceGetAttribute(&rate_khz, hipDeviceAttributeWallClockRate, device));
    plan->ticks_per_ms = rate_khz > 0 ? (double)rate_khz : 100000.0;
    return ARMOUR_OK;
}

int armour_solve_device_launch(const SolveArgs* d_args, int nb, const SolvePlan& plan, int B, hipStream_t stream) {
    const SolveArgs* p = d_args;
    void* params[1] = {&p};
    HIPCHK(hipLaunchCooperativeKernel(plan.fn, dim3((unsigned)B * (unsigned)nb), dim3(P2_BLOCK), params, (unsigned)plan.smem, stream));
    return ARMOUR_OK;
}
```

Before: 162,000.

## Cache device solve plan and control block, skip redundant uploads and cooperative launch

Caches the device solve plan across calls, keyed by a generation counter and the table contents. Device attributes and occupancy queries are also cached per device. Per-call parameters move into a by-value SolveCall kernel argument, and a generation tag lets the control block stay armed on the device so only changed bytes are uploaded. The cooperative launch is replaced by a plain launch guarded by a capacity check. The aim is to cut host-side planning, memcpy and launch overhead per solve, but co-residency is no longer guaranteed by the runtime and the cache state adds complexity.

```diff
diff --git a/armour_amd/csrc/api.hip b/armour_amd/csrc/api.hip
--- a/armour_amd/csrc/api.hip
+++ b/armour_amd/csrc/api.hip
@@ -249,6 +249,7 @@
     }
     HIPCHK(hipSetDevice(h->device));
     h->ready = false;
+    h->solve_gen++;
     h->rel.fresh = false; h->rel2.fresh = false;
     h->bounds_on_device = false; h->bounds_on_host = false;
     h->tables_from_host = false;
@@ -718,6 +719,7 @@
         if (ok && option == ARMOUR_OPT_P1_STEP_TWO_CU) { const int lv = (int)value % 10; ok = lv <= 3 && (value < 10.0 || lv >= 1); if (ok) h->p1_two_cu_off = false; }
         if (ok) {
             h->tuning[option - ARMOUR_OPT_FIRST_TUNING] = value;
+            h->solve_gen++;
             h->p1_step_cap_hint = 0; h->p1_tv_shape_hint = 0;
             return ARMOUR_OK;
         }
diff --git a/armour_amd/csrc/common.h b/armour_amd/csrc/common.h
--- a/armour_amd/csrc/common.h
+++ b/armour_amd/csrc/common.h
@@ -66,11 +66,17 @@
 #define ARMOUR_MODE_ARMOUR 0
 #define ARMOUR_MODE_ARMTD 1
 
+struct SolveCache;
 struct SolveDeviceWork {
     DevBuf<unsigned char> ctl;
     DevBuf<unsigned char> blk_word;
     int words_clean = 0;
     DevBuf<unsigned char> blk_rows, qp_rows, flags;
+    SolveCache* cache = nullptr;
+    SolveDeviceWork() = default;
+    SolveDeviceWork(const SolveDeviceWork&) = delete;
+    SolveDeviceWork& operator=(const SolveDeviceWork&) = delete;
+    ~SolveDeviceWork();
 };
 
 struct RelLists {
@@ -102,8 +108,9 @@
     int row0 = 0;
     std::vector<double> h_krange;
     DevBuf<double> d_jrs;
-    void* solve_pin[10] = {nullptr, nullptr, nullptr, nullptr, nullptr, nullptr, nullptr, nullptr, nullptr, nullptr};
-    size_t solve_pin_bytes[10] = {0, 0, 0, 0, 0, 0, 0, 0, 0, 0};
+    void* solve_pin[11] = {nullptr, nullptr, nullptr, nullptr, nullptr, nullptr, nullptr, nullptr, nullptr, nullptr, nullptr};
+    size_t solve_pin_bytes[11] = {0, 0, 0, 0, 0, 0, 0, 0, 0, 0, 0};
+    unsigned long long solve_gen = 0;
     bool stats_fresh = false;
     int opt_p1_build = 0;
     double opt_p1_work_mb = 0;
diff --git a/armour_amd/csrc/solver.hip b/armour_amd/csrc/solver.hip
--- a/armour_amd/csrc/solver.hip
+++ b/armour_amd/csrc/solver.hip
@@ -431,17 +431,33 @@
     return ARMOUR_OK;
 }
 
+struct SolveCache {
+    bool planned = false;
+    unsigned long long gen = 0;
+    P2Tables tb;
+    DevicePlan p;
+    const void* dev_block = nullptr;
+    const void* sent = nullptr;
+    bool armed = false;
+    int armed_B = 0;
+    unsigned ctl_gen = 0;
+    size_t fixed_off = 0, fixed_bytes = 0;
+};
+SolveDeviceWork::~SolveDeviceWork() { delete cache; }
+
 struct DeviceStage {
-    SolveArgs a;
+    SolveCall call;
     ArmourSolveResult* hres = nullptr;
     unsigned char* hblock = nullptr;
     long long* hstamps = nullptr;
     size_t off_args = 0, args_stride = 0, block_bytes = 0;
+    size_t up_off = 0, up_bytes = 0;
     double hard_s = 0;
 };
 
-static int stage_device_solve(ArmourPlanner* h, const ArmourSolveOptions& opt, const double* k_start, const P2Tables& tb, const DevicePlan& p, Clock::time_point t_begin, DeviceStage& s) {
+static int stage_device_solve(ArmourPlanner* h, const ArmourSolveOptions& opt, const double* k_start, const P2Tables& tb, SolveCache& c, Clock::time_point t_begin, DeviceStage& s) {
     const int B = h->B, n = h->n, m = h->m;
+    const DevicePlan& p = c.p;
     const SolvePlan& plan = p.plan;
     int rc;
     if ((rc = armour_upload_bounds(h)) != ARMOUR_OK) return rc;
@@ -453,23 +469,23 @@
     ARMOUR_TRY(w.ctl.reserve(s.block_bytes));
     bool fresh = false;
     ARMOUR_TRY(w.blk_word.reserve((size_t)p.Bs * p.nb * sizeof(BlockWord), &fresh));
+    if (!w.words_clean) c.armed = false;
     if (fresh || !w.words_clean) HIPCHK(hipMemsetAsync(w.blk_word, 0, w.blk_word.cap, h->stream));
     w.words_clean = 0;
     ARMOUR_TRY(w.blk_rows.reserve((size_t)p.Bs * p.nb * p.cap_blk * sizeof(SolveRow)));
     ARMOUR_TRY(w.qp_rows.reserve((size_t)p.Bs * p.cap_rows * sizeof(SolveRow)));
     ARMOUR_TRY(w.flags.reserve((size_t)p.Bs * 8 * (p.cap_rows + 2 * NV)));
     s.hres = reinterpret_cast<ArmourSolveResult*>(armour_handle_pinned(h, 1, (size_t)B * sizeof(ArmourSolveResult)));
-    s.hblock = reinterpret_cast<unsigned char*>(armour_handle_pinned(h, 2, s.block_bytes));
+    s.hblock = reinterpret_cast<unsigned char*>(armour_handle_pinned(h, 10, 2 * s.block_bytes));
     if (!s.hres || !s.hblock) return ARMOUR_EDEVICE;
-    SolveCtl* hctl = reinterpret_cast<SolveCtl*>(s.hblock);
+    unsigned char* sent = s.hblock + s.block_bytes;
+    if (c.dev_block != (const void*)w.ctl.p || c.sent != (const void*)sent) { c.dev_block = w.ctl.p; c.sent = sent; c.armed = false; c.fixed_bytes = 0; }
+    if (c.armed_B != B) c.armed = false;
     memset(s.hres, 0, (size_t)B * sizeof(ArmourSolveResult));
-    memset(hctl, 0, (size_t)B * sizeof(SolveCtl));
-    for (int b = 0; b < B; b++) {
-        hctl[b].go = 1; s.hres[b].status = -2;
-        if (k_start) for (int j = 0; j < n; j++) hctl[b].x[j] = k_start[(size_t)b * n + j];
-    }
+    for (int b = 0; b < B; b++) s.hres[b].status = -2;
+    memset(s.hblock + off_qdes, 0, s.block_bytes - off_qdes);
     memcpy(s.hblock + off_qdes, h->h_qdes.data(), (size_t)B * n * sizeof(double));
-    SolveArgs& a = s.a;
+    SolveArgs a;
     memset(&a, 0, sizeof(a));
     a.tb = tb; a.lp = plan.lp; a.nb = p.nb; a.n_tiles = plan.n_tiles; a.cap_blk = p.cap_blk; a.cap_rows = p.cap_rows;
     a.lds_rows = (int)(plan.smem / ((NV + 1) * sizeof(double)));
@@ -479,27 +495,50 @@
     a.blk_rows = w.blk_rows.as<SolveRow>(); a.qp_rows = w.qp_rows.as<SolveRow>(); a.flags = w.flags;
     a.q_des = reinterpret_cast<const double*>(w.ctl + off_qdes); a.out = s.hres;
     a.continuous_mask = h->continuous_mask();
-    a.max_iter = opt.max_iterations; a.max_ls = opt.max_line_search; a.tol = opt.tolerance;
     const slv::RowRule rule = armour_row_rule(h);
     a.n_checked_collision = rule.n_checked; a.torque_slack = rule.torque_slack; a.collision_slack = rule.collision_slack;
     a.t_plan = h->params.t_plan; a.cost_scale = h->params.cost_scale;
-    a.budget_ticks = -1;
-    if (opt.max_wall_time_s > 0) {
-        const double left_ms = (opt.max_wall_time_s - std::chrono::duration<double>(Clock::now() - t_begin).count()) * 1e3 / p.n_launch;
-        a.budget_ticks = left_ms > 0 ? (long long)(left_ms * plan.ticks_per_ms) : 0;
-    }
-    const double hard_cap_s = h->tune_f(ARMOUR_OPT_SOLVE_HARD_CAP_S);
-    const double no_budget_s = std::max(5.0, 1.0 + 50.0 * (double)std::max(1, opt.max_iterations) * (1.0 + std::max(0, opt.max_line_search)) * p.tiles_per_block * 4e-6);
-    s.hard_s = hard_cap_s > 0 ? hard_cap_s : (a.budget_ticks >= 0 ? a.budget_ticks / plan.ticks_per_ms * 1e-3 + 1.0 : no_budget_s);
-    a.hard_ticks = std::max<long long>(1, (long long)(s.hard_s * 1e3 * plan.ticks_per_ms));
     const bool timing = armour_trace_solve();
     s.hstamps = timing ? reinterpret_cast<long long*>(armour_handle_pinned(h, 0, (size_t)B * 64 * sizeof(long long) + (size_t)B * n * sizeof(double))) : nullptr;
     if (s.hstamps) memset(s.hstamps, 0, (size_t)B * 64 * sizeof(long long));
     a.stamps = s.hstamps;
-    return ARMOUR_OK;
-}
-
-static void report_device_timing(const ArmourPlanner* h, const DevicePlan& p, const DeviceStage& s, double ms, Clock::time_point t_begin, Clock::time_point t_launch) {
+    for (int li = 0; li < p.n_launch; li++) { a.b0 = li * p.Bs; memcpy(s.hblock + s.off_args + (size_t)li * s.args_stride, &a, sizeof(SolveArgs)); }
+    SolveCall& call = s.call;
+    memset(&call, 0, sizeof(call));
+    call.max_iter = opt.max_iterations; call.max_ls = opt.max_line_search; call.tol = opt.tolerance;
+    call.budget_ticks = -1;
+    if (opt.max_wall_time_s > 0) {
+        const double left_ms = (opt.max_wall_time_s - std::chrono::duration<double>(Clock::now() - t_begin).count()) * 1e3 / p.n_launch;
+        call.budget_ticks = left_ms > 0 ? (long long)(left_ms * plan.ticks_per_ms) : 0;
+    }
+    const double hard_cap_s = h->tune_f(ARMOUR_OPT_SOLVE_HARD_CAP_S);
+    const double no_budget_s = std::max(5.0, 1.0 + 50.0 * (double)std::max(1, opt.max_iterations) * (1.0 + std::max(0, opt.max_line_search)) * p.tiles_per_block * 4e-6);
+    s.hard_s = hard_cap_s > 0 ? hard_cap_s : (call.budget_ticks >= 0 ? call.budget_ticks / plan.ticks_per_ms * 1e-3 + 1.0 : no_budget_s);
+    call.hard_ticks = std::max<long long>(1, (long long)(s.hard_s * 1e3 * plan.ticks_per_ms));
+    const size_t ctl_bytes = (size_t)B * sizeof(SolveCtl);
+    const bool send_ctl = !c.armed || k_start != nullptr;
+    if (!c.armed) c.ctl_gen++;
+    call.gen = c.ctl_gen;
+    if (send_ctl) {
+        SolveCtl* hctl = reinterpret_cast<SolveCtl*>(s.hblock);
+        memset(hctl, 0, off_qdes);
+        for (int b = 0; b < B; b++) {
+            hctl[b].go = 1; hctl[b].gen = c.ctl_gen;
+            if (k_start) for (int j = 0; j < n; j++) hctl[b].x[j] = k_start[(size_t)b * n + j];
+        }
+    }
+    const size_t fixed_bytes = s.block_bytes - off_qdes;
+    const bool send_fixed = c.fixed_off != off_qdes || c.fixed_bytes != fixed_bytes || memcmp(sent + off_qdes, s.hblock + off_qdes, fixed_bytes) != 0;
+    s.up_off = send_ctl ? 0 : off_qdes;
+    s.up_bytes = send_fixed ? s.block_bytes - s.up_off : send_ctl ? ctl_bytes : 0;
+    if (send_fixed) { memcpy(sent + off_qdes, s.hblock + off_qdes, fixed_bytes); c.fixed_off = off_qdes; c.fixed_bytes = fixed_bytes; }
+    c.armed = false;
+    return ARMOUR_OK;
+}
+
+struct HostStamps { Clock::time_point planned, staged, copied, launched, done, results; };
+
+static void report_device_timing(const ArmourPlanner* h, const DevicePlan& p, const DeviceStage& s, double ms, Clock::time_point t_begin, Clock::time_point t_launch, const HostStamps& hs) {
     const SolvePlan& plan = p.plan;
     const ArmourSolveResult* hres = s.hres;
     const long long* hstamps = s.hstamps;
@@ -525,24 +564,39 @@
     long long longest_ok = 0, long_bad = 0, steps_all = 0;
     for (int b = 0; b < B; b++) { const long long* st = hstamps + (size_t)b * 64; longest_ok = std::max(longest_ok, st[48]); long_bad += st[49]; steps_all += st[44] + st[45] + st[46] + st[47]; }
     fprintf(stderr, "\n   all problems: %lld QP steps; longest attempt that ended feasible %lld steps; attempts of more than 60 steps that ended infeasible: %lld\n", steps_all, longest_ok, long_bad);
+    const auto us = [](Clock::time_point a, Clock::time_point b) { return std::chrono::duration<double, std::micro>(b - a).count(); };
+    fprintf(stderr, "[armour_solve, device form] host us: plan %.2f stage %.2f copy %.2f launch %.2f wait %.2f results %.2f\n", us(t_begin, hs.planned), us(hs.planned, hs.staged),
+            us(hs.staged, hs.copied), us(hs.copied, hs.launched), us(hs.launched, hs.done), us(hs.done, hs.results));
 }
 
 static int solve_on_device(ArmourPlanner* h, const ArmourSolveOptions& opt, const double* k_start, ArmourSolveResult* results, Clock::time_point t_begin, DeviceOutcome* out) {
     *out = DeviceOutcome::HandBack;
     const P2Tables tb = armour_make_tables(h);
-    DevicePlan p;
+    SolveDeviceWork& w = h->solve_dev;
+    if (!w.cache) w.cache = new SolveCache();
+    SolveCache& c = *w.cache;
     DeviceStage s;
+    HostStamps hs;
     int rc;
-    if ((rc = plan_device_solve(h, tb, p)) != ARMOUR_OK || p.plan.capacity < 1) return rc;
-    if ((rc = stage_device_solve(h, opt, k_start, tb, p, t_begin, s)) != ARMOUR_OK) return rc;
-    SolveDeviceWork& w = h->solve_dev;
+    if (!c.planned || c.gen != h->solve_gen || memcmp(&c.tb, &tb, sizeof(tb)) != 0) {
+        c.planned = false;
+        c.p = DevicePlan();
+        if ((rc = plan_device_solve(h, tb, c.p)) != ARMOUR_OK) return rc;
+        c.planned = true; c.gen = h->solve_gen; memcpy(&c.tb, &tb, sizeof(tb));
+    }
+    const DevicePlan& p = c.p;
+    if (p.plan.capacity < 1) return ARMOUR_OK;
+    hs.planned = Clock::now();
+    if ((rc = stage_device_solve(h, opt, k_start, tb, c, t_begin, s)) != ARMOUR_OK) return rc;
     const int B = h->B, n_launch = p.n_launch;
     const auto t_launch = Clock::now();
-    for (int li = 0; li < n_launch; li++) { s.a.b0 = li * p.Bs; memcpy(s.hblock + s.off_args + (size_t)li * s.args_stride, &s.a, sizeof(SolveArgs)); }
-    HIPCHK(hipMemcpyAsync(w.ctl, s.hblock, s.block_bytes, hipMemcpyHostToDevice, h->stream));
+    hs.staged = t_launch;
+    if (s.up_bytes) HIPCHK(hipMemcpyAsync(w.ctl + s.up_off, s.hblock + s.up_off, s.up_bytes, hipMemcpyHostToDevice, h->stream));
+    hs.copied = Clock::now();
     for (int li = 0; li < n_launch; li++)
-        if ((rc = armour_solve_device_launch(reinterpret_cast<const SolveArgs*>(w.ctl + s.off_args + (size_t)li * s.args_stride), p.nb, p.plan,
+        if ((rc = armour_solve_device_launch(reinterpret_cast<const SolveArgs*>(w.ctl + s.off_args + (size_t)li * s.args_stride), s.call, p.nb, p.plan,
                                              std::min(p.Bs, B - li * p.Bs), h->stream)) != ARMOUR_OK) return rc;
+    hs.launched = Clock::now();
     for (unsigned long long polls = 0;; polls++) {
         const hipError_t q = hipStreamQuery(h->stream);
         if (q == hipSuccess) break;
@@ -552,12 +606,15 @@
             return ARMOUR_EDEVICE;
         }
     }
+    hs.done = Clock::now();
+    for (int b = 0; b < B; b++)
+        if (s.hres[b].status < 0) return ARMOUR_OK;
     w.words_clean = 1;
-    for (int b = 0; b < B; b++)
-        if (s.hres[b].status < 0) { w.words_clean = 0; return ARMOUR_OK; }
+    c.armed = true; c.armed_B = B; c.ctl_gen++;
     const double ms = std::chrono::duration<double, std::milli>(Clock::now() - t_begin).count();
-    if (s.hstamps) report_device_timing(h, p, s, ms, t_begin, t_launch);
     for (int b = 0; b < B; b++) { results[b] = s.hres[b]; results[b].time_ms = ms; }
+    hs.results = Clock::now();
+    if (s.hstamps) report_device_timing(h, p, s, ms, t_begin, t_launch, hs);
     *out = DeviceOutcome::Solved;
     return ARMOUR_OK;
 }
diff --git a/armour_amd/csrc/solver_device.h b/armour_amd/csrc/solver_device.h
--- a/armour_amd/csrc/solver_device.h
+++ b/armour_amd/csrc/solver_device.h
@@ -6,7 +6,7 @@
 
 struct alignas(128) SolveCtl {
     unsigned go;
-    int pad0;
+    unsigned gen;
     double x[slv::NV];
 };
 struct alignas(64) BlockWord {
@@ -37,12 +37,18 @@
     const double* q_des;
     ArmourSolveResult* out;
     int continuous_mask;
+    int n_checked_collision;
+    double t_plan, cost_scale, torque_slack, collision_slack;
+    long long* stamps;
+};
+
+struct SolveCall {
     int max_iter, max_ls;
-    int n_checked_collision;
-    double t_plan, cost_scale, tol, torque_slack, collision_slack;
+    unsigned gen;
+    int pad0;
+    double tol;
     long long budget_ticks;
     long long hard_ticks;
-    long long* stamps;
 };
 
 struct SolvePlan {
@@ -60,7 +66,7 @@
 int armour_solve_device_capacity(const P2Tables& tb, int max_link, int max_torque, const unsigned long long* h_skip, int device, int b_launch, int waves_per_simd, SolvePlan* plan,
                                  int n_tiles_override = 0);
 int armour_solver_lists(ArmourPlanner* h, p2::SparseList* sl, const int** tq_tiles, const int** tq_count, int* tq_cap);
-int armour_solve_device_launch(const SolveArgs* d_args, int nb, const SolvePlan& plan, int B, hipStream_t stream);
+int armour_solve_device_launch(const SolveArgs* d_args, const SolveCall& call, int nb, const SolvePlan& plan, int B, hipStream_t stream);
 
 struct QpProbe {
     double x[slv::NV], gradf[slv::NV], Hd[slv::NV];
diff --git a/armour_amd/csrc/solver_device.hip b/armour_amd/csrc/solver_device.hip
--- a/armour_amd/csrc/solver_device.hip
+++ b/armour_amd/csrc/solver_device.hip
@@ -2,6 +2,7 @@
 #include <atomic>
 #include <cmath>
 #include <cstring>
+#include <mutex>
 
 #include "bezier.h"
 #include "cacc.h"
@@ -22,10 +23,12 @@
 
 __device__ inline unsigned ld_coh(const unsigned* p) { return __hip_atomic_load(p, __ATOMIC_RELAXED, __HIP_MEMORY_SCOPE_AGENT); }
 __device__ inline int ld_coh(const int* p) { return __hip_atomic_load(p, __ATOMIC_RELAXED, __HIP_MEMORY_SCOPE_AGENT); }
+__device__ inline unsigned long long ld_coh(const unsigned long long* p) { return __hip_atomic_load(p, __ATOMIC_RELAXED, __HIP_MEMORY_SCOPE_AGENT); }
 __device__ inline long long ld_coh(const long long* p) { return __hip_atomic_load(p, __ATOMIC_RELAXED, __HIP_MEMORY_SCOPE_AGENT); }
 __device__ inline double ld_coh(const double* p) { return __longlong_as_double(__hip_atomic_load(reinterpret_cast<const long long*>(p), __ATOMIC_RELAXED, __HIP_MEMORY_SCOPE_AGENT)); }
 __device__ inline void st_coh(unsigned* p, unsigned v) { __hip_atomic_store(p, v, __ATOMIC_RELAXED, __HIP_MEMORY_SCOPE_AGENT); }
 __device__ inline void st_coh(int* p, int v) { __hip_atomic_store(p, v, __ATOMIC_RELAXED, __HIP_MEMORY_SCOPE_AGENT); }
+__device__ inline void st_coh(unsigned long long* p, unsigned long long v) { __hip_atomic_store(p, v, __ATOMIC_RELAXED, __HIP_MEMORY_SCOPE_AGENT); }
 __device__ inline void st_coh(long long* p, long long v) { __hip_atomic_store(p, v, __ATOMIC_RELAXED, __HIP_MEMORY_SCOPE_AGENT); }
 __device__ inline void st_coh(double* p, double v) { __hip_atomic_store(reinterpret_cast<long long*>(p), __double_as_longlong(v), __ATOMIC_RELAXED, __HIP_MEMORY_SCOPE_AGENT); }
 __device__ inline void wait_my_memory_ops() { asm volatile("s_waitcnt vmcnt(0) lgkmcnt(0)" ::: "memory"); }
@@ -650,7 +653,7 @@
 }
 
 template <int WPS>
-__device__ __forceinline__ int leader_step(const SolveArgs& a, Leader& L, QpShared& QS, int b, long long viol_fx, int bad, SolveRow* cand,
+__device__ __forceinline__ int leader_step(const SolveArgs& a, const SolveCall& call, Leader& L, QpShared& QS, int b, long long viol_fx, int bad, SolveRow* cand,
                                   unsigned char* flags_g, double* x_pub, double* lds_stage) {
     const int n = a.tb.n, tid = threadIdx.x;
     const double viol = viol_from_fixed(viol_fx);
@@ -675,8 +678,8 @@
         } else {
             L.evals++;
             const double phi = fpt + L.mu * viol;
-            if (phi <= L.phi0 + 1e-4 * L.alpha * L.dphi || L.ls == a.max_ls) {
-                if (L.ls == a.max_ls && phi > L.phi0) { L.status = 4; L.stop = 1; }
+            if (phi <= L.phi0 + 1e-4 * L.alpha * L.dphi || L.ls == call.max_ls) {
+                if (L.ls == call.max_ls && phi > L.phi0) { L.status = 4; L.stop = 1; }
                 else {
                     for (int j = 0; j < n; j++) { L.x[j] = L.xt[j]; L.gradf[j] = L.np[j]; }
                     L.f = fpt; L.viol = viol; L.bad = bad; L.iters++; L.it++;
@@ -691,8 +694,8 @@
         }
         L.stage = ST_AFTER_TRIAL;
         if (L.stop == 0) {
-            if (L.it >= a.max_iter) { L.status = 2; L.stop = 1; }
-            else if (a.budget_ticks >= 0 && wall_clock64() - L.t_start >= a.budget_ticks) { L.status = 5; L.stop = 1; }
+            if (L.it >= call.max_iter) { L.status = 2; L.stop = 1; }
+            else if (call.budget_ticks >= 0 && wall_clock64() - L.t_start >= call.budget_ticks) { L.status = 5; L.stop = 1; }
         }
     }
     __syncthreads();
@@ -744,7 +747,7 @@
                 else {
                     double dn = 0, gd = 0;
                     for (int j = 0; j < n; j++) { L.d[j] = L.qx[j]; dn = fmax(dn, fabs(L.qx[j])); gd += L.gradf[j] * L.qx[j]; }
-                    if (dn <= a.tol * 1e-2 || (dn <= a.tol && L.viol <= a.tol)) { L.status = 1; L.stop = 1; }
+                    if (dn <= call.tol * 1e-2 || (dn <= call.tol && L.viol <= call.tol)) { L.status = 1; L.stop = 1; }
                     else {
                         L.mu = fmax(L.mu, 1.5 * L.max_mult + 1e-3);
                         L.phi0 = L.f + L.mu * L.viol;
@@ -794,7 +797,7 @@
 }
 
 template <bool LL, int PPW, int WPS>
-__global__ __launch_bounds__(P2_BLOCK) __attribute__((amdgpu_waves_per_eu(WPS, WPS))) void armour_solve_kernel(const SolveArgs* __restrict__ args) {
+__global__ __launch_bounds__(P2_BLOCK) __attribute__((amdgpu_waves_per_eu(WPS, WPS))) void armour_solve_kernel(const SolveArgs* __restrict__ args, const SolveCall call) {
     const SolveArgs& a = *args;
     extern __shared__ __attribute__((aligned(16))) unsigned char smem_raw[];
     __shared__ ScanShared scan_sh;
@@ -808,6 +811,7 @@
     const bool leader = jb == 0;
     const int n = a.tb.n, m = a.tb.m;
     SolveCtl* c = a.ctl + b;
+    unsigned long long* go_gen = reinterpret_cast<unsigned long long*>(&c->go);
     TileSet ts = {0, 0, 0, 0};
     int my_tiles = a.n_tiles;
     if (a.culled) { ts = problem_tiles(a, b); my_tiles = ts.ntq + ts.nsp + 1; }
@@ -845,9 +849,13 @@
         if (tid == 0) {
             unsigned w;
             unsigned spins = 0;
-            while (((w = ld_coh(&c->go)) >> 3) < phase) {
+            for (;;) {
+                const unsigned long long w2 = ld_coh(go_gen);
+                w = (unsigned)w2;
+                if ((unsigned)(w2 >> 32) != call.gen) { w = (unsigned)CMD_DONE; break; }
+                if ((w >> 3) >= phase) break;
                 __builtin_amdgcn_s_sleep(2);
-                if ((++spins & 1023u) == 0 && wall_clock64() - t_block > a.hard_ticks) { w = (unsigned)CMD_DONE; break; }
+                if ((++spins & 1023u) == 0 && wall_clock64() - t_block > call.hard_ticks) { w = (unsigned)CMD_DONE; break; }
             }
             asm volatile("" ::: "memory");
             s_cmd = (int)(w & 7u);
@@ -911,7 +919,7 @@
 #pragma unroll
             for (int e = 0; e < 4; e++) { const int j2 = tid * 4 + e; if (j2 < a.nb && ld_coh(&a.blk_word[(size_t)(b - a.b0) * a.nb + j2].flag) < phase) all = 0; }
             if (__syncthreads_and(all)) break;
-            if ((spins & 255u) == 255u && __syncthreads_or(wall_clock64() - t_block > a.hard_ticks ? 1 : 0)) { group_lost = true; break; }
+            if ((spins & 255u) == 255u && __syncthreads_or(wall_clock64() - t_block > call.hard_ticks ? 1 : 0)) { group_lost = true; break; }
         }
         asm volatile("" ::: "memory");
         if (group_lost) {
@@ -935,11 +943,15 @@
             __syncthreads();
         }
         if (a.stamps && tid == 0 && phase <= 16) a.stamps[(size_t)b * 64 + 2 * (phase - 1)] = wall_clock64() - L.t_start;
-        const int next = leader_step<WPS>(a, L, QS, b, viol_fx, nbad, cand, flags_g, c->x, reinterpret_cast<double*>(smem_raw));
+        const int next = leader_step<WPS>(a, call, L, QS, b, viol_fx, nbad, cand, flags_g, c->x, reinterpret_cast<double*>(smem_raw));
         if (a.stamps && tid == 0 && phase <= 16) a.stamps[(size_t)b * 64 + 2 * (phase - 1) + 1] = wall_clock64() - L.t_start;
+        if (next == CMD_DONE && tid < NV) st_coh(&c->x[tid], 0.0);
         wait_my_memory_ops();
         __syncthreads();
-        if (tid == 0) st_coh(&c->go, phase * 8u + (unsigned)next);
+        if (tid == 0) {
+            if (next == CMD_DONE) st_coh(go_gen, ((unsigned long long)(call.gen + 1u) << 32) | 1ull);
+            else st_coh(&c->go, phase * 8u + (unsigned)next);
+        }
         __syncthreads();
     }
 }
@@ -1020,6 +1032,54 @@
     return ARMOUR_OK;
 }
 
+namespace {
+struct SolveDeviceFacts {
+    bool known = false;
+    int coop = 0, cus = 0, rate_khz = 0;
+    int per_cu[3][2] = {{-1, -1}, {-1, -1}, {-1, -1}};
+};
+constexpr int kFactDevices = 64;
+std::mutex g_facts_mu;
+SolveDeviceFacts g_facts[kFactDevices];
+
+constexpr int kAdmittedBlocksPerCu = std::min(8, 800 / (112 + 16));
+
+int solve_device_facts(int device, SolveDeviceFacts* out) {
+    const bool cached = device >= 0 && device < kFactDevices;
+    if (cached) {
+        std::lock_guard<std::mutex> lk(g_facts_mu);
+        if (g_facts[device].known) { *out = g_facts[device]; return ARMOUR_OK; }
+    }
+    SolveDeviceFacts f;
+    HIPCHK(hipDeviceGetAttribute(&f.coop, hipDeviceAttributeCooperativeLaunch, device));
+    HIPCHK(hipDeviceGetAttribute(&f.cus, hipDeviceAttributeMultiprocessorCount, device));
+    HIPCHK(hipDeviceGetAttribute(&f.rate_khz, hipDeviceAttributeWallClockRate, device));
+    f.known = true;
+    if (cached) {
+        std::lock_guard<std::mutex> lk(g_facts_mu);
+        if (!g_facts[device].known) g_facts[device] = f;
+        *out = g_facts[device];
+    } else *out = f;
+    return ARMOUR_OK;
+}
+
+int solve_blocks_per_cu(int device, int which, int two, const void* fn, size_t smem, bool standard, int* per_cu) {
+    const bool cached = standard && device >= 0 && device < kFactDevices;
+    if (cached) {
+        std::lock_guard<std::mutex> lk(g_facts_mu);
+        if (g_facts[device].per_cu[which][two] >= 0) { *per_cu = g_facts[device].per_cu[which][two]; return ARMOUR_OK; }
+    }
+    int api = 0;
+    HIPCHK(hipOccupancyMaxActiveBlocksPerMultiprocessor(&api, fn, P2_BLOCK, smem));
+    *per_cu = std::min(api, kAdmittedBlocksPerCu);
+    if (cached) {
+        std::lock_guard<std::mutex> lk(g_facts_mu);
+        g_facts[device].per_cu[which][two] = *per_cu;
+    }
+    return ARMOUR_OK;
+}
+}
+
 int armour_solve_device_capacity(const P2Tables& tb, int max_link, int max_torque, const unsigned long long* h_skip, int device, int b_launch, int waves_per_simd, SolvePlan* plan,
                                  int n_tiles_override) {
     P2Launch lp;
@@ -1029,41 +1089,39 @@
     if (rc != ARMOUR_OK) return rc;
     plan->lp = lp; plan->smem = smem; plan->six = six;
     plan->n_tiles = n_tiles_override > 0 ? n_tiles_override : lp.nbt + lp.nbc + 1;
-    int coop = 0;
-    HIPCHK(hipDeviceGetAttribute(&coop, hipDeviceAttributeCooperativeLaunch, device));
-    if (!coop) { plan->capacity = 0; return ARMOUR_OK; }
-    hipDeviceProp_t prop;
-    HIPCHK(hipGetDeviceProperties(&prop, device));
+    SolveDeviceFacts facts;
+    if ((rc = solve_device_facts(device, &facts)) != ARMOUR_OK) return rc;
+    if (!facts.coop) { plan->capacity = 0; return ARMOUR_OK; }
     const void* fn1 = !tb.ll_shared ? (const void*)armour_solve_kernel<false, 9, 1> : six ? (const void*)armour_solve_kernel<true, 6, 1> : (const void*)armour_solve_kernel<true, 9, 1>;
     const void* fn2 = !tb.ll_shared ? (const void*)armour_solve_kernel<false, 9, 2> : six ? (const void*)armour_solve_kernel<true, 6, 2> : (const void*)armour_solve_kernel<true, 9, 2>;
     const int wps_env = waves_per_simd;
     const size_t smem1 = std::max(smem, kSolveLdsOnePerCu), smem2 = std::max(smem, kSolveLdsTwoPerCu);
+    const int which = !tb.ll_shared ? 0 : six ? 1 : 2;
     int per_cu = 0;
     {
         static std::atomic<unsigned long long> set1[3], set2[3];
-        const int which = !tb.ll_shared ? 0 : six ? 1 : 2;
         const unsigned long long bit = 1ull << (device & 63);
         if (smem1 > kSolveLdsOnePerCu || !(set1[which].load() & bit)) { HIPCHK(hipFuncSetAttribute(fn1, hipFuncAttributeMaxDynamicSharedMemorySize, (int)smem1)); set1[which].fetch_or(bit); }
         if (smem2 > kSolveLdsTwoPerCu || !(set2[which].load() & bit)) { HIPCHK(hipFuncSetAttribute(fn2, hipFuncAttributeMaxDynamicSharedMemorySize, (int)smem2)); set2[which].fetch_or(bit); }
     }
-    HIPCHK(hipOccupancyMaxActiveBlocksPerMultiprocessor(&per_cu, fn1, P2_BLOCK, smem1));
-    const int cap1 = per_cu * prop.multiProcessorCount;
+    if ((rc = solve_blocks_per_cu(device, which, 0, fn1, smem1, smem1 == kSolveLdsOnePerCu, &per_cu)) != ARMOUR_OK) return rc;
+    const int cap1 = per_cu * facts.cus;
     const int blocks1 = cap1 / std::max(1, b_launch);
     const bool one = wps_env ? wps_env == 1 : (blocks1 >= 1 && (n_tiles_override > 0 || (plan->n_tiles + blocks1 - 1) / blocks1 <= 24));
     const void* fn = one ? fn1 : fn2;
     plan->fn = fn;
     plan->smem = one ? smem1 : smem2;
-    if (!one) HIPCHK(hipOccupancyMaxActiveBlocksPerMultiprocessor(&per_cu, fn, P2_BLOCK, smem2));
-    plan->capacity = per_cu * prop.multiProcessorCount;
-    int rate_khz = 0;
-    HIPCHK(hipDeviceGetAttribute(&rate_khz, hipDeviceAttributeWallClockRate, device));
-    plan->ticks_per_ms = rate_khz > 0 ? (double)rate_khz : 100000.0;
+    if (!one && (rc = solve_blocks_per_cu(device, which, 1, fn, smem2, smem2 == kSolveLdsTwoPerCu, &per_cu)) != ARMOUR_OK) return rc;
+    plan->capacity = per_cu * facts.cus;
+    plan->ticks_per_ms = facts.rate_khz > 0 ? (double)facts.rate_khz : 100000.0;
     return ARMOUR_OK;
 }
 
-int armour_solve_device_launch(const SolveArgs* d_args, int nb, const SolvePlan& plan, int B, hipStream_t stream) {
+int armour_solve_device_launch(const SolveArgs* d_args, const SolveCall& call, int nb, const SolvePlan& plan, int B, hipStream_t stream) {
+    if ((long long)B * nb > plan.capacity) { armour_set_error("armour_solve (device form): %d x %d blocks exceed the %d the device holds at once", B, nb, plan.capacity); return ARMOUR_EINVAL; }
     const SolveArgs* p = d_args;
-    void* params[1] = {&p};
-    HIPCHK(hipLaunchCooperativeKernel(plan.fn, dim3((unsigned)B * (unsigned)nb), dim3(P2_BLOCK), params, (unsigned)plan.smem, stream));
+    SolveCall by_value = call;
+    void* params[2] = {&p, &by_value};
+    HIPCHK(hipLaunchKernel(plan.fn, dim3((unsigned)B * (unsigned)nb), dim3(P2_BLOCK), params, plan.smem, stream));
     return ARMOUR_OK;
 }
```

Result: no change. 160,700 (-0.8%).
